# binli123/dsmil-wsi

Hardware: AMD Instinct MI355X
Metric: bags/sec aggregated (10kx512) (higher is better)
Workload: dtype f32; 1 GPU; DSMIL aggregator forward (FCLayer+BClassifier), c16 weights C=1, 64 bags x 10000 x 512 fp32 per GPU per pass, HBM-resident; bags_per_pass_per_gpu=64, rows=10000, feats=512, classes=1, tile_rows=128, parallelism=bag-sharded x1, streams=3, distinct_batches=3, logits_form=1, device_cus=256, persistent_grid=256

## Files before the change

### dsmil-wsi_amd/_native.py

```python
import ctypes
import os

PKG_DIR = os.path.dirname(os.path.abspath(__file__))
LIB_PATH = os.path.join(PKG_DIR, os.path.basename(os.environ.get("DSMIL_NATIVE_LIB", "libdsmil_hip.so")))

c_f32p = ctypes.c_void_p
c_i64p = ctypes.c_void_p


class NativeLibraryError(RuntimeError):
    pass


class AggParams(ctypes.Structure):
    _fields_ = [("fc_w", ctypes.c_void_p), ("fc_b", ctypes.c_void_p),
                ("q0_w", ctypes.c_void_p), ("q0_b", ctypes.c_void_p),
                ("q2_w", ctypes.c_void_p), ("q2_b", ctypes.c_void_p),
                ("fcc_w", ctypes.c_void_p), ("fcc_b", ctypes.c_void_p),
                ("K", ctypes.c_int32), ("Kv", ctypes.c_int32),
                ("C", ctypes.c_int32), ("nonlinear", ctypes.c_int32)]


class AggOpts(ctypes.Structure):
    _fields_ = [("packed_split", ctypes.c_void_p), ("row_map", ctypes.c_void_p), ("packed_f2", ctypes.c_void_p)]


class AggCall(ctypes.Structure):
    _fields_ = [("total_rows", ctypes.c_int64), ("max_rows", ctypes.c_int64)] + [(n, ctypes.c_int32) for n in (
        "n_bags", "K", "Kv", "C", "nonlinear", "bf16", "aligned", "classes_given", "vals_separate", "row_map", "packed_split",
        "packed_f2", "phase", "skip_pred", "prologue_job", "several_streams", "cus")]


class AggRoute(ctypes.Structure):
    _fields_ = [(n, ctypes.c_int32) for n in (
        "nw", "r0", "logits", "logits_vec", "logits_cp", "prologue", "rowmax", "qmax", "qmax_vec", "qmax_threads", "ragged",
        "ragged_attend", "tile_attend", "tile_logits", "image", "attend", "attend_nw", "attend_vec", "attend_np", "attend_xe",
        "attend_tu", "finish", "finish_rows", "pred")]


LOGITS = ("none", "given", "stream", "pipe", "argmax")
QMAX = ("launch", "inline", "shard1", "shard2")
IMAGE = ("none", "f2_caller", "f2_cut", "split_caller", "split_cut", "bf16")
ATTEND = ("none", "f3", "f2", "bf16_res", "bf16_dma", "bf16_ring", "split", "hs", "f32")
FINISH = ("none", "lean", "vec4", "scalar")


def forward_route(**call):
    c = AggCall(**dict({"aligned": 7}, **call))
    r = AggRoute()
    check(lib().dsmil_agg_forward_route(ctypes.byref(c), ctypes.byref(r)), "dsmil_agg_forward_route")
    return r


class AggGrads(ctypes.Structure):
    _fields_ = [(n, ctypes.c_void_p) for n in
                ("fc_w", "fc_b", "q0_w", "q0_b", "q2_w", "q2_b", "fcc_w", "fcc_b")]


class BceWeights(ctypes.Structure):
    _fields_ = [("pos_weight", ctypes.c_void_p), ("weight", ctypes.c_void_p)]


class AdamState(ctypes.Structure):
    _fields_ = [("exp_avg", ctypes.POINTER(ctypes.c_void_p)), ("exp_avg_sq", ctypes.POINTER(ctypes.c_void_p)),
                ("step", ctypes.c_int64), ("lr", ctypes.c_double), ("beta1", ctypes.c_double), ("beta2", ctypes.c_double),
                ("eps", ctypes.c_double), ("weight_decay", ctypes.c_double)]


SIGNATURES = {
    "dsmil_abi_version": (ctypes.c_int, []),
    "dsmil_strerror": (ctypes.c_char_p, [ctypes.c_int]),
    "dsmil_agg_mlp_form": (ctypes.c_int, []),
    "dsmil_agg_inline_query": (ctypes.c_int, [ctypes.c_int]),
    "dsmil_agg_batch_form": (ctypes.c_int, [ctypes.c_int]),
    "dsmil_agg_persistent_grid": (ctypes.c_int, [ctypes.c_int]),
    "dsmil_agg_logits_form": (ctypes.c_int, [ctypes.c_int]),
    "dsmil_device_cus": (ctypes.c_int, []),
    "dsmil_agg_packed_f2_bytes": (ctypes.c_size_t, [ctypes.c_int32]),
    "dsmil_agg_pack_f2": (ctypes.c_int, [c_f32p, c_f32p, ctypes.c_int32, ctypes.c_void_p, ctypes.c_void_p]),
    "dsmil_agg_packed_split_bytes": (ctypes.c_size_t, [ctypes.c_int32, ctypes.c_int32]),
    "dsmil_agg_pack_split": (ctypes.c_int, [c_f32p, c_f32p, ctypes.c_int32, ctypes.c_void_p, ctypes.c_void_p]),
    "dsmil_agg_forward_ex": (ctypes.c_int, [c_f32p, c_f32p, c_i64p, ctypes.c_int32, ctypes.c_int64,
                                            ctypes.c_int64, ctypes.POINTER(AggParams), ctypes.POINTER(AggOpts), c_f32p,
                                            c_f32p, c_f32p, c_f32p, c_f32p, c_i64p, ctypes.c_void_p,
                                            ctypes.c_size_t, ctypes.c_void_p]),
    "dsmil_agg_loss_head": (ctypes.c_int, [c_f32p, c_f32p, c_i64p, c_f32p, ctypes.c_int32, c_f32p, c_f32p, c_f32p,
                                           c_f32p, ctypes.c_void_p]),
    "dsmil_agg_loss_head_w": (ctypes.c_int, [c_f32p, c_f32p, c_i64p, c_f32p, ctypes.c_int32, c_f32p, c_f32p, c_f32p,
                                             c_f32p, ctypes.POINTER(BceWeights), ctypes.c_void_p]),
    "dsmil_agg_backward_ex": (ctypes.c_int, [c_f32p, c_f32p, ctypes.c_int64, ctypes.POINTER(AggParams), c_f32p,
                                             c_f32p, c_i64p, c_f32p, c_f32p, c_f32p, c_f32p, c_f32p,
                                             ctypes.POINTER(AggGrads), c_f32p, c_i64p, ctypes.c_void_p, ctypes.c_size_t,
                                             ctypes.c_void_p]),
    "dsmil_agg_shard_argmax": (ctypes.c_int, [c_f32p, ctypes.c_int64, ctypes.POINTER(AggParams), c_f32p, c_f32p,
                                              c_i64p, ctypes.c_void_p, ctypes.c_size_t, ctypes.c_void_p]),
    "dsmil_agg_shard_attend": (ctypes.c_int, [c_f32p, c_f32p, ctypes.c_int64, ctypes.POINTER(AggParams), c_f32p,
                                              c_f32p, c_f32p, c_f32p, ctypes.c_void_p, ctypes.c_size_t,
                                              ctypes.c_void_p]),
    "dsmil_agg_tile_rows": (ctypes.c_int, [ctypes.c_int32, ctypes.c_int64]),
    "dsmil_agg_forward_route": (ctypes.c_int, [ctypes.POINTER(AggCall), ctypes.POINTER(AggRoute)]),
    "dsmil_agg_workspace_bytes": (ctypes.c_size_t, [ctypes.c_int32, ctypes.c_int64, ctypes.c_int32,
                                                    ctypes.c_int32, ctypes.c_int32]),
    "dsmil_agg_packed_bf16_bytes": (ctypes.c_size_t, [ctypes.c_int32]),
    "dsmil_agg_pack_bf16": (ctypes.c_int, [c_f32p, c_f32p, ctypes.c_int32, ctypes.c_void_p, ctypes.c_void_p]),
    "dsmil_agg_forward_bf16": (ctypes.c_int, [ctypes.c_void_p, ctypes.c_void_p, c_i64p, ctypes.c_int32,
                                              ctypes.c_int64, ctypes.c_int64, ctypes.POINTER(AggParams),
                                              ctypes.c_void_p, c_f32p, c_f32p, c_f32p, c_f32p, c_f32p, c_i64p,
                                              ctypes.c_void_p, ctypes.c_size_t, ctypes.c_void_p]),
    "dsmil_profile_enable": (ctypes.c_int, [ctypes.c_int]),
    "dsmil_profile_collect": (ctypes.c_int, [ctypes.c_int, ctypes.POINTER(ctypes.c_double), ctypes.POINTER(ctypes.c_int64)]),
    "dsmil_resnet18_packed_bytes": (ctypes.c_size_t, []),
    "dsmil_resnet18_pack": (ctypes.c_int, [ctypes.POINTER(ctypes.c_void_p), c_f32p, ctypes.c_void_p]),
    "dsmil_resnet18_workspace_bytes": (ctypes.c_size_t, [ctypes.c_int32, ctypes.c_int32, ctypes.c_int32]),
    "dsmil_resnet18in_forward": (ctypes.c_int, [c_f32p, ctypes.c_int32, ctypes.c_int32, ctypes.c_int32,
                                                c_f32p, c_f32p, c_f32p, c_f32p, ctypes.c_int32, c_f32p,
                                                c_f32p, ctypes.c_void_p, ctypes.c_size_t, ctypes.c_void_p]),
    "dsmil_resnet18in_forward_u8": (ctypes.c_int, [ctypes.c_void_p, ctypes.c_int32, ctypes.c_int32, ctypes.c_int32,
                                                   c_f32p, c_f32p, c_f32p, c_f32p, ctypes.c_int32, c_f32p,
                                                   c_f32p, ctypes.c_void_p, ctypes.c_size_t, ctypes.c_void_p]),
    "dsmil_resnet18_norm_channels": (ctypes.c_int32, []),
    "dsmil_resnet18bn_forward": (ctypes.c_int, [ctypes.c_void_p, ctypes.c_int32, ctypes.c_int32, ctypes.c_int32,
                                                ctypes.c_int32, c_f32p, c_f32p, c_f32p, c_f32p, c_f32p, c_f32p,
                                                ctypes.c_int32, c_f32p, c_f32p, ctypes.c_void_p, ctypes.c_size_t,
                                                ctypes.c_void_p]),
    "dsmil_resnet_num_convs": (ctypes.c_int32, [ctypes.c_int32]),
    "dsmil_resnet_workspace_bytes": (ctypes.c_size_t, [ctypes.c_int32, ctypes.c_int32, ctypes.c_int32, ctypes.c_int32]),
    "dsmil_resnet_feature_dim": (ctypes.c_int32, [ctypes.c_int32]),
    "dsmil_resnet_mfma_forms": (ctypes.c_int, [ctypes.POINTER(ctypes.c_int32), ctypes.POINTER(ctypes.c_int32)]),
    "dsmil_resnet_norm_channels": (ctypes.c_int32, [ctypes.c_int32]),
    "dsmil_resnet_packed_bytes": (ctypes.c_size_t, [ctypes.c_int32]),
    "dsmil_resnet_packed_bytes_ex": (ctypes.c_size_t, [ctypes.c_int32, ctypes.c_int32]),
    "dsmil_resnet_pack": (ctypes.c_int, [ctypes.c_int32, ctypes.POINTER(ctypes.c_void_p), c_f32p, ctypes.c_void_p]),
    "dsmil_resnet_forward": (ctypes.c_int, [ctypes.c_int32, ctypes.c_void_p, ctypes.c_int32, ctypes.c_int32,
                                            ctypes.c_int32, ctypes.c_int32, c_f32p, c_f32p, c_f32p, c_f32p, c_f32p,
                                            c_f32p, ctypes.c_int32, c_f32p, c_f32p, ctypes.c_void_p,
                                            ctypes.c_size_t, ctypes.c_void_p]),
    "dsmil_resnet_pack_ex": (ctypes.c_int, [ctypes.c_int32, ctypes.POINTER(ctypes.c_void_p), c_f32p, ctypes.c_int32, ctypes.c_void_p]),
    "dsmil_resnet_forward_ex": (ctypes.c_int, [ctypes.c_int32, ctypes.c_void_p, ctypes.c_int32, ctypes.c_int32,
                                               ctypes.c_int32, ctypes.c_int32, c_f32p, c_f32p, c_f32p, c_f32p, c_f32p,
                                               c_f32p, ctypes.c_int32, c_f32p, c_f32p, ctypes.c_void_p,
                                               ctypes.c_size_t, ctypes.c_int32, ctypes.c_void_p]),
    "dsmil_trunk16_positions": (ctypes.c_size_t, [ctypes.c_int32, ctypes.c_int32, ctypes.c_int32]),
    "dsmil_trunk16_layout": (ctypes.c_int, [c_f32p, ctypes.c_void_p] + [ctypes.c_int32] * 6 + [ctypes.c_void_p]),
    "dsmil_trunk16_conv_workspace_bytes": (ctypes.c_size_t, [ctypes.c_int32, ctypes.c_int32, ctypes.c_int32]),
    "dsmil_trunk16_conv": (ctypes.c_int, [ctypes.c_void_p, c_f32p, ctypes.c_void_p] + [ctypes.c_int32] * 9 +
                           [ctypes.c_void_p, ctypes.c_size_t, ctypes.c_void_p]),
    "dsmil_trunk16_norm_workspace_bytes": (ctypes.c_size_t, [ctypes.c_int32, ctypes.c_int32]),
    "dsmil_trunk16_norm": (ctypes.c_int, [ctypes.c_void_p, ctypes.c_void_p, ctypes.c_void_p] + [ctypes.c_int32] * 6 +
                           [ctypes.c_void_p, ctypes.c_size_t, ctypes.c_void_p]),
    "dsmil_trunk16_pool": (ctypes.c_int, [ctypes.c_void_p, ctypes.c_void_p, c_f32p] + [ctypes.c_int32] * 5 +
                           [ctypes.c_void_p, ctypes.c_size_t, ctypes.c_void_p]),
    "dsmil_trunk16_workspace_bytes": (ctypes.c_size_t, [ctypes.c_int32] * 4),
    "dsmil_trunk16_forward": (ctypes.c_int, [ctypes.c_int32, c_f32p, ctypes.c_int32, ctypes.c_int32, ctypes.c_int32,
                                             ctypes.POINTER(ctypes.c_void_p), c_f32p, ctypes.c_int32, ctypes.c_void_p,
                                             ctypes.c_size_t, ctypes.c_void_p]),
    "dsmil_trunk32_conv_plan": (ctypes.c_int, [ctypes.c_int32] * 10 + [ctypes.POINTER(ctypes.c_int32)]),
    "dsmil_trunk32_conv_workspace_bytes": (ctypes.c_size_t, [ctypes.c_int32] * 9),
    "dsmil_trunk32_conv": (ctypes.c_int, [c_f32p] * 9 + [ctypes.c_int32] * 9 + [ctypes.c_void_p, ctypes.c_size_t, ctypes.c_void_p]),
    "dsmil_trunk32_stem_workspace_bytes": (ctypes.c_size_t, [ctypes.c_int32] * 3),
    "dsmil_trunk32_stem": (ctypes.c_int, [ctypes.c_void_p, ctypes.c_int32] + [c_f32p] * 6 + [ctypes.c_int32] * 4 +
                           [ctypes.c_void_p, ctypes.c_size_t, ctypes.c_void_p]),
    "dsmil_trunk32_tail": (ctypes.c_int, [ctypes.c_int32] + [c_f32p] * 7 + [ctypes.c_int32] * 4 + [ctypes.c_void_p]),
    "dsmil_tile_stats": (ctypes.c_int, [ctypes.c_void_p, ctypes.c_int32, ctypes.c_int32, ctypes.c_int32, ctypes.c_void_p,
                                        ctypes.c_void_p]),
    "dsmil_jpeg_plan_bytes": (ctypes.c_size_t, [ctypes.c_int32]),
    "dsmil_jpeg_workspace_bytes": (ctypes.c_size_t, [ctypes.c_int32, ctypes.c_int32, ctypes.c_int32, ctypes.c_int64]),
    "dsmil_jpeg_parse": (ctypes.c_int, [ctypes.c_void_p, ctypes.c_void_p, ctypes.c_int32, ctypes.c_void_p]),
    "dsmil_read_files": (ctypes.c_int64, [ctypes.c_void_p, ctypes.c_void_p, ctypes.c_int32, ctypes.c_void_p, ctypes.c_int64, ctypes.c_void_p]),
    "dsmil_csv_parse_f32": (ctypes.c_int64, [ctypes.c_void_p, ctypes.c_int64, ctypes.c_int64, ctypes.c_void_p, ctypes.c_int64]),
    "dsmil_csv_format_f32": (ctypes.c_int64, [ctypes.c_void_p, ctypes.c_int64, ctypes.c_int64, ctypes.c_int64, ctypes.c_int32,
                                              ctypes.c_void_p, ctypes.c_int64]),
    "dsmil_jpeg_decode": (ctypes.c_int, [ctypes.c_void_p, ctypes.c_int64, ctypes.c_void_p, ctypes.c_int32, ctypes.c_int32, ctypes.c_int32,
                                         ctypes.c_void_p, ctypes.c_void_p, ctypes.c_void_p, ctypes.c_size_t, ctypes.c_void_p]),
    "dsmil_fc_forward": (ctypes.c_int, [c_f32p, ctypes.c_int64, ctypes.c_int32, ctypes.c_int32,
                                        c_f32p, c_f32p, c_f32p, ctypes.c_void_p]),
    "dsmil_agg_backward_workspace_bytes": (ctypes.c_size_t, [ctypes.c_int64, ctypes.c_int32, ctypes.c_int32,
                                                             ctypes.c_int32]),
    "dsmil_agg_backward": (ctypes.c_int, [c_f32p, c_f32p, ctypes.c_int64, ctypes.POINTER(AggParams), c_f32p,
                                          c_f32p, c_i64p, c_f32p, c_f32p, c_f32p, c_f32p,
                                          ctypes.POINTER(AggGrads), c_f32p, ctypes.c_void_p, ctypes.c_size_t,
                                          ctypes.c_void_p]),
    "dsmil_agg_backward_rows_workspace_bytes": (ctypes.c_size_t, [ctypes.c_int64, ctypes.c_int32, ctypes.c_int32,
                                                                  ctypes.c_int32]),
    "dsmil_agg_backward_rows": (ctypes.c_int, [c_f32p, c_f32p, ctypes.c_int64, ctypes.POINTER(AggParams), c_f32p,
                                               c_f32p, c_i64p, c_f32p, c_f32p, c_f32p, c_f32p, c_f32p,
                                               ctypes.POINTER(AggGrads), c_f32p, c_i64p, ctypes.c_void_p, ctypes.c_size_t,
                                               ctypes.c_void_p, c_f32p]),
    "dsmil_agg_backward_bags_workspace_bytes": (ctypes.c_size_t, [ctypes.c_int32, ctypes.c_int64, ctypes.c_int32,
                                                                  ctypes.c_int32, ctypes.c_int32]),
    "dsmil_agg_backward_bags": (ctypes.c_int, [c_f32p, c_f32p, c_i64p, ctypes.c_int32, ctypes.c_int64, ctypes.c_int64,
                                               ctypes.POINTER(AggParams), c_f32p, c_f32p, c_i64p, c_f32p, c_f32p, c_f32p,
                                               c_f32p, c_f32p, ctypes.POINTER(AggGrads), c_f32p, c_i64p, ctypes.c_void_p,
                                               ctypes.c_size_t, ctypes.c_void_p, c_f32p]),
    "dsmil_agg_backward_bags_bf16_workspace_bytes": (ctypes.c_size_t, [ctypes.c_int32, ctypes.c_int64, ctypes.c_int32,
                                                                       ctypes.c_int32, ctypes.c_int32]),
    "dsmil_agg_backward_bags_bf16": (ctypes.c_int, [ctypes.c_void_p, ctypes.c_void_p, c_i64p, ctypes.c_int32, ctypes.c_int64,
                                                    ctypes.c_int64, ctypes.POINTER(AggParams), c_f32p, c_f32p, c_i64p, c_f32p,
                                                    c_f32p, c_f32p, c_f32p, c_f32p, ctypes.POINTER(AggGrads), c_f32p,
                                                    ctypes.c_void_p, ctypes.c_size_t, ctypes.c_void_p]),
    "dsmil_agg_loss_head_bags": (ctypes.c_int, [c_f32p, c_i64p, c_f32p, c_i64p, c_f32p, ctypes.c_int32, ctypes.c_int32,
                                                c_f32p, c_f32p, c_f32p, c_f32p, ctypes.c_void_p]),
    "dsmil_agg_loss_head_bags_w": (ctypes.c_int, [c_f32p, c_i64p, c_f32p, c_i64p, c_f32p, ctypes.c_int32, ctypes.c_int32,
                                                  c_f32p, c_f32p, c_f32p, c_f32p, ctypes.POINTER(BceWeights), ctypes.c_void_p]),
    "dsmil_value_backward_rows": (ctypes.c_int, [c_f32p, c_f32p, c_f32p, ctypes.c_int64, ctypes.c_int32, ctypes.c_int32,
                                                 c_f32p, ctypes.c_void_p, ctypes.c_int32, c_f32p, ctypes.c_void_p,
                                                 ctypes.c_size_t, ctypes.c_void_p]),
    "dsmil_value_packed_bytes": (ctypes.c_size_t, [ctypes.c_int32, ctypes.c_int32]),
    "dsmil_value_pack": (ctypes.c_int, [c_f32p, ctypes.c_int32, ctypes.c_int32, ctypes.c_void_p, ctypes.c_void_p]),
    "dsmil_value_workspace_bytes": (ctypes.c_size_t, [ctypes.c_int64, ctypes.c_int32, ctypes.c_int32]),
    "dsmil_value_forward": (ctypes.c_int, [c_f32p, ctypes.c_int64, ctypes.c_int32, ctypes.c_int32, c_f32p, c_f32p,
                                           ctypes.c_void_p, c_i64p, c_f32p, ctypes.c_void_p, ctypes.c_size_t, ctypes.c_void_p]),
    "dsmil_value_backward": (ctypes.c_int, [c_f32p, c_f32p, c_f32p, ctypes.c_int64, ctypes.c_int32, ctypes.c_int32, c_i64p,
                                            c_f32p, c_f32p, ctypes.c_void_p, ctypes.c_size_t, ctypes.c_void_p]),
    "dsmil_value_packed_bf16_bytes": (ctypes.c_size_t, [ctypes.c_int32, ctypes.c_int32]),
    "dsmil_value_pack_bf16": (ctypes.c_int, [c_f32p, ctypes.c_int32, ctypes.c_int32, ctypes.c_void_p, ctypes.c_void_p]),
    "dsmil_value_workspace_bf16_bytes": (ctypes.c_size_t, [ctypes.c_int64, ctypes.c_int32, ctypes.c_int32]),
    "dsmil_value_forward_bf16": (ctypes.c_int, [ctypes.c_void_p, ctypes.c_int64, ctypes.c_int32, ctypes.c_int32, c_f32p, c_f32p,
                                                ctypes.c_void_p, ctypes.c_void_p, ctypes.c_void_p, ctypes.c_size_t,
                                                ctypes.c_void_p]),
    "dsmil_value_backward_bf16_workspace_bytes": (ctypes.c_size_t, [ctypes.c_int64, ctypes.c_int32, ctypes.c_int32]),
    "dsmil_value_backward_bf16": (ctypes.c_int, [ctypes.c_void_p, ctypes.c_void_p, c_f32p, ctypes.c_int64, ctypes.c_int32,
                                                 ctypes.c_int32, c_f32p, c_f32p, ctypes.c_void_p, ctypes.c_size_t,
                                                 ctypes.c_void_p]),
    "dsmil_agg_train_step_workspace_bytes": (ctypes.c_size_t, [ctypes.c_int64, ctypes.c_int32, ctypes.c_int32, ctypes.c_int32]),
    "dsmil_agg_train_step": (ctypes.c_int, [c_f32p, ctypes.c_int64, c_i64p, c_f32p, ctypes.POINTER(AggParams),
                                            ctypes.POINTER(AdamState), c_f32p, ctypes.c_void_p, ctypes.c_size_t,
                                            ctypes.c_void_p]),
    "dsmil_agg_train_step_bags_workspace_bytes": (ctypes.c_size_t, [ctypes.c_int32, ctypes.c_int64, ctypes.c_int32,
                                                                    ctypes.c_int32, ctypes.c_int32]),
# ... 73 lines not shown
```

### dsmil-wsi_amd/csrc/agg_f3.h

```cpp
#pragma once
#include "agg_f2.h"

namespace {

constexpr int F3_BM = 32;
constexpr int F3_THREADS = 256;
constexpr int F3_MAX_WG = 1024;
constexpr int F3_HROW = 528;
constexpr int F3_SCR = 1856;
__host__ __device__ constexpr int f3_row_bytes(int K) { return 4 * K + 16; }
__host__ __device__ constexpr int f3_lds_bytes(int K) { return 2 * F3_BM * f3_row_bytes(K) + F3_BM * F3_HROW + F3_SCR * 4; }

__device__ __forceinline__ void f3_mfma_a(f32x4& acc, const f32x4& a_agpr, const f32x4& b) {
    asm volatile("v_mfma_f32_16x16x32_f16 %0, %1, %2, %0" : "+v"(acc) : "a"(a_agpr), "v"(b));
}
__device__ __forceinline__ void f3_mfma_a0(f32x4& acc, const f32x4& a_agpr, const f32x4& b) {
    asm volatile("v_mfma_f32_16x16x32_f16 %0, %1, %2, 0" : "=&v"(acc) : "a"(a_agpr), "v"(b));
}
__device__ __forceinline__ void f3_mfma_v(f32x4& acc, const f32x4& a, const f32x4& b) {
    asm volatile("v_mfma_f32_16x16x32_f16 %0, %1, %2, %0" : "+v"(acc) : "v"(a), "v"(b));
}
__device__ __forceinline__ void f3_mfma_v0(f32x4& acc, const f32x4& a, const f32x4& b) {
    asm volatile("v_mfma_f32_16x16x32_f16 %0, %1, %2, 0" : "=&v"(acc) : "v"(a), "v"(b));
}
#define F3_NOP() asm volatile("s_nop 15" ::: "memory")

template <int B, int E, class F>
__device__ __forceinline__ void f3_static_for(F&& f) {
    if constexpr (B < E) {
        f(std::integral_constant<int, B>{});
        f3_static_for<B + 1, E>(f);
    }
}

struct F3Work {
    int bag;
    long long off0, Nb, row0;
};

struct F3Cur {
    int item, b, tile;
};
__device__ __forceinline__ F3Cur f3_next(F3Cur c, int tiles_per_bag) {
    ++c.item;
    if (++c.tile == tiles_per_bag) { c.tile = 0; ++c.b; }
    return c;
}

__device__ __forceinline__ bool f3_fetch(const AttendArgs& a, int tiles_per_bag, int end, F3Cur& c, F3Work& w, const F3Work* hint = nullptr) {
    const __attribute__((address_space(4))) long long* offs = (const __attribute__((address_space(4))) long long*)(uintptr_t)a.offsets;
    while (c.item < end) {
        const int bag = a.bag0 + c.b;
        long long off0, Nb;
        if (hint && hint->bag == bag) { off0 = hint->off0; Nb = hint->Nb; }
        else { off0 = offs[bag]; Nb = offs[bag + 1] - off0; }
        const long long row0 = (long long)c.tile * F3_BM;
        if (row0 < Nb) {
            w.bag = bag; w.off0 = off0; w.Nb = Nb; w.row0 = row0;
            return true;
        }
        if (tiles_per_bag) c.item += tiles_per_bag - c.tile;
        c.tile = 0;
        ++c.b;
    }
    return false;
}

template <int NK1, bool TWO, int DBG = 0>
__global__ __launch_bounds__(F3_THREADS, 1) void k_attend_f3(AttendArgs a, const float* __restrict__ rowmax, int tiles_per_bag,
                                                             int n_items, int per_wg) {
    static_assert(NK1 % 4 == 0 && NK1 >= 4 && NK1 <= 16, "K a multiple of 128 up to 512");
    constexpr int K = 32 * NK1, NKS = 2 * NK1, NG = NK1 / 2;
    constexpr int RB = f3_row_bytes(K), BUF = F3_BM * RB;
    constexpr int NC = TWO ? 2 : 1;
    constexpr bool W2_STREAM = NK1 > 8;
    constexpr int NMOVE = 2;
    extern __shared__ __attribute__((aligned(16))) float smem[];
    char* sX = reinterpret_cast<char*>(smem);
    char* sH = sX + 2 * BUF;
    float* scr = reinterpret_cast<float*>(sH + F3_BM * F3_HROW);
    float* sS = scr;
    float* sBias = scr + 1024;
    float* sPall = scr + 1280;
    float* sInvAll = scr + 1536;
    float* sQ = scr + 1600;
    const int tid = threadIdx.x, lane = tid & 63;
    const int wave = __builtin_amdgcn_readfirstlane(tid >> 6);
    const int l31 = lane & 31, hi = lane >> 5;
    const int l15 = lane & 15, g = lane >> 4;
    const int ubase = 32 * wave + 16 * (g >> 1) + 4 * (g & 1);
    const f32x4* wimg = reinterpret_cast<const f32x4*>(a.wpk);
    const float* trailer = reinterpret_cast<const float*>(wimg + (long long)(NKS + 8) * F2_CHUNK_F4);
    const float* feats = reinterpret_cast<const float*>(a.feats);
    const float scale = 0.08838834764831845f;

    F3Cur pos;
    pos.item = (int)blockIdx.x * per_wg;
    if (a.tile_pre) {
        const int real = ((const __attribute__((address_space(4))) int*)(uintptr_t)a.tile_pre)[a.n_bags];
        n_items = n_items < real ? n_items : real;
        if (pos.item >= n_items) return;
        pos.b = tile_owner(a.tile_pre, a.n_bags, pos.item);
        pos.tile = pos.item - a.tile_pre[pos.b];
    } else {
        pos.b = pos.item / tiles_per_bag;
        pos.tile = pos.item - pos.b * tiles_per_bag;
    }
    const int item_end = pos.item + per_wg < n_items ? pos.item + per_wg : n_items;
    F3Work cur, nxt, nn;
    if (!f3_fetch(a, tiles_per_bag, item_end, pos, cur)) return;

    F2Frag w1[NK1][2][2], w2[4][2][2];
#pragma unroll
    for (int s = 0; s < NK1; ++s)
#pragma unroll
        for (int uh = 0; uh < 2; ++uh)
#pragma unroll
            for (int p = 0; p < 2; ++p) w1[s][uh][p].f = wimg[f3_frag_slot(s, 2 * wave + uh, p, lane)];
    const f32x4* w2p1 = wimg + f3_frag_slot(NK1, 2 * wave, 1, lane);
#pragma unroll
    for (int st = 0; st < 4; ++st)
#pragma unroll
        for (int uh = 0; uh < 2; ++uh) {
            w2[st][uh][0].f = wimg[f3_frag_slot(NK1 + st, 2 * wave + uh, 0, lane)];
            if constexpr (!W2_STREAM) w2[st][uh][1].f = w2p1[(long long)2 * st * F2_CHUNK_F4 + 8 * uh];
        }
    const float ia1 = trailer[0], ia2 = trailer[1];
    const float hb_n1 = trailer[2] * 16384.f;
    const float hb_b = wave_max(fmaxf(fabsf(a.q0_b[lane]), fabsf(a.q0_b[lane + 64])));
    sBias[tid] = tid < QD ? a.q0_b[tid] : a.q2_b[tid - QD];
#pragma unroll
    for (int s = 0; s < NK1; ++s)
#pragma unroll
        for (int uh = 0; uh < 2; ++uh)
#pragma unroll
            for (int p = 0; p < 2; ++p) asm volatile("" : "+a"(w1[s][uh][p].f));

    const int rr = lane & 7, o = lane >> 3;
    const int myrow = 8 * wave + rr;
    f32x4 ring[NG][2];
    auto row_raw = [&](const F3Work& w, float& rm, long long& phys, long long& logical) {
        long long gr = w.row0 + myrow;
        if (gr >= w.Nb) gr = w.Nb - 1;
        rm = rowmax[w.off0 + gr];
        const long long* mp = a.rowmap ? reinterpret_cast<const long long*>(a.rowmap) + (w.off0 + gr) : reinterpret_cast<const long long*>(a.offsets);
        phys = *mp;
        logical = w.off0 + gr;
    };
    auto row_done = [&](float rm, long long phys, long long logical, float& sc, float& sinv) -> const float* {
        sc = f2_scale(rm, sinv);
        return feats + (a.rowmap ? phys : logical) * (long long)K + 8 * o;
    };
    auto row_src = [&](const F3Work& w, float& sc, float& sinv) -> const float* {
        float rm;
        long long phys, logical;
        row_raw(w, rm, phys, logical);
        asm volatile("" : "+v"(phys));
        return row_done(rm, phys, logical, sc, sinv);
    };
    auto fill = [&](const float* src, int c) {
        ring[c][0] = *(const DSMIL_GLOBAL f32x4*)(src + 64 * c);
        ring[c][1] = *(const DSMIL_GLOBAL f32x4*)(src + 64 * c + 4);
    };
    char* const cut_dst = sX + myrow * RB + 16 * o;
    auto cut_write = [&](int pb, int c, float sc) {
        F2Frag f[2];
        split2h_scaled(ring[c][0], ring[c][1], sc, f);
        char* d = cut_dst + pb * BUF + 128 * c;
        *reinterpret_cast<f32x4*>(d) = f[0].f;
        *reinterpret_cast<f32x4*>(d + 2 * K) = f[1].f;
    };

    F2Frag cutf[2];
    auto cut_piece = [&](int pb, auto s_c, auto j_c, float sc, const float* refill_src) {
        constexpr int s_ = decltype(s_c)::value, j = decltype(j_c)::value;
        constexpr int c = s_ / 2, ph = (s_ % 2) * 8 + j;
        if constexpr (c < NG) {
            char* d = cut_dst + pb * BUF + 128 * c;
            if constexpr (ph < 8) {
                constexpr int i = ph / 2;
                const float va = i < 2 ? ring[c][0][(2 * i) & 3] : ring[c][1][(2 * i) & 3];
                const float vb = i < 2 ? ring[c][0][(2 * i + 1) & 3] : ring[c][1][(2 * i + 1) & 3];
                if constexpr (ph % 2 == 0) {
                    unsigned h;
                    asm("v_fma_mixlo_f16 %0, %1, %3, 0\n\tv_fma_mixhi_f16 %0, %2, %3, 0" : "=&v"(h) : "v"(va), "v"(vb), "v"(sc));
                    cutf[0].u[i] = h;
                } else {
                    unsigned l;
                    const unsigned h = cutf[0].u[i];
                    asm("v_fma_mixlo_f16 %0, %1, %3, -%4 op_sel_hi:[0,0,1]\n\tv_fma_mixhi_f16 %0, %2, %3, -%4 op_sel:[0,0,1] op_sel_hi:[0,0,1]"
                        : "=&v"(l) : "v"(va), "v"(vb), "v"(sc), "v"(h));
                    cutf[1].u[i] = l;
                }
            } else if constexpr (ph == 8) {
                *reinterpret_cast<f32x4*>(d) = cutf[0].f;
            } else if constexpr (ph == 9) {
                *reinterpret_cast<f32x4*>(d + 2 * K) = cutf[1].f;
            } else if constexpr (ph == 10) {
                if constexpr (DBG != 4 && c < NG - NMOVE) fill(refill_src, c);
            }
        }
    };

    float sc_c = 1.f, sinv_c = 1.f, sc_n = 1.f, sinv_n = 1.f, sc_nn = 1.f, sinv_nn = 1.f;
    const float* src_c = row_src(cur, sc_c, sinv_c);
#pragma unroll
    for (int c = 0; c < NG; ++c) fill(src_c, c);
    F3Cur pos_n = f3_next(pos, tiles_per_bag);
    bool has_next = f3_fetch(a, tiles_per_bag, item_end, pos_n, nxt);
    const float* src_n = has_next ? row_src(nxt, sc_n, sinv_n) : src_c;
    if (!has_next) { nxt = cur; sc_n = sc_c; sinv_n = sinv_c; }
#pragma unroll
    for (int c = 0; c < NG; ++c) {
        cut_write(0, c, sc_c);
        fill(src_n, c);
    }
    if (o == 0) sInvAll[myrow] = sinv_c;
    F3Cur pos_nn = f3_next(pos_n, tiles_per_bag);
    bool has_nn = has_next && f3_fetch(a, tiles_per_bag, item_end, pos_nn, nn);
    const float* src_nn = has_nn ? row_src(nn, sc_nn, sinv_nn) : src_n;
    if (!has_nn) { nn = nxt; sc_nn = sc_n; sinv_nn = sinv_n; }

    float bacc[NC][8];
    float l_run[NC];
    float m_bag[NC];
    auto reset_acc = [&]() {
#pragma unroll
        for (int c = 0; c < NC; ++c) {
            l_run[c] = 0.f;
#pragma unroll
            for (int e = 0; e < 8; ++e) bacc[c][e] = 0.f;
        }
    };
    reset_acc();
#pragma unroll
    for (int c = 0; c < NC; ++c) m_bag[c] = 0.f;
    int qbag = -1;
    float* sPw = sPall + wave * 64;

    unsigned long long stamps[16];
#pragma unroll
    for (int i = 0; i < 16; ++i) stamps[i] = 0;
    auto STAMP = [&](int i) {
        if constexpr (DBG >= 1) {
            __builtin_amdgcn_sched_barrier(0);
            asm volatile("s_waitcnt vmcnt(63) lgkmcnt(0)" ::: "memory");
            stamps[i] = __builtin_readcyclecounter();
            __builtin_amdgcn_sched_barrier(0);
        }
    };
    for (int t = 0;; ++t) {
        const int buf = t & 1;
        STAMP(0);
        if (cur.bag != qbag) {
            __syncthreads();
            if (tid < NC * QD) sQ[tid] = a.qmax[(long long)cur.bag * a.C * QD + tid];
            qbag = cur.bag;
            __syncthreads();
#pragma unroll
            for (int c = 0; c < NC; ++c) m_bag[c] = wave_sum(fabsf(sQ[c * QD + lane]) + fabsf(sQ[c * QD + 64 + lane])) * scale;
        }
        F3Cur pos_n3 = f3_next(pos_nn, tiles_per_bag);
        F3Work n3 = nn;
        float rm_n3;
        long long phys_n3, log_n3;
        const bool has_n3 = has_nn && f3_fetch(a, tiles_per_bag, item_end, pos_n3, n3, &nn);
        if (!has_n3) n3 = nn;
        row_raw(n3, rm_n3, phys_n3, log_n3);
        __syncthreads();
        STAMP(1);
        const char* xb_ = sX + buf * BUF + (2 * l15) * RB + 16 * g;
        const float* sInv = sInvAll + buf * F3_BM;
        f32x4 Hacc[2][2];
        {
            F2Frag xs[2][2][2];
            auto rd = [&](int s_, int rh, int p, F2Frag& d) {
                d.f = *reinterpret_cast<const f32x4*>(xb_ + rh * RB + p * (2 * K) + 64 * s_);
            };
#pragma unroll
            for (int q = 0; q < 4; ++q) rd(0, q >> 1, q & 1, xs[0][q >> 1][q & 1]);
            f3_static_for<0, NK1>([&](auto s_c) {
                constexpr int s = decltype(s_c)::value;
                f3_static_for<0, 12>([&](auto j_c) {
                    constexpr int j = decltype(j_c)::value;
                    constexpr int pr = j / 4, uh = (j >> 1) & 1, rh = j & 1;
                    constexpr int pa = pr == 0 ? 1 : 0, pb = pr == 1 ? 1 : 0;
                    __builtin_amdgcn_sched_barrier(0);
                    if constexpr (s == 0 && pr == 0) f3_mfma_a0(Hacc[uh][rh], w1[s][uh][pa].f, xs[s % 2][rh][pb].f);
                    else f3_mfma_a(Hacc[uh][rh], w1[s][uh][pa].f, xs[s % 2][rh][pb].f);
                    if constexpr (j < 4) {
                        if constexpr (DBG != 3 && DBG != 5 && s + 1 < NK1) rd(s + 1, j >> 1, j & 1, xs[(s + 1) % 2][j >> 1][j & 1]);
                    } else if constexpr (DBG != 2 && DBG != 5) {
                        cut_piece(buf ^ 1, s_c, std::integral_constant<int, j - 4>{}, sc_n, src_nn);
                    }
                });
                __builtin_amdgcn_sched_barrier(0);
                if constexpr (s == 3) STAMP(10);
                if constexpr (s == 7) STAMP(11);
                if constexpr (s == 11) STAMP(12);
            });
            F3_NOP();
        }
        if (o == 0) sInvAll[(buf ^ 1) * F3_BM + myrow] = sinv_n;
        if constexpr (W2_STREAM) {
#pragma unroll
            for (int st = 0; st < 4; ++st)
#pragma unroll
                for (int uh = 0; uh < 2; ++uh) w2[st][uh][1].f = *(const DSMIL_GLOBAL f32x4*)(w2p1 + (long long)2 * st * F2_CHUNK_F4 + 8 * uh);
        }
        STAMP(2);
        const float rinv1[2] = {sInv[2 * l15], sInv[2 * l15 + 1]};
#pragma unroll
        for (int uh = 0; uh < 2; ++uh) {
            const f32x4 bq = *reinterpret_cast<const f32x4*>(sBias + ubase + 8 * uh);
#pragma unroll
            for (int rh = 0; rh < 2; ++rh) {
                const float iv1 = ia1 * rinv1[rh];
#pragma unroll
                for (int e = 0; e < 4; ++e) Hacc[uh][rh][e] = fmaxf(fmaf(Hacc[uh][rh][e], iv1, bq[e]), 0.f);
            }
        }
        STAMP(3);
        float hinv[2];
#pragma unroll
        for (int rh = 0; rh < 2; ++rh) {
            const float hsc = f2_scale(fmaf(hb_n1, rinv1[rh], hb_b), hinv[rh]);
            F2Frag f[2];
            split2h_scaled(Hacc[0][rh], Hacc[1][rh], hsc, f);
            char* d = sH + (2 * l15 + rh) * F3_HROW + 64 * wave + 16 * g;
            *reinterpret_cast<f32x4*>(d) = f[0].f;
            *reinterpret_cast<f32x4*>(d + 256) = f[1].f;
        }
        __syncthreads();
        STAMP(4);
        f32x4 Qacc[2][2];
        {
            const char* hb_ = sH + (2 * l15) * F3_HROW + 16 * g;
            F2Frag hs[2][2][2];
            auto rdh = [&](int st_, F2Frag (&d)[2][2]) {
#pragma unroll
                for (int rh = 0; rh < 2; ++rh)
#pragma unroll
                    for (int p = 0; p < 2; ++p) d[rh][p].f = *reinterpret_cast<const f32x4*>(hb_ + rh * F3_HROW + 256 * p + 64 * st_);
            };
            rdh(0, hs[0]);
            f3_static_for<0, 4>([&](auto st_c) {
                constexpr int st = decltype(st_c)::value;
                if constexpr (st + 1 < 4) rdh(st + 1, hs[(st + 1) % 2]);
                f3_static_for<0, 12>([&](auto j_c) {
                    constexpr int j = decltype(j_c)::value;
                    constexpr int pr = j / 4, uh = (j >> 1) & 1, rh = j & 1;
                    constexpr int pa = pr == 0 ? 1 : 0, pb = pr == 1 ? 1 : 0;
                    __builtin_amdgcn_sched_barrier(0);
                    if constexpr (st == 0 && pr == 0) f3_mfma_v0(Qacc[uh][rh], w2[st][uh][pa].f, hs[st % 2][rh][pb].f);
                    else f3_mfma_v(Qacc[uh][rh], w2[st][uh][pa].f, hs[st % 2][rh][pb].f);
                    if constexpr (DBG != 4 && st == 0 && j % 6 == 5 && j / 6 < NMOVE) fill(src_nn, NG - NMOVE + j / 6);
                });
                __builtin_amdgcn_sched_barrier(0);
            });
            F3_NOP();
        }
        STAMP(5);
        {
            float s0[2] = {0.f, 0.f}, s1[2] = {0.f, 0.f};
#pragma unroll
            for (int uh = 0; uh < 2; ++uh) {
                const f32x4 bq = *reinterpret_cast<const f32x4*>(sBias + QD + ubase + 8 * uh);
                const f32x4 u0 = *reinterpret_cast<const f32x4*>(sQ + ubase + 8 * uh);
                f32x4 u1 = u0;
                if constexpr (TWO) u1 = *reinterpret_cast<const f32x4*>(sQ + QD + ubase + 8 * uh);
#pragma unroll
                for (int rh = 0; rh < 2; ++rh) {
                    const float iv2 = ia2 * hinv[rh];
#pragma unroll
                    for (int e = 0; e < 4; ++e) {
                        const float qv = fast_tanh(fmaf(Qacc[uh][rh][e], iv2, bq[e]));
                        s0[rh] = fmaf(qv, u0[e], s0[rh]);
                        if constexpr (TWO) s1[rh] = fmaf(qv, u1[e], s1[rh]);
                    }
                }
            }
#pragma unroll
            for (int rh = 0; rh < 2; ++rh) {
                sS[((wave * 4 + g) * 2 + 0) * F3_BM + 2 * l15 + rh] = s0[rh];
                if constexpr (TWO) sS[((wave * 4 + g) * 2 + 1) * F3_BM + 2 * l15 + rh] = s1[rh];
            }
        }
        STAMP(6);
        __syncthreads();
        STAMP(7);
        {
            const long long grow = cur.row0 + l31;
            const bool valid = grow < cur.Nb;
            const float rinv = sInv[l31];
#pragma unroll
            for (int c = 0; c < NC; ++c) {
                auto part = [&](int i) { return sS[(i * 2 + c) * F3_BM + l31]; };
                auto quad = [&](int i) { return (part(i) + part(i + 1)) + (part(i + 2) + part(i + 3)); };
                const float s = ((quad(0) + quad(4)) + (quad(8) + quad(12))) * scale;
                const float p = valid ? expf(s - m_bag[c]) : 0.f;
                if (hi == 0) l_run[c] += p;
                if (DBG == 0 && wave == 0 && hi == 0 && valid) a.scores[(cur.off0 + grow) * (long long)a.C + c] = s;
                if (hi == 0) sPw[c * F3_BM + l31] = p * rinv;
            }
        }
        STAMP(8);
        if (lane < K / 8) {
            const char* xv = sX + buf * BUF + (8 * wave) * RB + 16 * lane;
#pragma unroll
            for (int j = 0; j < 8; ++j) {
                F2Frag f0, f1;
                f0.f = *reinterpret_cast<const f32x4*>(xv + j * RB);
                f1.f = *reinterpret_cast<const f32x4*>(xv + j * RB + 2 * K);
#pragma unroll
                for (int c = 0; c < NC; ++c) {
                    const float w = sPw[c * F3_BM + 8 * wave + j];
#pragma unroll
                    for (int e = 0; e < 8; ++e) {
                        bacc[c][e] = fmaf((float)f0.v[e], w, bacc[c][e]);
                        bacc[c][e] = fmaf((float)f1.v[e], w, bacc[c][e]);
                    }
                }
            }
        }
        STAMP(9);
        if constexpr (DBG >= 1) {
            if (tid == 0 && !TWO && cur.row0 + F3_BM <= cur.Nb) {
                unsigned long long* so = reinterpret_cast<unsigned long long*>(a.scores + (cur.off0 + cur.row0));
#pragma unroll
                for (int i = 0; i < 16; ++i) so[i] = stamps[i];
            }
        }
        if (!has_next || nxt.bag != cur.bag) {
            const long long slot = (long long)blockIdx.x + cur.bag;
            float* red = reinterpret_cast<float*>(sH);
            __syncthreads();
            if (lane < K / 8) {
#pragma unroll
                for (int c = 0; c < NC; ++c) {
                    float* d = red + (wave * NC + c) * K + 8 * lane;
                    *reinterpret_cast<f32x4*>(d) = f32x4{bacc[c][0], bacc[c][1], bacc[c][2], bacc[c][3]};
                    *reinterpret_cast<f32x4*>(d + 4) = f32x4{bacc[c][4], bacc[c][5], bacc[c][6], bacc[c][7]};
                }
            }
            __syncthreads();
            for (int i = tid; i < NC * K; i += F3_THREADS) {
                const int c = i / K, k = i - c * K;
                const float v = (red[(0 * NC + c) * K + k] + red[(1 * NC + c) * K + k]) + (red[(2 * NC + c) * K + k] + red[(3 * NC + c) * K + k]);
                a.part_B[(slot * a.C + c) * (long long)a.Kv + k] = v;
            }
            if (wave == 0) {
#pragma unroll
                for (int c = 0; c < NC; ++c) {
                    const float lsum = wave_sum(hi == 0 ? l_run[c] : 0.f);
                    if (lane == 0) {
                        float* ml = a.part_ml + (slot * a.C + c) * 2;
                        ml[0] = m_bag[c];
                        ml[1] = lsum;
                    }
                }
            }
            reset_acc();
        }
        STAMP(13);
        if constexpr (DBG >= 1) {
            if (tid == 0 && !TWO && cur.row0 + F3_BM <= cur.Nb)
                reinterpret_cast<unsigned long long*>(a.scores + (cur.off0 + cur.row0))[13] = stamps[13];
        }
        if (!has_next) break;
        cur = nxt; nxt = nn; nn = n3;
        has_next = has_nn; has_nn = has_n3;
        pos_nn = pos_n3;
        sc_c = sc_n; sinv_c = sinv_n;
        sc_n = sc_nn; sinv_n = sinv_nn; src_n = src_nn;
        asm volatile("" : "+v"(rm_n3), "+v"(phys_n3));
        src_nn = row_done(rm_n3, phys_n3, log_n3, sc_nn, sinv_nn);
    }
}

}
```

### dsmil-wsi_amd/csrc/agg_fwd.hip

```cpp

#include <hip/hip_runtime.h>
#include <stdint.h>
#include <math.h>
#include <stdio.h>
#include <stdlib.h>
#include <string.h>
#include <atomic>
#include "dsmil_hip.h"
#include "prof.h"

#include "agg_common.h"
#include "agg_split.h"
#include "agg_hs.h"
#include "agg_f2.h"
#include "agg_f3.h"
#include "agg_res.h"
#define DSMIL_VALUE_FWD
#include "agg_value.h"
#include "lds_attr.h"

namespace {

template <int VEC, bool GIVEN, typename T = float>
__device__ __forceinline__ void logits_tile(
    const T* __restrict__ feats, const int64_t* __restrict__ offsets,
    const float* __restrict__ fc_w, const float* __restrict__ fc_b,
    const float* __restrict__ classes_in, float* __restrict__ classes_out,
    float* __restrict__ part_val, long long* __restrict__ part_idx, int K, int C,
    int bag, int tile, float* s_v, long long* s_i, const int64_t* __restrict__ rowmap) {
    const long long off0 = offsets[bag];
    const long long Nb = offsets[bag + 1] - off0;
    const long long row0 = (long long)tile * R0;
    if (row0 >= Nb) return;
    const int lane = threadIdx.x & 63, wave = threadIdx.x >> 6;
    const long long slot = off0 / R0 + bag + tile;

    for (int c0 = 0; c0 < C; c0 += 2) {
        const int c1 = (c0 + 1 < C) ? c0 + 1 : c0;
        float bv0 = -INFINITY, bv1 = -INFINITY;
        long long bi0 = 0x7fffffffffffffffLL, bi1 = 0x7fffffffffffffffLL;
        for (int rg = 0; rg < 8; ++rg) {
            const long long rbase = row0 + wave * 32 + rg * 4;
            if (rbase >= Nb) break;
            float va0, va1, vb0, vb1, vc0, vc1, vd0, vd1;
            const long long ra = rbase, rb = (rbase + 1 < Nb) ? rbase + 1 : Nb - 1,
                            rc = (rbase + 2 < Nb) ? rbase + 2 : Nb - 1, rd = (rbase + 3 < Nb) ? rbase + 3 : Nb - 1;
            if constexpr (!GIVEN) {
                const T* xa = feats + phys_row(rowmap, off0 + ra) * (long long)K;
                const T* xb = feats + phys_row(rowmap, off0 + rb) * (long long)K;
                const T* xc = feats + phys_row(rowmap, off0 + rc) * (long long)K;
                const T* xd = feats + phys_row(rowmap, off0 + rd) * (long long)K;
                const float* w0p = fc_w + (long long)c0 * K;
                const float* w1p = fc_w + (long long)c1 * K;
                va0 = va1 = vb0 = vb1 = vc0 = vc1 = vd0 = vd1 = 0.f;
                for (int k0 = 0; k0 < K; k0 += 256) {
                    const int k = k0 + lane * 4;
                    const f32x4 w0 = load4<VEC>(w0p, k, K);
                    const f32x4 w1 = load4<VEC>(w1p, k, K);
                    const f32x4 a = load4<VEC, T>(xa, k, K);
                    const f32x4 b = load4<VEC, T>(xb, k, K);
                    const f32x4 c = load4<VEC, T>(xc, k, K);
                    const f32x4 d = load4<VEC, T>(xd, k, K);
#pragma unroll
                    for (int e = 0; e < 4; ++e) {
                        va0 = fmaf(a[e], w0[e], va0); va1 = fmaf(a[e], w1[e], va1);
                        vb0 = fmaf(b[e], w0[e], vb0); vb1 = fmaf(b[e], w1[e], vb1);
                        vc0 = fmaf(c[e], w0[e], vc0); vc1 = fmaf(c[e], w1[e], vc1);
                        vd0 = fmaf(d[e], w0[e], vd0); vd1 = fmaf(d[e], w1[e], vd1);
                    }
                }
                const float b0 = fc_b[c0], b1 = fc_b[c1];
                va0 = wave_sum(va0) + b0; va1 = wave_sum(va1) + b1;
                vb0 = wave_sum(vb0) + b0; vb1 = wave_sum(vb1) + b1;
                vc0 = wave_sum(vc0) + b0; vc1 = wave_sum(vc1) + b1;
                vd0 = wave_sum(vd0) + b0; vd1 = wave_sum(vd1) + b1;
                if (lane < 4 && rbase + lane < Nb) {
                    const float o0 = lane == 0 ? va0 : lane == 1 ? vb0 : lane == 2 ? vc0 : vd0;
                    const float o1 = lane == 0 ? va1 : lane == 1 ? vb1 : lane == 2 ? vc1 : vd1;
                    float* o = classes_out + (off0 + rbase + lane) * (long long)C;
                    o[c0] = o0;
                    if (c1 != c0) o[c1] = o1;
                }
            } else {
                const float* ci = classes_in + off0 * (long long)C;
                va0 = ci[ra * C + c0]; va1 = ci[ra * C + c1];
                vb0 = ci[rb * C + c0]; vb1 = ci[rb * C + c1];
                vc0 = ci[rc * C + c0]; vc1 = ci[rc * C + c1];
                vd0 = ci[rd * C + c0]; vd1 = ci[rd * C + c1];
            }
            if (better(va0, ra, bv0, bi0)) { bv0 = va0; bi0 = ra; }
            if (better(vb0, rb, bv0, bi0)) { bv0 = vb0; bi0 = rb; }
            if (better(vc0, rc, bv0, bi0)) { bv0 = vc0; bi0 = rc; }
            if (better(vd0, rd, bv0, bi0)) { bv0 = vd0; bi0 = rd; }
            if (better(va1, ra, bv1, bi1)) { bv1 = va1; bi1 = ra; }
            if (better(vb1, rb, bv1, bi1)) { bv1 = vb1; bi1 = rb; }
            if (better(vc1, rc, bv1, bi1)) { bv1 = vc1; bi1 = rc; }
            if (better(vd1, rd, bv1, bi1)) { bv1 = vd1; bi1 = rd; }
        }
        __syncthreads();
        if (lane == 0) { s_v[wave] = bv0; s_i[wave] = bi0; s_v[4 + wave] = bv1; s_i[4 + wave] = bi1; }
        __syncthreads();
        if (threadIdx.x < 2 && (threadIdx.x == 0 || c1 != c0)) {
            const int h = threadIdx.x * 4;
            float bv = s_v[h];
            long long bi = s_i[h];
            for (int w = 1; w < 4; ++w)
                if (better(s_v[h + w], s_i[h + w], bv, bi)) { bv = s_v[h + w]; bi = s_i[h + w]; }
            const int c = threadIdx.x ? c1 : c0;
            part_val[slot * C + c] = bv;
            part_idx[slot * C + c] = bi;
        }
    }
}

template <int VEC, bool GIVEN, typename T = float>
__global__ __launch_bounds__(256) void k_logits_argmax(
    const T* __restrict__ feats, const int64_t* __restrict__ offsets,
    const float* __restrict__ fc_w, const float* __restrict__ fc_b,
    const float* __restrict__ classes_in, float* __restrict__ classes_out,
    float* __restrict__ part_val, long long* __restrict__ part_idx, int K, int C, int bag0,
    const int64_t* __restrict__ rowmap) {
    __shared__ float s_v[8];
    __shared__ long long s_i[8];
    logits_tile<VEC, GIVEN, T>(feats, offsets, fc_w, fc_b, classes_in, classes_out, part_val, part_idx, K, C,
                               bag0 + (int)blockIdx.y, (int)blockIdx.x, s_v, s_i, rowmap);
}

template <typename T>
struct StreamVec;
template <>
struct StreamVec<float> {
    static constexpr int EPL = 4;
    f32x4 v;
    __device__ __forceinline__ void load(const float* p) { v = __builtin_nontemporal_load((const DSMIL_GLOBAL f32x4*)p); }
    __device__ __forceinline__ float at(int e) const { return v[e]; }
};
template <>
struct StreamVec<bf16_t> {
    static constexpr int EPL = 8;
    typedef unsigned u32x4_t __attribute__((ext_vector_type(4)));
    u32x4_t v;
    __device__ __forceinline__ void load(const bf16_t* p) { v = __builtin_nontemporal_load((const DSMIL_GLOBAL u32x4_t*)p); }
    __device__ __forceinline__ float at(int e) const {
        const unsigned w = v[e >> 1];
        return __uint_as_float((e & 1) ? (w & 0xffff0000u) : (w << 16));
    }
};

template <int CP, typename T>
__global__ __launch_bounds__(256, (CP == 1 ? 6 : 3)) void k_logits_stream(
    const T* __restrict__ feats, const int64_t* __restrict__ offsets,
    const float* __restrict__ fc_w, const float* __restrict__ fc_b, float* __restrict__ classes_out,
    float* __restrict__ part_val, long long* __restrict__ part_idx, int K, int C, int bag0,
    const int64_t* __restrict__ rowmap, int r0 = R0, int* __restrict__ qm_flag = nullptr,
    TrainPrologueJob job = TrainPrologueJob{}, float* __restrict__ rowmax = nullptr,
    const int* __restrict__ tile_pre = nullptr, int n_bags = 0) {
    if (qm_flag && blockIdx.x == 0 && (int)threadIdx.x < C) qm_flag[(long long)(bag0 + (int)blockIdx.y) * C + threadIdx.x] = 0;
    if (job.blocks) {
        const int first = (int)gridDim.x - job.blocks;
        if ((int)blockIdx.x >= first) {
// ... 113 lines not shown
        __syncthreads();
        if (tid < 2 && (tid == 0 || c1 != c0)) {
            const int h = tid * 4;
            float bv = s_v[h];
            long long bi = s_i[h];
            for (int w = 1; w < 4; ++w)
                if (better(s_v[h + w], s_i[h + w], bv, bi)) { bv = s_v[h + w]; bi = s_i[h + w]; }
            const int c = tid ? c1 : c0;
            part_val[slot * C + c] = bv;
            part_idx[slot * C + c] = bi;
        }
    }
}

template <int CP>
__global__ __launch_bounds__(256, 6) void k_logits_pipe(
    const bf16_t* __restrict__ feats, const int64_t* __restrict__ offsets,
    const float* __restrict__ fc_w, const float* __restrict__ fc_b, float* __restrict__ classes_out,
    float* __restrict__ part_val, long long* __restrict__ part_idx, int bag0,
    int r0, const int* __restrict__ tile_pre, int n_bags) {
    constexpr int K = 512, SEG = 64;
    __shared__ __attribute__((aligned(16))) float s_w[CP * K];
    __shared__ float s_v[8];
    __shared__ int s_i[8];
    int bag = bag0 + (int)blockIdx.y, tile = (int)blockIdx.x;
    if (tile_pre) {
        if ((int)blockIdx.x >= tile_pre[n_bags]) return;
        const int b = tile_owner(tile_pre, n_bags, (int)blockIdx.x);
        bag = bag0 + b;
        tile = (int)blockIdx.x - tile_pre[b];
    }
    const long long off0 = offsets[bag];
    const long long Nbl = offsets[bag + 1] - off0;
    const long long row0l = (long long)tile * r0;
    if (row0l >= Nbl) return;
    const int Nb = (int)Nbl, row0 = (int)row0l;
    const int tid = threadIdx.x, lane = tid & 63, wave = tid >> 6;
    const int j = lane & 7, rr = lane >> 3;
    const int ngrp = r0 >> 5, rpw = r0 >> 2;
    const int wbase = row0 + wave * rpw;
    int ng = 0;
    if (wbase < Nb) { const int left = (Nb - wbase + 7) >> 3; ng = left < ngrp ? left : ngrp; }
    for (int i = tid; i < CP * K; i += 256) s_w[i] = fc_w[i];
    __syncthreads();
    const float b0 = fc_b[0], b1 = fc_b[CP - 1];
    float bv0 = -INFINITY, bv1 = -INFINITY;
    int bi0 = 0x7fffffff, bi1 = 0x7fffffff;
    if (ng > 0) {
        typedef StreamVec<bf16_t> SV;
        const bf16_t* fbase = feats + j * 8;
        auto row_of = [&](int g) { const int r = wbase + g * 8 + rr; return r < Nb ? r : Nb - 1; };
        auto ptr_of = [&](int r) { return fbase + (off0 + r) * (long long)K; };
        SV va[4], vb[4];
        float a0 = 0.f, a1 = 0.f;
        const unsigned wad = (unsigned)(size_t)(__attribute__((address_space(3))) float*)s_w + j * 32;
        auto piece = [&](const SV& v, auto off_tag) {
            constexpr int OFF = decltype(off_tag)::value;
            f32x4 wa, wb, wc, wd;
            if constexpr (CP == 2) {
                asm volatile("ds_read_b128 %0, %6 offset:%7\n\tds_read_b128 %1, %6 offset:%8\n\t"
                             "ds_read_b128 %2, %6 offset:%9\n\tds_read_b128 %3, %6 offset:%10\n\ts_waitcnt lgkmcnt(0)"
                             : "=&v"(wa), "=&v"(wb), "=&v"(wc), "=&v"(wd), "+v"(a0), "+v"(a1)
                             : "v"(wad), "n"(OFF), "n"(OFF + 16), "n"(OFF + K * 4), "n"(OFF + K * 4 + 16) : "memory");
            } else {
                asm volatile("ds_read_b128 %0, %3 offset:%4\n\tds_read_b128 %1, %3 offset:%5\n\ts_waitcnt lgkmcnt(0)"
                             : "=&v"(wa), "=&v"(wb), "+v"(a0) : "v"(wad), "n"(OFF), "n"(OFF + 16) : "memory");
            }
#pragma unroll
            for (int e = 0; e < 4; ++e) a0 = fmaf(v.at(e), wa[e], a0);
#pragma unroll
            for (int e = 0; e < 4; ++e) a0 = fmaf(v.at(4 + e), wb[e], a0);
            if constexpr (CP == 2) {
#pragma unroll
                for (int e = 0; e < 4; ++e) a1 = fmaf(v.at(e), wc[e], a1);
#pragma unroll
                for (int e = 0; e < 4; ++e) a1 = fmaf(v.at(4 + e), wd[e], a1);
            }
        };
        auto consume_lo = [&](const SV (&v)[4]) {
            piece(v[0], std::integral_constant<int, 0 * 256>{}); piece(v[1], std::integral_constant<int, 1 * 256>{});
            piece(v[2], std::integral_constant<int, 2 * 256>{}); piece(v[3], std::integral_constant<int, 3 * 256>{});
        };
        auto consume_hi = [&](const SV (&v)[4]) {
            piece(v[0], std::integral_constant<int, 4 * 256>{}); piece(v[1], std::integral_constant<int, 5 * 256>{});
            piece(v[2], std::integral_constant<int, 6 * 256>{}); piece(v[3], std::integral_constant<int, 7 * 256>{});
        };
        auto finish_rows = [&](int g, int r) {
#pragma unroll
            for (int m = 1; m < 8; m <<= 1) {
                a0 += __shfl_xor(a0, m, 64);
                if constexpr (CP == 2) a1 += __shfl_xor(a1, m, 64);
            }
            a0 += b0;
            a1 += b1;
            if (j == 0 && wbase + g * 8 + rr < Nb) {
                float* o = classes_out + (off0 + r) * (long long)CP;
                o[0] = a0;
                if constexpr (CP == 2) o[1] = a1;
            }
            if (a0 > bv0 || (a0 == bv0 && r < bi0)) { bv0 = a0; bi0 = r; }
            if (CP == 2 && (a1 > bv1 || (a1 == bv1 && r < bi1))) { bv1 = a1; bi1 = r; }
            a0 = 0.f;
            a1 = 0.f;
        };
        int r = row_of(0);
        const bf16_t* x = ptr_of(r);
#pragma unroll
        for (int u = 0; u < 4; ++u) va[u].load(x + u * SEG);
#pragma unroll 1
        for (int g = 0; g + 1 < ng; ++g) {
            const int rn = row_of(g + 1);
            const bf16_t* xn = ptr_of(rn);
#pragma unroll
            for (int u = 0; u < 4; ++u) vb[u].load(x + (4 + u) * SEG);
            consume_lo(va);
#pragma unroll
            for (int u = 0; u < 4; ++u) va[u].load(xn + u * SEG);
            consume_hi(vb);
            finish_rows(g, r);
            r = rn;
            x = xn;
        }
#pragma unroll
        for (int u = 0; u < 4; ++u) vb[u].load(x + (4 + u) * SEG);
        consume_lo(va);
        consume_hi(vb);
        finish_rows(ng - 1, r);
    }
#pragma unroll
    for (int m = 8; m < 64; m <<= 1) {
        const float ov0 = __shfl_xor(bv0, m, 64);
        const int oi0 = __shfl_xor(bi0, m, 64);
        if (ov0 > bv0 || (ov0 == bv0 && oi0 < bi0)) { bv0 = ov0; bi0 = oi0; }
        if constexpr (CP == 2) {
            const float ov1 = __shfl_xor(bv1, m, 64);
            const int oi1 = __shfl_xor(bi1, m, 64);
            if (ov1 > bv1 || (ov1 == bv1 && oi1 < bi1)) { bv1 = ov1; bi1 = oi1; }
        }
    }
    if (lane == 0) { s_v[wave] = bv0; s_i[wave] = bi0; s_v[4 + wave] = bv1; s_i[4 + wave] = bi1; }
    __syncthreads();
    if (tid < CP) {
        const int h = tid * 4;
        float bv = s_v[h];
        int bi = s_i[h];
        for (int w = 1; w < 4; ++w)
            if (s_v[h + w] > bv || (s_v[h + w] == bv && s_i[h + w] < bi)) { bv = s_v[h + w]; bi = s_i[h + w]; }
        const long long slot = off0 / r0 + bag + tile;
        part_val[slot * CP + tid] = bv;
        part_idx[slot * CP + tid] = bi == 0x7fffffff ? 0x7fffffffffffffffLL : (long long)bi;
    }
}

template <int VEC, typename T = float, bool PRE = false>
__device__ __forceinline__ void qmax_block(
    const T* __restrict__ feats, const int64_t* __restrict__ offsets,
    const float* __restrict__ part_val, const long long* __restrict__ part_idx,
    const float* __restrict__ q0_w, const float* __restrict__ q0_b,
    const float* __restrict__ q2_w, const float* __restrict__ q2_b,
    float* __restrict__ qmax, int64_t* __restrict__ idx_out, int K, int C, int nonlinear,
    int bag, int c, float* s_v, long long* s_i, float* s_h, int mode = 0, float* __restrict__ best_val_out = nullptr,
    const int64_t* __restrict__ rowmap = nullptr, int r0 = R0) {
    const long long off0 = mode == 2 ? 0 : offsets[bag];
    const long long Nb = mode == 2 ? C : offsets[bag + 1] - off0;
    const int lane = threadIdx.x & 63, wave = threadIdx.x >> 6;
    const int nwv = (int)blockDim.x >> 6;
    const int upw = QD / nwv;
    const long long slot0 = off0 / r0 + bag;
    const long long ntile = mode == 2 ? 0 : (Nb + r0 - 1) / r0;
    f32x4 w1r[PRE ? 32 : 1];
    float w2r[PRE ? 32 : 1];
    bool pre = false;
    float bv = -INFINITY;
    long long bi = 0x7fffffffffffffffLL;
    long long t_next = threadIdx.x;
    if constexpr (PRE) {
        pre = K == 512 && nwv == 8 && nonlinear && VEC == 4;
        if (pre) {
            if (t_next < ntile) {
                bv = part_val[(slot0 + t_next) * C + c];
                bi = part_idx[(slot0 + t_next) * C + c];
                t_next += blockDim.x;
            }
            __builtin_amdgcn_sched_barrier(0);
#pragma unroll
            for (int jb = 0; jb < 2; ++jb)
#pragma unroll
                for (int kk = 0; kk < 2; ++kk)
#pragma unroll
                    for (int u = 0; u < 8; ++u)
                        w1r[(jb * 2 + kk) * 8 + u] = *reinterpret_cast<const f32x4*>(q0_w + (long long)(wave * 16 + jb * 8 + u) * 512 + kk * 256 + lane * 4);
#pragma unroll
            for (int jb = 0; jb < 2; ++jb)
#pragma unroll
                for (int u = 0; u < 8; ++u) {
                    const float* wr = q2_w + (long long)(wave * 16 + jb * 8 + u) * QD;
                    w2r[(jb * 8 + u) * 2] = wr[lane];
                    w2r[(jb * 8 + u) * 2 + 1] = wr[lane + 64];
                }
            __builtin_amdgcn_sched_barrier(0);
        }
    }
    for (long long t = t_next; t < ntile; t += blockDim.x) {
        const float v = part_val[(slot0 + t) * C + c];
        const long long i = part_idx[(slot0 + t) * C + c];
        if (better(v, i, bv, bi)) { bv = v; bi = i; }
    }
#pragma unroll
    for (int o = 32; o >= 1; o >>= 1) {
        const float ov = __shfl_xor(bv, o, 64);
        const long long oi = __shfl_xor(bi, o, 64);
        if (better(ov, oi, bv, bi)) { bv = ov; bi = oi; }
    }
    if (lane == 0) { s_v[wave] = bv; s_i[wave] = bi; }
    __syncthreads();
    bv = s_v[0]; bi = s_i[0];
    for (int w = 1; w < nwv; ++w)
        if (better(s_v[w], s_i[w], bv, bi)) { bv = s_v[w]; bi = s_i[w]; }
    long long best = mode == 2 ? c : bi;
    if (best < 0 || best >= Nb) best = 0;
    if (threadIdx.x == 0 && mode != 2) {
        idx_out[(long long)bag * C + c] = best;
        if (best_val_out) best_val_out[(long long)bag * C + c] = bv;
    }
    if (mode == 1) return;
    const T* x = feats + (mode == 2 ? best : phys_row(rowmap, off0 + best)) * (long long)K;
    if (PRE && pre) {
        const f32x4 xv0 = load4<VEC, T>(x, lane * 4, K), xv1 = load4<VEC, T>(x, 256 + lane * 4, K);
#pragma unroll
        for (int jb = 0; jb < 2; ++jb) {
            float acc[8] = {0.f, 0.f, 0.f, 0.f, 0.f, 0.f, 0.f, 0.f};
#pragma unroll
            for (int kk = 0; kk < 2; ++kk) {
                const f32x4 xv = kk ? xv1 : xv0;
#pragma unroll
                for (int u = 0; u < 8; ++u) {
                    const f32x4 wv = w1r[(jb * 2 + kk) * 8 + u];
#pragma unroll
                    for (int e = 0; e < 4; ++e) acc[u] = fmaf(xv[e], wv[e], acc[u]);
                }
            }
#pragma unroll
            for (int u = 0; u < 8; ++u) {
                const float a = fmaxf(wave_sum(acc[u]) + q0_b[wave * 16 + jb * 8 + u], 0.f);
                if (lane == 0) s_h[wave * 16 + jb * 8 + u] = a;
            }
        }
        __syncthreads();
        float* out = qmax + ((long long)bag * C + c) * QD;
        const float h0 = s_h[lane], h1 = s_h[lane + 64];
#pragma unroll
        for (int jb = 0; jb < 2; ++jb) {
            float acc[8];
#pragma unroll
            for (int u = 0; u < 8; ++u) acc[u] = fmaf(h0, w2r[(jb * 8 + u) * 2], h1 * w2r[(jb * 8 + u) * 2 + 1]);
#pragma unroll
            for (int u = 0; u < 8; ++u) {
                const float a = wave_sum(acc[u]) + q2_b[wave * 16 + jb * 8 + u];
                if (lane == 0) out[wave * 16 + jb * 8 + u] = tanhf(a);
            }
        }
        return;
    }
    for (int jb = 0; jb < upw; jb += 8) {
        float acc[8] = {0.f, 0.f, 0.f, 0.f, 0.f, 0.f, 0.f, 0.f};
        const float* wr = q0_w + (long long)(wave * upw + jb) * K;
        for (int k0 = 0; k0 < K; k0 += 256) {
            const int k = k0 + lane * 4;
            const f32x4 xv = load4<VEC, T>(x, k, K);
#pragma unroll
            for (int u = 0; u < 8; ++u) {
                const f32x4 wv = load4<VEC>(wr + (long long)u * K, k, K);
#pragma unroll
                for (int e = 0; e < 4; ++e) acc[u] = fmaf(xv[e], wv[e], acc[u]);
            }
        }
#pragma unroll
        for (int u = 0; u < 8; ++u) {
            float a = wave_sum(acc[u]) + q0_b[wave * upw + jb + u];
            if (nonlinear) a = fmaxf(a, 0.f);
            if (lane == 0) s_h[wave * upw + jb + u] = a;
        }
    }
    __syncthreads();
    float* out = qmax + ((long long)bag * C + c) * QD;
    if (!nonlinear) {
        if (threadIdx.x < QD) out[threadIdx.x] = s_h[threadIdx.x];
        return;
    }
    const float h0 = s_h[lane], h1 = s_h[lane + 64];
    for (int jb = 0; jb < upw; jb += 8) {
        float acc[8];
#pragma unroll
        for (int u = 0; u < 8; ++u) {
            const float* wr = q2_w + (long long)(wave * upw + jb + u) * QD;
            acc[u] = fmaf(h0, wr[lane], h1 * wr[lane + 64]);
        }
#pragma unroll
        for (int u = 0; u < 8; ++u) {
            const float a = wave_sum(acc[u]) + q2_b[wave * upw + jb + u];
            if (lane == 0) out[wave * upw + jb + u] = tanhf(a);
        }
    }
}

constexpr int QMAX_T = 1024;
// ... 322 lines not shown
                for (int sidx = 0; sidx < 2; ++sidx) {
                    union { unsigned u[4]; bf16x8 v; } hb;
#pragma unroll
                    for (int e = 0; e < 4; ++e)
                        hb.u[e] = pack_bf16x2(H[t][8 * sidx + 2 * e], H[t][8 * sidx + 2 * e + 1]);
#pragma unroll
                    for (int t2 = 0; t2 < 4; ++t2) {
                        union { f32x4 f; bf16x8 v; } wa;
                        wa.f = w[((tt * 2 + sidx) * 4 + t2) * 64];
                        Q[t2] = __builtin_amdgcn_mfma_f32_32x32x16_bf16(wa.v, hb.v, Q[t2], 0, 0, 0);
                    }
                }
            }
            S3_WAIT_VM(0);
            __builtin_amdgcn_s_barrier();
        }
#pragma unroll
        for (int t = 0; t < 4; ++t)
#pragma unroll
            for (int g = 0; g < 4; ++g) {
                const f32x4 b = *reinterpret_cast<const f32x4*>(a.q2_b + 32 * t + 8 * g + 4 * hi);
#pragma unroll
                for (int e = 0; e < 4; ++e) Q[t][4 * g + e] = fast_tanh(Q[t][4 * g + e] + b[e]);
            }
    } else {
#pragma unroll
        for (int t = 0; t < 4; ++t) Q[t] = H[t];
    }
    attend_tail<NW, 4, bf16_t>(a, Q, smem, bag, off0, Nb, row0, slot);
}

__global__ void k_pack_agg_bf16(const float* __restrict__ q0_w, const float* __restrict__ q2_w,
                                bf16_t* __restrict__ out, int K, int K64) {
    const int n1 = QD * K64;
    const int nrow = n1 + QD * QD;
    const int nfrag = (K64 / 64 + 2) * BD_WCHUNK_F4 * 8;
    for (int i = blockIdx.x * blockDim.x + threadIdx.x; i < nrow + nfrag; i += gridDim.x * blockDim.x) {
        if (i < n1) {
            const int j = i / K64, k = i - j * K64;
            out[i] = k < K ? f2bf(q0_w[(long long)j * K + k]) : (bf16_t)0;
        } else if (i < nrow) {
            const int q = i - n1, j = q / QD, kk = q - j * QD;
            const int base = kk & ~15, r = kk & 15, hi = r >> 3, e = r & 7;
            out[i] = q2_w ? f2bf(q2_w[j * QD + base + (e & 3) + 8 * (e >> 2) + 4 * hi]) : (bf16_t)0;
        } else {
            int r = i - nrow;
            const int e = r & 7; r >>= 3;
            const int lane = r & 63; r >>= 6;
            const int t = r & 3; r >>= 2;
            const int ks = r & 3; r >>= 2;
            const int s = r, l31 = lane & 31, hi = lane >> 5;
            float v = 0.f;
            if (s < K64 / 64) {
                const int k = 64 * s + 16 * ks + 8 * hi + e;
                if (k < K) v = q0_w[(long long)(32 * t + l31) * K + k];
            } else if (q2_w) {
                const int c2 = s - K64 / 64, tt = ks >> 1, sidx = ks & 1;
                v = q2_w[(32 * t + l31) * QD + 32 * (2 * c2 + tt) + 16 * sidx + (e & 3) + 8 * (e >> 2) + 4 * hi];
            }
            out[i] = f2bf(v);
        }
    }
}

__device__ __forceinline__ void publish_flag(int* flag) {
    __builtin_amdgcn_fence(__ATOMIC_RELEASE, "agent");
    asm volatile("s_waitcnt vmcnt(0)" ::: "memory");
    __hip_atomic_store(flag, 1, __ATOMIC_RELAXED, __HIP_MEMORY_SCOPE_AGENT);
}

template <int NP>
__global__ __launch_bounds__(HS_THREADS, 2) void k_attend_hs(AttendArgs a) {
    extern __shared__ __attribute__((aligned(16))) float smem[];
    const int bag = a.bag0 + (int)blockIdx.y;
    int tile = (int)blockIdx.x;
    if (a.qm_flag) {
        if (tile < a.C) {
            if (a.offsets[bag + 1] <= a.offsets[bag]) {
                if (threadIdx.x == 0) {
                    a.qm_idx[(long long)bag * a.C + tile] = 0;
                    publish_flag(a.qm_flag + (long long)bag * a.C + tile);
                }
                return;
            }
            long long* s_i = reinterpret_cast<long long*>(smem);
            float* s_v = smem + 2 * (HS_THREADS / 64), *s_h = s_v + HS_THREADS / 64;
            qmax_block<4, float, true>(reinterpret_cast<const float*>(a.feats), a.offsets, a.qm_part_val, a.qm_part_idx, a.q0_w, a.q0_b,
                                 a.q2_w, a.q2_b, const_cast<float*>(a.qmax), a.qm_idx, a.K, a.C, a.nonlinear, bag, tile, s_v, s_i,
                                 s_h, 0, nullptr, a.rowmap, a.qm_r0);
            __syncthreads();
            if (threadIdx.x == 0) publish_flag(a.qm_flag + (long long)bag * a.C + tile);
            return;
        }
        tile -= a.C;
    }
    f32x16 Hw[HS_RG], Qw[HS_RG];
    if (!mlp_tile_hs<NP>(a, bag, tile, smem, Hw, Qw)) return;
    const long long off0 = a.offsets[bag];
    const long long Nb = a.offsets[bag + 1] - off0;
    attend_tail_hs<float>(a, Qw, smem + HS_STAGE + HS_PLANES, smem, bag, off0, Nb, (long long)tile * HS_BM, off0 / HS_BM + bag + tile);
#ifdef DSMIL_TRACE
    if (DSMIL_EXPT_ON(a, 64) && threadIdx.x == 0 && a.C == 1)
        reinterpret_cast<unsigned long long*>(a.scores + (off0 + (long long)tile * HS_BM) * (long long)a.C)[4] = __builtin_readcyclecounter();
#endif
}

__global__ __launch_bounds__(1024) void k_tile_prefix(const int64_t* __restrict__ offsets, int n_bags, int BMa, int BMb,
                                                      int* __restrict__ pre_a, int* __restrict__ pre_b) {
    __shared__ int s_w[2][16];
    __shared__ int s_base[2];
    const int tid = threadIdx.x, lane = tid & 63, wave = tid >> 6;
    if (tid < 2) s_base[tid] = 0;
    __syncthreads();
    for (int b0 = 0; b0 < n_bags; b0 += 1024) {
        const int b = b0 + tid;
        int v[2] = {0, 0}, x[2];
        if (b < n_bags) {
            const long long n = offsets[b + 1] - offsets[b];
            v[0] = (int)((n + BMa - 1) / BMa);
            v[1] = (int)((n + BMb - 1) / BMb);
        }
#pragma unroll
        for (int q = 0; q < 2; ++q) {
            x[q] = v[q];
#pragma unroll
            for (int d = 1; d < 64; d <<= 1) {
                const int y = __shfl_up(x[q], d);
                if (lane >= d) x[q] += y;
            }
            if (lane == 63) s_w[q][wave] = x[q];
        }
        __syncthreads();
        int before[2] = {s_base[0], s_base[1]};
        for (int w = 0; w < wave; ++w) { before[0] += s_w[0][w]; before[1] += s_w[1][w]; }
        if (b < n_bags) { pre_a[b] = before[0] + x[0] - v[0]; pre_b[b] = before[1] + x[1] - v[1]; }
        __syncthreads();
        if (tid == 1023) { s_base[0] = before[0] + x[0]; s_base[1] = before[1] + x[1]; }
        __syncthreads();
    }
    if (tid == 0) { pre_a[n_bags] = s_base[0]; pre_b[n_bags] = s_base[1]; }
}

constexpr int FR = 2048;
inline long long finish_blocks(long long max_rows, int Kv) {
    const long long a = (max_rows + FR - 1) / FR, b = (Kv + 63) / 64;
    return a > b ? (a > 1 ? a : 1) : b;
}

template <int VEC, int UB = 8>
__global__ __launch_bounds__(256, (UB == 8 ? 1 : 6)) void k_finish(
    const int64_t* __restrict__ offsets, const float* __restrict__ part_ml,
    const float* __restrict__ part_B, const float* __restrict__ fcc_w,
    float* __restrict__ A, float* __restrict__ B, float* __restrict__ pred_part, int Kv, int C, int BM,
    float* __restrict__ ml_out = nullptr, int seg_per = 0, int seg_T = 0, const int* __restrict__ tile_pre = nullptr) {
    const int bag = blockIdx.y, nblk = gridDim.x;
    const long long off0 = offsets[bag];
    const long long Nb = offsets[bag + 1] - off0;
    long long slot0 = off0 / BM + bag;
    long long ntile = (Nb + BM - 1) / BM;
    if (seg_per > 0 && ntile > 0) {
        const long long it0 = tile_pre ? (long long)tile_pre[bag] : (long long)bag * seg_T, g_lo = it0 / seg_per, g_hi = (it0 + ntile - 1) / seg_per;
        slot0 = g_lo + bag;
        ntile = g_hi - g_lo + 1;
    }
    const int tid = threadIdx.x, lane = tid & 63, wave = tid >> 6;
    __shared__ float s_red[8];
    __shared__ __attribute__((aligned(16))) float s_acc[16][64];
    const int kb = (int)blockIdx.x * 64;
    const bool has_k = kb < Kv;
    long long rpb = (Nb + nblk - 1) / nblk;
    rpb = rpb < 256 ? 256 : rpb;
    const long long rbeg = (long long)blockIdx.x * rpb;
    const long long rend = (rbeg + rpb < Nb) ? rbeg + rpb : Nb;
    const int kq = tid & 15, tg = tid >> 4;
    constexpr int UA = UB == 8 ? 8 : 4;
    if (!has_k && rbeg >= rend && !ml_out) {
        for (int i = tid; i < C * C; i += 256) pred_part[(((long long)bag * nblk + blockIdx.x) * C) * C + i] = 0.f;
        return;
    }
    for (int c = 0; c < C; ++c) {
        float m = -INFINITY;
        for (long long t = tid; t < ntile; t += 256) m = fmaxf(m, part_ml[((slot0 + t) * C + c) * 2]);
        m = wave_max(m);
        __syncthreads();
        if (lane == 0) s_red[wave] = m;
        __syncthreads();
        m = fmaxf(fmaxf(s_red[0], s_red[1]), fmaxf(s_red[2], s_red[3]));
        float l = 0.f;
        for (long long t = tid; t < ntile; t += 256) {
            const float* ml = part_ml + ((slot0 + t) * C + c) * 2;
            l += ml[1] * expf(ml[0] - m);
        }
        l = wave_sum(l);
        if (lane == 0) s_red[4 + wave] = l;
        __syncthreads();
        l = (s_red[4] + s_red[5]) + (s_red[6] + s_red[7]);
        const float il = ml_out ? 1.f : 1.f / l;
        if (ml_out && blockIdx.x == 0 && tid == 0) { ml_out[((long long)bag * C + c) * 2] = m; ml_out[((long long)bag * C + c) * 2 + 1] = l; }
        for (long long r0 = rbeg + tid; r0 < rend; r0 += 256 * UA) {
            float sv[UA];
#pragma unroll
            for (int u = 0; u < UA; ++u) {
                const long long r = r0 + 256 * u;
                sv[u] = A[(off0 + (r < rend ? r : rend - 1)) * (long long)C + c];
            }
#pragma unroll
            for (int u = 0; u < UA; ++u) {
                const long long r = r0 + 256 * u;
                if (r < rend) A[(off0 + r) * (long long)C + c] = expf(sv[u] - m) * il;
            }
        }
        float* pp = pred_part + (((long long)bag * nblk + blockIdx.x) * C) * C + c;
        if (!has_k) {
            for (int o = tid; o < C; o += 256) pp[(long long)o * C] = 0.f;
            continue;
        }
        f32x4 acc = {0.f, 0.f, 0.f, 0.f};
        const float* pb = part_B + (slot0 * C + c) * (long long)Kv;
        const float* pm = part_ml + (slot0 * C + c) * 2;
        for (long long t0 = tg; t0 < ntile; t0 += 16 * UB) {
            float wv[UB];
            f32x4 bv[UB];
#pragma unroll
            for (int u = 0; u < UB; ++u) {
                long long t = t0 + 16 * u;
                t = t < ntile ? t : ntile - 1;
                wv[u] = pm[t * C * 2];
                bv[u] = load4<VEC>(pb + t * C * (long long)Kv, kb + kq * 4, Kv);
            }
#pragma unroll
            for (int u = 0; u < UB; ++u) {
                if (t0 + 16 * u < ntile) {
                    const float w = expf(wv[u] - m);
#pragma unroll
                    for (int e = 0; e < 4; ++e) acc[e] = fmaf(w, bv[u][e], acc[e]);
                }
            }
        }
        *reinterpret_cast<f32x4*>(&s_acc[tg][kq * 4]) = acc;
        __syncthreads();
        if (wave == 0) {
            float b = 0.f;
#pragma unroll
            for (int g = 0; g < 16; ++g) b += s_acc[g][lane];
            b *= il;
            const int k = kb + lane;
            if (k < Kv) B[((long long)bag * C + c) * Kv + k] = b;
            for (int o = 0; o < C; ++o) {
                const float d = wave_sum(k < Kv ? fcc_w[((long long)o * C + c) * Kv + k] * b : 0.f);
                if (lane == 0) pp[o * C] = d;
            }
        }
        __syncthreads();
    }
}

__global__ void k_pred(const float* __restrict__ pred_part, const float* __restrict__ fcc_b,
                       float* __restrict__ pred, int C, int nblk, int n_bags) {
    const int i = blockIdx.x * blockDim.x + threadIdx.x;
    if (i >= n_bags * C) return;
    const int bag = i / C, o = i % C;
    float s = fcc_b[o];
    for (int j = 0; j < nblk; ++j)
        for (int c = 0; c < C; ++c) s += pred_part[(((long long)bag * nblk + j) * C + o) * C + c];
    pred[i] = s;
}

template <int VEC>
__global__ __launch_bounds__(256) void k_fc(const float* __restrict__ feats,
                                            const float* __restrict__ fc_w,
                                            const float* __restrict__ fc_b,
                                            float* __restrict__ classes, long long N, int K, int C,
                                            const int64_t* __restrict__ rowmap) {
    const int lane = threadIdx.x & 63;
    const long long wid = (long long)blockIdx.x * 4 + (threadIdx.x >> 6);
    const long long nw = (long long)gridDim.x * 4;
    for (long long r = wid; r < N; r += nw) {
        const float* x = feats + phys_row(rowmap, r) * K;
        for (int c = 0; c < C; ++c) {
            float acc = 0.f;
            for (int k0 = 0; k0 < K; k0 += 256) {
                const int k = k0 + lane * 4;
                const f32x4 xv = load4<VEC>(x, k, K);
                const f32x4 wv = load4<VEC>(fc_w + (long long)c * K, k, K);
#pragma unroll
                for (int e = 0; e < 4; ++e) acc = fmaf(xv[e], wv[e], acc);
            }
            acc = wave_sum(acc) + fc_b[c];
            if (lane == 0) classes[r * C + c] = acc;
        }
    }
}

struct WsLayout {
    size_t part_val, part_idx, qmax, qflag, part_ml, part_B, pred_part, wsplit, wf2, rowmax, off2, tile_pre, total;
    long long slots0, slots, nchunk_max;
};

struct Expt {
    int bits;
    int nw;
    int lds_pad;
    int logits_old;
    int no_hs, no_qmi, no_f2;
    int f2_abl, f2_grid, f3_dbg;
    int no_prologue_role;
    int mlp;
};
#ifdef DSMIL_EXPERIMENTS
const Expt& expt() {
    static const Expt e = [] {
        auto env = [](const char* name) { const char* v = getenv(name); return v ? atoi(v) : 0; };
        const char* m = getenv("DSMIL_MLP");
        return Expt{env("DSMIL_EXPT"), env("DSMIL_NW"), env("DSMIL_LDS_PAD"), env("DSMIL_LOGITS_OLD"), env("DSMIL_NO_HS"),
                    env("DSMIL_NO_QMI"), env("DSMIL_NO_F2"), env("DSMIL_F2_ABL"), env("DSMIL_F2_GRID"), env("DSMIL_F3_DBG"),
                    env("DSMIL_NO_PROLOGUE_ROLE"), !m ? 0 : !strcmp(m, "f32") ? 1 : !strcmp(m, "s9") ? 9 : 0};
    }();
    return e;
}
#else
constexpr Expt kNoExpt{};
constexpr const Expt& expt() { return kNoExpt; }
#endif

int mlp_mode() { return expt().mlp == 1 ? 0 : expt().mlp == 9 ? 9 : 6; }

int pick_nw(int n_bags, long long total_rows) {
    const int force = expt().nw;
    if (force == 8 || force == 4 || force == 1) return force;
    const long long tiles128 = total_rows / 128 + n_bags;
    return tiles128 >= 512 ? 4 : 1;
}

inline size_t f2_image_bytes(int K) { return (size_t)(2 * ((K + 31) / 32) + 8) * F2_CHUNK_F4 * 16 + F2_TRAILER_BYTES; }

WsLayout ws_layout(int n_bags, long long total_rows, long long max_rows, int K, int Kv, int C) {
    WsLayout w;
    const int BM = pick_nw(n_bags, total_rows) * 32;
    w.slots0 = total_rows / 32 + n_bags + 1;
    const int bms = BM > F2_BM ? F2_BM : BM;
    w.slots = total_rows / bms + n_bags + 1;
    if (w.slots < RS_MAX_WG + n_bags) w.slots = RS_MAX_WG + n_bags;
    w.nchunk_max = finish_blocks(max_rows, Kv);
    size_t o = 0;
    auto take = [&](size_t bytes) { size_t p = o; o = al(o + bytes); return p; };
    w.part_val = take((size_t)w.slots0 * C * sizeof(float));
    w.part_idx = take((size_t)w.slots0 * C * sizeof(long long));
    w.qmax = take((size_t)n_bags * C * QD * sizeof(float));
    w.qflag = take((size_t)n_bags * C * sizeof(int));
    w.part_ml = take((size_t)w.slots * C * 2 * sizeof(float));
    w.part_B = take((size_t)w.slots * C * Kv * sizeof(float));
    w.pred_part = take((size_t)n_bags * w.nchunk_max * C * C * sizeof(float));
    w.wsplit = take((size_t)(2 * ((K + 31) / 32) + 8) * S3_CHUNK_F4 * 16);
    w.wf2 = take(f2_image_bytes(K));
    w.rowmax = take((size_t)total_rows * sizeof(float));
    w.off2 = take(2 * sizeof(int64_t));
    w.tile_pre = take((size_t)2 * (n_bags + 1) * sizeof(int));
    w.total = o;
    return w;
}

int device_cus() {
    static std::atomic<int> cus[64];
    int dev = 0;
    if (hipGetDevice(&dev) != hipSuccess || dev < 0 || dev >= 64) return 0;
    int v = cus[dev].load(std::memory_order_relaxed);
    if (v <= 0) {
        if (hipDeviceGetAttribute(&v, hipDeviceAttributeMultiprocessorCount, dev) != hipSuccess) return 0;
        cus[dev].store(v, std::memory_order_relaxed);
    }
    return v;
}

std::atomic<int> g_inline_query{1};
std::atomic<int> g_use_f2{2};
std::atomic<int> g_persistent_grid{256};
std::atomic<int> g_logits_form{1};
bool several_streams_recently(hipStream_t st) {
    static std::atomic<uintptr_t> ring[4];
    static std::atomic<unsigned> pos{0};
    const uintptr_t me = (uintptr_t)st + 1;
    bool several = false;
    for (auto& r : ring) {
        const uintptr_t v = r.load(std::memory_order_relaxed);
        several |= (v != 0 && v != me);
    }
    ring[pos.fetch_add(1, std::memory_order_relaxed) & 3].store(me, std::memory_order_relaxed);
    return several;
}
constexpr int PIPE_R0 = 512;
constexpr int PIPE_QT = 256;
int persistent_grid(int cap) {
    int g = g_persistent_grid.load(std::memory_order_relaxed);
    if (g <= 0) g = 256;
    return g < cap ? g : cap;
}

typedef dsmil_agg_call Call;
typedef dsmil_agg_route Route;

int aligned_bits(const void* feats, const void* vals, const dsmil_agg_params* p, const void* crit_rows) {
    const uintptr_t all = (uintptr_t)feats | (uintptr_t)vals | (uintptr_t)p->q0_w | (uintptr_t)p->fc_w |
                          (uintptr_t)(p->nonlinear ? p->q2_w : p->q0_w);
    const uintptr_t w = (uintptr_t)p->q0_w | (uintptr_t)p->fc_w, r = (uintptr_t)crit_rows | (uintptr_t)p->q0_w;
    return (all % 16 == 0 ? 1 : 0) | (w % 16 == 0 ? 2 : 0) | (r % 16 == 0 ? 4 : 0);
}
bool call_v4(const Call& c) { return c.bf16 || ((c.K % 4 == 0) && (c.Kv % 4 == 0) && (c.aligned & 1)); }
bool call_w4(const Call& c) { return (c.K % 4 == 0) && (c.aligned & 2); }
bool stream_ok(const Call& c) { return !c.classes_given && !expt().logits_old && (c.bf16 ? (c.K % 8 == 0) : call_v4(c)); }
bool pipe_shape(const Call& c) {
    return c.bf16 && stream_ok(c) && c.K == 512 && c.C <= 2 && pick_nw(c.n_bags, c.total_rows) == 4 && c.phase == 0 &&
           !c.row_map && c.max_rows < 0x7fffffffLL;
}

Route pick_route(const Call& c) {
    const Expt& ex = expt();
    const int K = c.K, C = c.C, NW = pick_nw(c.n_bags, c.total_rows), BM = NW * 32;
    const bool bf16 = c.bf16, v4 = call_v4(c), w4 = call_w4(c), sok = stream_ok(c), same_vals = !c.vals_separate;
    const int batch_form = g_use_f2.load(std::memory_order_relaxed), logits_form = g_logits_form.load(std::memory_order_relaxed);
    Route r{};
    r.nw = NW;
    const bool lpipe = pipe_shape(c) && (logits_form == 2 || (logits_form == 1 && c.several_streams));
    r.r0 = lpipe ? PIPE_R0 : (NW == 1 && sok && c.phase != 2) ? 32 : R0;
    if (c.phase == 2) r.logits = DSMIL_LOGITS_NONE;
    else if (c.classes_given) { r.logits = DSMIL_LOGITS_GIVEN; r.logits_vec = 1; }
    else if (sok) { r.logits = lpipe ? DSMIL_LOGITS_PIPE : DSMIL_LOGITS_STREAM; r.logits_cp = C >= 2 ? 2 : 1; }
    else { r.logits = DSMIL_LOGITS_ARGMAX; r.logits_vec = (bf16 ? w4 : v4) ? 4 : 1; }
    r.prologue = c.prologue_job && r.logits == DSMIL_LOGITS_STREAM && !bf16;
    const bool use_hs = !bf16 && NW == 1 && v4 && !ex.no_hs && mlp_mode() == 6 && !(ex.bits & 8);
    const bool use_f2 = !bf16 && NW == 4 && v4 && !ex.no_f2 && mlp_mode() == 6 && sok && c.phase == 0 && same_vals &&
                        (K % 128 == 0) && K <= 16 * F2_MAXSTEPS && batch_form;
    r.rowmax = use_f2;
    r.ragged = NW == 4 && sok && c.phase == 0 && (long long)c.max_rows * c.n_bags != (long long)c.total_rows &&
               c.total_rows / 32 + c.n_bags < 0x7fffffffLL;
    r.tile_attend = bf16 ? RS_BM : F3_BM;
    r.tile_logits = r.r0;
    const long long hs_wgs = ((c.max_rows + HS_BM - 1) / HS_BM + C) * (long long)c.n_bags;
    auto hs_inline_fits = [&] { return hs_wgs <= 2LL * (c.cus > 0 ? c.cus : device_cus()); };
    r.qmax_threads = QMAX_T;
    if (c.phase == 1) { r.qmax = DSMIL_QMAX_SHARD1; r.qmax_vec = v4 ? 4 : 1; return r; }
    if (use_hs && sok && c.phase == 0 && !ex.no_qmi && g_inline_query.load(std::memory_order_relaxed) && hs_inline_fits())
        r.qmax = DSMIL_QMAX_INLINE, r.qmax_threads = 0;
    else if (c.phase == 2) { r.qmax = DSMIL_QMAX_SHARD2; r.qmax_vec = (K % 4 == 0) && (c.aligned & 4) ? 4 : 1; }
    else if (bf16) { r.qmax = DSMIL_QMAX_LAUNCH; r.qmax_vec = w4 ? 4 : 1; r.qmax_threads = lpipe ? PIPE_QT : QMAX_T; }
    else { r.qmax = DSMIL_QMAX_LAUNCH; r.qmax_vec = v4 ? 4 : 1; }
    const int mode = (NW == 8) ? 0 : mlp_mode();
    if (use_f2) r.image = c.packed_f2 ? DSMIL_IMAGE_F2_CALLER : DSMIL_IMAGE_F2_CUT;
    else if (!bf16 && mode) r.image = c.packed_split ? DSMIL_IMAGE_SPLIT_CALLER : DSMIL_IMAGE_SPLIT_CUT;
    else r.image = bf16 ? DSMIL_IMAGE_BF16 : DSMIL_IMAGE_NONE;
    const bool bf16_dma = bf16 && NW == 4 && !(ex.bits & 256);
    const bool bf16_res = bf16_dma && (K == 512 || K == 256) && c.Kv == K && same_vals && C <= 2 && !(ex.bits & 512);
    const bool use_f3 = use_f2 && c.nonlinear && C <= 2 && batch_form == 2;
    auto tiled = [&](int kind, int nw, int vec, int np, int xe = 0, int tu = 8) {
        r.attend = kind; r.attend_nw = nw; r.attend_vec = vec; r.attend_np = np; r.attend_xe = xe; r.attend_tu = tu;
    };
    const int vec = v4 ? 4 : 1;
    if (use_f3) r.attend = DSMIL_ATTEND_F3;
    else if (use_f2) r.attend = DSMIL_ATTEND_F2;
    else if (bf16_res) r.attend = DSMIL_ATTEND_BF16_RES;
    else if (bf16_dma) r.attend = DSMIL_ATTEND_BF16_DMA;
    else if (bf16) tiled(DSMIL_ATTEND_BF16_RING, NW == 4 ? 4 : 1, 0, 0);
    else if (mode == 9) tiled(DSMIL_ATTEND_SPLIT, NW == 4 ? 4 : 1, vec, 9);
    else if (mode == 6 && NW == 4 && v4 && (ex.bits & 16)) tiled(DSMIL_ATTEND_SPLIT, 4, 4, 6, 0, 16);
    else if (mode == 6 && NW == 4 && v4 && (ex.bits & 32)) tiled(DSMIL_ATTEND_SPLIT, 4, 4, 6, 0, 32);
    else if (mode == 6 && (NW == 4 || NW == 1) && v4 && (ex.bits & 8)) tiled(DSMIL_ATTEND_SPLIT, NW, 4, 6, 1);
    else if (mode == 6 && NW == 4) tiled(DSMIL_ATTEND_SPLIT, 4, vec, 6);
    else if (use_hs) r.attend = DSMIL_ATTEND_HS;
    else if (mode == 6) tiled(DSMIL_ATTEND_SPLIT, 1, vec, 6);
    else if (NW == 8) tiled(DSMIL_ATTEND_F32, 8, 4, 0);
    else tiled(DSMIL_ATTEND_F32, NW == 4 ? 4 : 1, vec, 0);
    r.ragged_attend = r.ragged && (use_f3 || bf16_res);
    if (ex.bits & 64) return r;
    const int a_bm = r.attend == DSMIL_ATTEND_F3 ? F3_BM : r.attend == DSMIL_ATTEND_F2 ? F2_BM : r.attend == DSMIL_ATTEND_HS ? HS_BM :
                     r.attend == DSMIL_ATTEND_BF16_RES ? RS_BM : BM;
    if (c.Kv % 4 == 0 && lpipe && r.attend == DSMIL_ATTEND_BF16_RES) { r.finish = DSMIL_FINISH_LEAN; r.finish_rows = RS_BM; }
    else if (c.Kv % 4 == 0) { r.finish = DSMIL_FINISH_VEC4; r.finish_rows = a_bm; }
    else { r.finish = DSMIL_FINISH_SCALAR; r.finish_rows = BM; }
    r.pred = c.phase == 0 && !c.skip_pred;
    return r;
}

template <typename Kern, typename... Args>
int launch_attend_kernel(Kern kern, dim3 grid, int threads, size_t lds, hipStream_t st, const Args&... args) {
    if (!dsmil_lds::allow((const void*)kern, (int)lds)) return DSMIL_E_LAUNCH;
    const int slot = dsmil_prof::begin(dsmil_prof::CH_ATTEND, st);
    hipLaunchKernelGGL(kern, grid, dim3(threads), lds, st, args...);
    dsmil_prof::end(dsmil_prof::CH_ATTEND, slot, st);
    return hipGetLastError() == hipSuccess ? DSMIL_OK : DSMIL_E_LAUNCH;
}

struct Attended { int rc, per, T; };

template <typename Kern, typename... Lead>
Attended launch_runs(Kern kern, int threads, int lds, int bm, int cap, int ragged_T, const AttendArgs& a, long long max_rows,
                     long long total_rows, int n_bags, hipStream_t st, const Lead&... lead) {
    const int cus = persistent_grid(cap);
    const long long T = a.tile_pre ? ragged_T : (max_rows + bm - 1) / bm;
    const long long n_items = a.tile_pre ? total_rows / bm + n_bags : T * n_bags;
    if (n_items > 0x7fffffffLL) return {DSMIL_E_UNSUPPORTED, 0, 0};
    const long long per = (n_items + cus - 1) / cus;
    const unsigned grid = (unsigned)((n_items + per - 1) / per);
    return {launch_attend_kernel(kern, dim3(grid), threads, (size_t)lds, st, a, lead..., (int)T, (int)n_items, (int)per), (int)per, (int)T};
}

Attended launch_f3(const AttendArgs& a, const float* rowmax, long long max_rows, long long total_rows, int n_bags, hipStream_t st) {
    void (*fn)(AttendArgs, const float*, int, int, int) = nullptr;
    const bool two = a.C == 2;
    switch (a.K / 32) {
        case 4: fn = two ? k_attend_f3<4, true> : k_attend_f3<4, false>; break;
        case 8: fn = two ? k_attend_f3<8, true> : k_attend_f3<8, false>; break;
        case 12: fn = two ? k_attend_f3<12, true> : k_attend_f3<12, false>; break;
        case 16: fn = two ? k_attend_f3<16, true> : k_attend_f3<16, false>; break;
        default: return {DSMIL_E_UNSUPPORTED, 0, 0};
    }
#ifdef DSMIL_EXPERIMENTS
#define F3_DBG(n) case n: fn = k_attend_f3<16, false, n>; break;
    if (a.K == 512 && a.C == 1) switch (expt().f3_dbg) { F3_DBG(1) F3_DBG(2) F3_DBG(3) F3_DBG(4) F3_DBG(5) default: break; }
#undef F3_DBG
#endif
    return launch_runs(fn, F3_THREADS, f3_lds_bytes(a.K), F3_BM, F3_MAX_WG, 0, a, max_rows, total_rows, n_bags, st, rowmax);
}

int launch_f2(const AttendArgs& a, const float* rowmax, long long max_rows, int n_bags, hipStream_t st) {
    void (*fn)(AttendArgs, const float*, int, int) = nullptr;
    switch (a.K / 32) {
        case 4: fn = k_attend_f2<4>; break;
        case 8: fn = k_attend_f2<8>; break;
        case 12: fn = k_attend_f2<12>; break;
        case 16: fn = k_attend_f2<16>; break;
        default: return DSMIL_E_UNSUPPORTED;
    }
#ifdef DSMIL_EXPERIMENTS
#define F2_ABL(n) case n: fn = k_attend_f2<16, n>; break;
    switch (a.K == 512 ? expt().f2_abl : 0) {
        F2_ABL(1) F2_ABL(2) F2_ABL(3) F2_ABL(4) F2_ABL(7) F2_ABL(8) F2_ABL(16) F2_ABL(31) F2_ABL(32) F2_ABL(64) F2_ABL(128) F2_ABL(192) F2_ABL(256)
        default: break;
    }
#undef F2_ABL
#endif
    const int tiles_per_bag = (int)((max_rows + F2_BM - 1) / F2_BM);
    const long long n_items = (long long)tiles_per_bag * n_bags;
    if (n_items > 0x7fffffffLL) return DSMIL_E_UNSUPPORTED;
    const int cus = expt().f2_grid > 0 ? expt().f2_grid : persistent_grid(1 << 20);
    const long long grid = n_items < cus ? n_items : cus;
    return launch_attend_kernel(fn, dim3((unsigned)grid), F2_THREADS, F2_LDS_BYTES, st, a, rowmax, tiles_per_bag, (int)n_items);
}

Attended launch_bf16_res(const AttendArgs& a, long long max_rows, long long total_rows, int n_bags, hipStream_t st) {
    void (*fn)(AttendArgs, int, int, int);
#define RES_FN(nch) (a.C == 2 ? (a.nonlinear ? k_attend_bf16_res<nch, true, true> : k_attend_bf16_res<nch, true, false>) \
                              : (a.nonlinear ? k_attend_bf16_res<nch, false, true> : k_attend_bf16_res<nch, false, false>))
    fn = a.K == 512 ? RES_FN(8) : RES_FN(4);
#undef RES_FN
#ifdef DSMIL_EXPERIMENTS
    if (a.K == 512 && a.C == 2 && a.nonlinear && (a.expt & 1024)) fn = k_attend_bf16_res<8, true, true, 1>;
    if (a.K == 512 && a.C == 2 && a.nonlinear && (a.expt & 2048)) fn = k_attend_bf16_res<8, true, true, 2>;
#endif
    return launch_runs(fn, RS_THREADS, RS_LDS_BYTES, RS_BM, RS_MAX_WG, 1, a, max_rows, total_rows, n_bags, st);
}

template <int NW, int VEC, int NP, bool XE = false, int TU = 8>
int launch_split(const AttendArgs& a, dim3 grid, hipStream_t st) {
    constexpr int BM = NW * 32;
    const size_t lds = (VEC == 4 ? (size_t)(3 * S3_CHUNK_F4 * 4 + 2 * BM * 32) * sizeof(float)
                                 : (size_t)(2 * S3_CHUNK_F4 * 4 + 2 * BM * LDK) * sizeof(float)) + (size_t)expt().lds_pad;
    return launch_attend_kernel(k_query_attend_split<NW, VEC, NP, XE, TU>, grid, NW * 64, lds, st, a);
}

Attended launch_attend(const Route& r, AttendArgs a, const float* rowmax, long long max_rows, long long total_rows, int n_bags,
                       hipStream_t st) {
    const int BM = r.attend_nw * 32, threads = r.attend_nw * 64;
    const dim3 grid((unsigned)((max_rows + BM - 1) / (BM ? BM : 1)), (unsigned)n_bags);
    const size_t lds_ring = (size_t)(2 * W_TILE + 2 * BM * LDK) * sizeof(float);
    const bool n4 = r.attend_nw == 4, vec4 = r.attend_vec == 4;
    auto plain = [](int rc) { return Attended{rc, 0, 0}; };
    switch (r.attend) {
        case DSMIL_ATTEND_F3: return launch_f3(a, rowmax, max_rows, total_rows, n_bags, st);
        case DSMIL_ATTEND_F2: return plain(launch_f2(a, rowmax, max_rows, n_bags, st));
        case DSMIL_ATTEND_BF16_RES:
        case DSMIL_ATTEND_BF16_DMA:
            a.wpk = a.wpk + (size_t)QD * ((a.K + 63) / 64 * 64) + QD * QD;
            if (r.attend == DSMIL_ATTEND_BF16_RES) return launch_bf16_res(a, max_rows, total_rows, n_bags, st);
            return plain(launch_attend_kernel(k_query_attend_bf16_dma<4>, dim3((unsigned)((max_rows + 127) / 128), (unsigned)n_bags), 256,
                                              (size_t)(2 * BD_WCHUNK_F4 + 3 * 128 * 8) * 16, st, a));
        case DSMIL_ATTEND_BF16_RING:
            return plain(n4 ? launch_attend_kernel(k_query_attend_bf16<4>, grid, threads, lds_ring, st, a)
                            : launch_attend_kernel(k_query_attend_bf16<1>, grid, threads, lds_ring, st, a));
        case DSMIL_ATTEND_SPLIT:
#ifdef DSMIL_EXPERIMENTS
            if (r.attend_np == 9) return plain(n4 ? (vec4 ? launch_split<4, 4, 9>(a, grid, st) : launch_split<4, 1, 9>(a, grid, st))
                                                  : (vec4 ? launch_split<1, 4, 9>(a, grid, st) : launch_split<1, 1, 9>(a, grid, st)));
            if (r.attend_tu == 16) return plain(launch_split<4, 4, 6, false, 16>(a, grid, st));
            if (r.attend_tu == 32) return plain(launch_split<4, 4, 6, false, 32>(a, grid, st));
            if (r.attend_xe) return plain(n4 ? launch_split<4, 4, 6, true>(a, grid, st) : launch_split<1, 4, 6, true>(a, grid, st));
#endif
            return plain(n4 ? (vec4 ? launch_split<4, 4, 6>(a, grid, st) : launch_split<4, 1, 6>(a, grid, st))
                            : (vec4 ? launch_split<1, 4, 6>(a, grid, st) : launch_split<1, 1, 6>(a, grid, st)));
        case DSMIL_ATTEND_HS:
            return plain(launch_attend_kernel(k_attend_hs<6>, dim3((unsigned)((max_rows + HS_BM - 1) / HS_BM + (a.qm_flag ? a.C : 0)), (unsigned)n_bags),
                                              HS_THREADS, (size_t)HS_LDS_BYTES + (size_t)expt().lds_pad, st, a));
        case DSMIL_ATTEND_F32:
#ifdef DSMIL_EXPERIMENTS
            if (r.attend_nw == 8) return plain(launch_attend_kernel(k_query_attend<8, 4>, grid, threads, lds_ring, st, a));
#endif
            return plain(n4 ? (vec4 ? launch_attend_kernel(k_query_attend<4, 4>, grid, threads, lds_ring, st, a)
                                    : launch_attend_kernel(k_query_attend<4, 1>, grid, threads, lds_ring, st, a))
                            : (vec4 ? launch_attend_kernel(k_query_attend<1, 4>, grid, threads, lds_ring, st, a)
                                    : launch_attend_kernel(k_query_attend<1, 1>, grid, threads, lds_ring, st, a)));
        default: return plain(DSMIL_E_INVALID);
    }
}

}

int dsmil_fc_forward_rows(const float* feats, int64_t total_rows, int32_t K, int32_t C, const float* fc_w,
                          const float* fc_b, float* classes, const int64_t* rowmap, void* stream) {
    if (!feats || !fc_w || !fc_b || !classes || total_rows <= 0 || K <= 0 || C <= 0) return DSMIL_E_INVALID;
    hipStream_t st = (hipStream_t)stream;
    long long blocks = (total_rows + 3) / 4;
    if (blocks > 4096) blocks = 4096;
    const bool v4 = (K % 4 == 0) && (((uintptr_t)feats | (uintptr_t)fc_w) % 16 == 0);
    auto go = [&](auto kern) { hipLaunchKernelGGL(kern, dim3((unsigned)blocks), dim3(256), 0, st, feats, fc_w, fc_b, classes, (long long)total_rows, K, C, rowmap); };
    if (v4) go(k_fc<4>); else go(k_fc<1>);
    return hipGetLastError() == hipSuccess ? DSMIL_OK : DSMIL_E_LAUNCH;
}

void dsmil_agg_forward_leftovers(void* ws, int32_t n_bags, int64_t total_rows, int32_t K, int32_t Kv, int32_t C,
                                 const float** qmax, const float** pred_part, int* pred_blocks) {
    const WsLayout L = ws_layout(n_bags, total_rows, total_rows, K, Kv, C);
    if (pred_part) *pred_part = (const float*)((char*)ws + L.pred_part);
    if (pred_blocks) *pred_blocks = (int)L.nchunk_max;
    if (qmax) *qmax = (const float*)((char*)ws + L.qmax);
}

extern "C" {

int dsmil_abi_version(void) { return DSMIL_ABI_VERSION; }

int dsmil_agg_mlp_form(void) { return mlp_mode(); }
int dsmil_agg_batch_form(int mode) {
    if (mode >= 0 && mode <= 2) return g_use_f2.exchange(mode);
    return g_use_f2.load();
}
int dsmil_agg_logits_form(int mode) {
    if (mode >= 0 && mode <= 2) return g_logits_form.exchange(mode);
    return g_logits_form.load();
}
int dsmil_agg_persistent_grid(int n) {
    if (n >= 1 && n <= 1024) return g_persistent_grid.exchange(n);
    return g_persistent_grid.load();
}
int dsmil_device_cus(void) { return device_cus(); }
int dsmil_agg_inline_query(int mode) {
    if (mode == 0 || mode == 1) return g_inline_query.exchange(mode);
    return g_inline_query.load();
}

const char* dsmil_strerror(int code) {
    switch (code) {
        case DSMIL_OK: return "ok";
        case DSMIL_E_INVALID: return "invalid argument";
        case DSMIL_E_UNSUPPORTED: return "unsupported shape or dtype";
        case DSMIL_E_WORKSPACE: return "workspace too small";
        case DSMIL_E_LAUNCH: return "kernel launch failed";
        case DSMIL_E_ALIGN: return "pointer not aligned";
        default: return "unknown error";
    }
}

int dsmil_agg_tile_rows(int32_t n_bags, int64_t total_rows) { return pick_nw(n_bags, total_rows) * 32; }

int dsmil_agg_forward_route(const dsmil_agg_call* call, dsmil_agg_route* route) {
    if (!call || !route) return DSMIL_E_INVALID;
    if (call->n_bags <= 0 || call->total_rows <= 0 || call->max_rows <= 0 || call->max_rows > call->total_rows) return DSMIL_E_INVALID;
    if (call->K <= 0 || call->Kv <= 0 || call->C <= 0) return DSMIL_E_INVALID;
    *route = pick_route(*call);
    return DSMIL_OK;
}

size_t dsmil_agg_workspace_bytes(int32_t n_bags, int64_t total_rows, int32_t K, int32_t Kv,
                                 int32_t C) {
    if (n_bags <= 0 || total_rows <= 0 || Kv <= 0 || C <= 0) return 0;
    return ws_layout(n_bags, total_rows, total_rows, K, Kv, C).total;
}

int dsmil_fc_forward(const float* feats, int64_t total_rows, int32_t K, int32_t C,
                     const float* fc_w, const float* fc_b, float* classes, void* stream) {
    return dsmil_fc_forward_rows(feats, total_rows, K, C, fc_w, fc_b, classes, nullptr, stream);
}

struct ShardCtl {
    int phase = 0;
    const float* crit_rows = nullptr;
    float* best_val = nullptr;
    float* ml_out = nullptr;
    bool skip_pred = false;
    const TrainPrologueJob* job = nullptr;
    const void* packed_f2 = nullptr;
};

static Call describe_call(const void* feats, const void* vals, int32_t n_bags, int64_t total_rows, int64_t max_rows,
                          const dsmil_agg_params* p, bool bf16, bool classes_given, const ShardCtl& sh, const void* packed_split,
                          const int64_t* rowmap) {
    Call c{};
    c.total_rows = total_rows; c.max_rows = max_rows; c.n_bags = n_bags;
    c.K = p->K; c.Kv = p->Kv; c.C = p->C; c.nonlinear = p->nonlinear;
    c.bf16 = bf16;
    c.aligned = aligned_bits(feats, vals, p, sh.crit_rows);
    c.classes_given = classes_given; c.vals_separate = vals != feats; c.row_map = rowmap != nullptr;
    c.packed_split = packed_split != nullptr; c.packed_f2 = sh.packed_f2 != nullptr;
    c.phase = sh.phase; c.skip_pred = sh.skip_pred; c.prologue_job = sh.job != nullptr;
    return c;
}

static int agg_forward_impl(const void* feats, const void* vals, const int64_t* offsets,
                            int32_t n_bags, int64_t total_rows, int64_t max_rows, const dsmil_agg_params* p,
                            const void* packed_bf16, bool bf16, const float* classes_in, float* classes_out,
                            float* A, float* B, float* pred, int64_t* idx, void* ws, size_t ws_bytes,
                            void* stream, const ShardCtl& sh = ShardCtl(), const void* packed_split = nullptr,
                            const int64_t* rowmap = nullptr) {
    if (!feats || !p || !ws) return DSMIL_E_INVALID;
    if (sh.phase == 0 && (!offsets || !A || !B || (!pred && !sh.skip_pred) || !idx)) return DSMIL_E_INVALID;
    if (sh.phase == 1 && (!classes_out || !idx || !sh.best_val)) return DSMIL_E_INVALID;
    if (sh.phase == 2 && (!A || !B || !sh.crit_rows || !sh.ml_out)) return DSMIL_E_INVALID;
    if (n_bags <= 0 || total_rows <= 0 || max_rows <= 0 || max_rows > total_rows) return DSMIL_E_INVALID;
    if (p->K <= 0 || p->Kv <= 0 || p->C <= 0) return DSMIL_E_INVALID;
    if (!p->q0_w || !p->q0_b || !p->fcc_w || !p->fcc_b) return DSMIL_E_INVALID;
    if (p->nonlinear && (!p->q2_w || !p->q2_b)) return DSMIL_E_INVALID;
    if (sh.phase != 2 && !classes_in && (!p->fc_w || !p->fc_b || !classes_out)) return DSMIL_E_INVALID;
    if (bf16 && !packed_bf16) return DSMIL_E_INVALID;
    if (n_bags > 65535) return DSMIL_E_UNSUPPORTED;
    if (!vals) vals = feats;
    if (vals == feats && p->Kv != p->K) return DSMIL_E_INVALID;
    if (((uintptr_t)ws % 256) || ((uintptr_t)p->q0_b % 16) || (p->nonlinear && ((uintptr_t)p->q2_b % 16)))
        return DSMIL_E_ALIGN;
    const int K = p->K, Kv = p->Kv, C = p->C;
    if (bf16 && ((K % 8) || (Kv % 4) || ((uintptr_t)feats % 16) || ((uintptr_t)vals % 8) ||
                 ((uintptr_t)packed_bf16 % 16)))
        return DSMIL_E_UNSUPPORTED;
    const WsLayout L = ws_layout(n_bags, total_rows, max_rows, K, Kv, C);
    if (ws_bytes < L.total) return DSMIL_E_WORKSPACE;
    hipStream_t st = (hipStream_t)stream;
    char* w8 = (char*)ws;
    if (sh.phase) {
        int64_t* off2 = (int64_t*)(w8 + L.off2);
        hipLaunchKernelGGL(k_set_offsets, dim3(1), dim3(1), 0, st, off2, (long long)total_rows);
        if (hipGetLastError() != hipSuccess) return DSMIL_E_LAUNCH;
        offsets = off2;
    }
    float* part_val = (float*)(w8 + L.part_val);
    long long* part_idx = (long long*)(w8 + L.part_idx);
    float* qmax = (float*)(w8 + L.qmax);
    float* part_ml = (float*)(w8 + L.part_ml);
    float* part_B = (float*)(w8 + L.part_B);
    float* pred_part = (float*)(w8 + L.pred_part);
    const float* f32 = (const float*)feats;
    const bf16_t* b16 = (const bf16_t*)feats;

    Call call = describe_call(feats, vals, n_bags, total_rows, max_rows, p, bf16, classes_in != nullptr, sh, packed_split, rowmap);
    if (pipe_shape(call)) call.several_streams = several_streams_recently(st);
    const Route r = pick_route(call);
    AttendArgs a{feats, vals, (const bf16_t*)packed_bf16, offsets, p->q0_w, p->q0_b, p->q2_w, p->q2_b, qmax, A,
                 part_ml, part_B, K, Kv, C, p->nonlinear, expt().bits, 0, rowmap};
    float* rowmax = r.rowmax ? (float*)(w8 + L.rowmax) : nullptr;
    int* qflag = r.qmax == DSMIL_QMAX_INLINE ? (int*)(w8 + L.qflag) : nullptr;
    int *tile_pre_a = nullptr, *tile_pre_l = nullptr;
    if (r.ragged) {
        tile_pre_a = (int*)(w8 + L.tile_pre);
        tile_pre_l = tile_pre_a + (n_bags + 1);
        hipLaunchKernelGGL(k_tile_prefix, dim3(1), dim3(1024), 0, st, offsets, n_bags, r.tile_attend, r.tile_logits, tile_pre_a, tile_pre_l);
        if (hipGetLastError() != hipSuccess) return DSMIL_E_LAUNCH;
    }
    {
        const dim3 grid = r.ragged ? dim3((unsigned)(total_rows / r.r0 + n_bags), 1u)
                                   : dim3((unsigned)((max_rows + r.r0 - 1) / r.r0), (unsigned)n_bags);
        auto argmax = [&](auto kern, auto* x) {
            hipLaunchKernelGGL(kern, grid, dim3(256), 0, st, x, offsets, p->fc_w, p->fc_b, classes_in, classes_out, part_val, part_idx, K, C, 0, rowmap);
        };
        auto pipe = [&](auto kern) {
            hipLaunchKernelGGL(kern, grid, dim3(256), 0, st, b16, offsets, p->fc_w, p->fc_b, classes_out, part_val, part_idx, 0, r.r0, tile_pre_l, n_bags);
        };
        auto strm = [&](auto kern, auto* x, int kstep) {
            const size_t ldsw = (size_t)r.logits_cp * (((K + kstep - 1) / kstep + 1) * kstep) * sizeof(float);
            const TrainPrologueJob job = r.prologue ? *sh.job : TrainPrologueJob{};
            const dim3 gridj(grid.x + (unsigned)job.blocks, grid.y);
            hipLaunchKernelGGL(kern, gridj, dim3(256), ldsw, st, x, offsets, p->fc_w, p->fc_b, classes_out, part_val, part_idx, K, C, 0, rowmap, r.r0, qflag, job, rowmax, tile_pre_l, n_bags);
        };
        const bool two = r.logits_cp == 2, vec4 = r.logits_vec == 4;
        switch (r.logits) {
            case DSMIL_LOGITS_GIVEN: argmax(k_logits_argmax<1, true, float>, f32); break;
            case DSMIL_LOGITS_PIPE: if (two) pipe(k_logits_pipe<2>); else pipe(k_logits_pipe<1>); break;
            case DSMIL_LOGITS_STREAM:
                if (bf16) { if (two) strm(k_logits_stream<2, bf16_t>, b16, 64); else strm(k_logits_stream<1, bf16_t>, b16, 64); }
                else { if (two) strm(k_logits_stream<2, float>, f32, 32); else strm(k_logits_stream<1, float>, f32, 32); }
                break;
            case DSMIL_LOGITS_ARGMAX:
                if (bf16) { if (vec4) argmax(k_logits_argmax<4, false, bf16_t>, b16); else argmax(k_logits_argmax<1, false, bf16_t>, b16); }
                else { if (vec4) argmax(k_logits_argmax<4, false, float>, f32); else argmax(k_logits_argmax<1, false, float>, f32); }
                break;
            default: break;
        }
        if (hipGetLastError() != hipSuccess) return DSMIL_E_LAUNCH;
    }
    if (r.qmax == DSMIL_QMAX_INLINE) {
        a.qm_flag = qflag; a.qm_part_val = part_val; a.qm_part_idx = part_idx; a.qm_idx = idx; a.qm_r0 = r.r0;
    } else {
        auto go = [&](auto kern, auto* x) {
            hipLaunchKernelGGL(kern, dim3((unsigned)n_bags, (unsigned)C), dim3(r.qmax_threads), 0, st, x, offsets, part_val, part_idx, p->q0_w, p->q0_b, p->q2_w, p->q2_b,
                               qmax, idx, K, C, p->nonlinear, 0, sh.phase, sh.best_val, sh.phase == 2 ? nullptr : rowmap, r.r0);
        };
        const float* x = sh.phase == 2 ? sh.crit_rows : f32;
        if (bf16 && !sh.phase) { if (r.qmax_vec == 4) go(k_qmax<4, bf16_t>, b16); else go(k_qmax<1, bf16_t>, b16); }
        else { if (r.qmax_vec == 4) go(k_qmax<4, float>, x); else go(k_qmax<1, float>, x); }
        if (hipGetLastError() != hipSuccess) return DSMIL_E_LAUNCH;
        if (sh.phase == 1) return DSMIL_OK;
    }
    switch (r.image) {
        case DSMIL_IMAGE_F2_CALLER: a.wpk = (const bf16_t*)sh.packed_f2; break;
        case DSMIL_IMAGE_SPLIT_CALLER: a.wpk = (const bf16_t*)packed_split; break;
        case DSMIL_IMAGE_F2_CUT:
        case DSMIL_IMAGE_SPLIT_CUT: {
            const float* w2 = p->nonlinear ? p->q2_w : nullptr;
            const int nks = 2 * ((K + 31) / 32);
            a.wpk = (const bf16_t*)(w8 + (r.image == DSMIL_IMAGE_F2_CUT ? L.wf2 : L.wsplit));
            if (r.image == DSMIL_IMAGE_F2_CUT) hipLaunchKernelGGL(k_pack_agg_f2, dim3(64), dim3(256), 0, st, p->q0_w, w2, (_Float16*)a.wpk, K, nks);
            else hipLaunchKernelGGL(k_pack_agg_split, dim3(64), dim3(256), 0, st, p->q0_w, w2, (bf16_t*)a.wpk, K, nks);
            if (hipGetLastError() != hipSuccess) return DSMIL_E_LAUNCH;
            break;
        }
        default: break;
    }
    if (r.ragged_attend) { a.tile_pre = tile_pre_a; a.n_bags = n_bags; }
    const Attended att = launch_attend(r, a, rowmax, max_rows, total_rows, n_bags, st);
    if (att.rc != DSMIL_OK) return att.rc;
    if (r.finish == DSMIL_FINISH_NONE) return DSMIL_OK;
    auto finish = [&](auto kern, int per, int T, const int* tile_pre) {
        hipLaunchKernelGGL(kern, dim3((unsigned)L.nchunk_max, (unsigned)n_bags), dim3(256), 0, st, offsets, part_ml, part_B, p->fcc_w, A, B, pred_part, Kv, C,
                           r.finish_rows, sh.ml_out, per, T, tile_pre);
    };
    if (r.finish == DSMIL_FINISH_LEAN) finish(k_finish<4, 2>, att.per, att.T, a.tile_pre);
    else if (r.finish == DSMIL_FINISH_VEC4) finish(k_finish<4>, att.per, att.T, a.tile_pre);
    else finish(k_finish<1>, 0, 0, nullptr);
    if (hipGetLastError() != hipSuccess) return DSMIL_E_LAUNCH;
    if (!r.pred) return DSMIL_OK;
    const int n = n_bags * C;
    hipLaunchKernelGGL(k_pred, dim3((unsigned)((n + 255) / 256)), dim3(256), 0, st, pred_part,
                       p->fcc_b, pred, C, (int)L.nchunk_max, n_bags);
    return hipGetLastError() == hipSuccess ? DSMIL_OK : DSMIL_E_LAUNCH;
}

int dsmil_agg_forward(const float* feats, const float* vals, const int64_t* offsets,
                      int32_t n_bags, int64_t total_rows, int64_t max_rows,
                      const dsmil_agg_params* p, const float* classes_in, float* classes_out,
                      float* A, float* B, float* pred, int64_t* idx, void* ws, size_t ws_bytes,
                      void* stream) {
    return agg_forward_impl(feats, vals, offsets, n_bags, total_rows, max_rows, p, nullptr, false, classes_in,
                            classes_out, A, B, pred, idx, ws, ws_bytes, stream);
}

size_t dsmil_agg_packed_split_bytes(int32_t K, int32_t nonlinear) {
    if (K <= 0) return 0;
    return (size_t)(2 * ((K + 31) / 32) + (nonlinear ? 8 : 0)) * S3_CHUNK_F4 * 16;
}

int dsmil_agg_pack_split(const float* q0_w, const float* q2_w, int32_t K, void* packed, void* stream) {
    if (!q0_w || !packed || K <= 0) return DSMIL_E_INVALID;
    if ((uintptr_t)packed % 16) return DSMIL_E_ALIGN;
    hipLaunchKernelGGL(k_pack_agg_split, dim3(64), dim3(256), 0, (hipStream_t)stream, q0_w, q2_w, (bf16_t*)packed, K,
                       2 * ((K + 31) / 32));
    return hipGetLastError() == hipSuccess ? DSMIL_OK : DSMIL_E_LAUNCH;
}

size_t dsmil_agg_packed_f2_bytes(int32_t K) { return K <= 0 ? 0 : f2_image_bytes(K); }

int dsmil_agg_pack_f2(const float* q0_w, const float* q2_w, int32_t K, void* packed, void* stream) {
    if (!q0_w || !packed || K <= 0) return DSMIL_E_INVALID;
    if ((uintptr_t)packed % 16) return DSMIL_E_ALIGN;
    hipLaunchKernelGGL(k_pack_agg_f2, dim3(64), dim3(256), 0, (hipStream_t)stream, q0_w, q2_w, (_Float16*)packed, K,
                       2 * ((K + 31) / 32));
    return hipGetLastError() == hipSuccess ? DSMIL_OK : DSMIL_E_LAUNCH;
}

size_t dsmil_value_packed_bytes(int32_t K, int32_t Kv) { return (K <= 0 || Kv <= 0) ? 0 : vp_image_bytes(K, Kv); }

int dsmil_value_pack(const float* v_w, int32_t K, int32_t Kv, void* packed, void* stream) {
    if (!v_w || !packed || K <= 0 || Kv <= 0) return DSMIL_E_INVALID;
    if ((uintptr_t)packed % 16) return DSMIL_E_ALIGN;
    hipLaunchKernelGGL(k_pack_value, dim3(256), dim3(256), 0, (hipStream_t)stream, v_w, (_Float16*)packed, K, Kv, vp_nks(K),
                       vp_ntp(Kv));
    return hipGetLastError() == hipSuccess ? DSMIL_OK : DSMIL_E_LAUNCH;
}

int dsmil_value_forward(const float* feats, int64_t rows, int32_t K, int32_t Kv, const float* v_w, const float* v_b,
                        const void* packed, const int64_t* row_map, float* V_out, void* ws, size_t ws_bytes, void* stream) {
    if (!feats || !v_w || !v_b || !V_out || rows <= 0 || K <= 0 || Kv <= 0) return DSMIL_E_INVALID;
    if (rows * (int64_t)Kv / 256 + 1 > 0x7fffffffLL) return DSMIL_E_UNSUPPORTED;
    hipStream_t st = (hipStream_t)stream;
    if (K > VP_MAX_K) {
        hipLaunchKernelGGL(k_value_proj_valu, dim3((unsigned)((rows * Kv + 255) / 256)), dim3(256), 0, st, feats, row_map, v_w,
                           v_b, V_out, (long long)rows, K, Kv);
        return hipGetLastError() == hipSuccess ? DSMIL_OK : DSMIL_E_LAUNCH;
    }
    if (!packed) {
        if (!ws) return DSMIL_E_INVALID;
        if ((uintptr_t)ws % 256) return DSMIL_E_ALIGN;
        if (ws_bytes < vp_image_bytes(K, Kv)) return DSMIL_E_WORKSPACE;
        const int rc = dsmil_value_pack(v_w, K, Kv, ws, stream);
        if (rc) return rc;
        packed = ws;
    }
    if ((uintptr_t)packed % 16) return DSMIL_E_ALIGN;
    const int nks = vp_nks(K);
    const int RG = K <= 512 ? 2 : 1;
    const int lds = nks * 4 * (32 * RG) * 16 + 32 * RG * 4;
    const int vec = (K % 4 == 0) && ((uintptr_t)feats % 16 == 0);
    const bool full = vec && K % 32 == 0;
    void (*fn)(const float*, const int64_t*, const f32x4*, const float*, float*, long long, int, int, int) =
        RG == 2 ? (full ? (nks == 32 ? k_value_proj<2, 32, true> : k_value_proj<2, 0, true>) : k_value_proj<2, 0, false>)
                : (full ? k_value_proj<1, 0, true> : k_value_proj<1, 0, false>);
    if (!dsmil_lds::allow((const void*)fn, lds)) return DSMIL_E_LAUNCH;
    const long long tiles = (rows + 32 * RG - 1) / (32 * RG);
    hipLaunchKernelGGL(fn, dim3((unsigned)tiles), dim3(VP_THREADS), lds, st, feats, row_map, (const f32x4*)packed, v_b, V_out,
                       (long long)rows, K, Kv, vec);
    return hipGetLastError() == hipSuccess ? DSMIL_OK : DSMIL_E_LAUNCH;
}

size_t dsmil_value_packed_bf16_bytes(int32_t K, int32_t Kv) { return (K <= 0 || Kv <= 0) ? 0 : vb_image_bytes(K, Kv); }

int dsmil_value_pack_bf16(const float* v_w, int32_t K, int32_t Kv, void* packed, void* stream) {
    if (!v_w || !packed || K <= 0 || Kv <= 0) return DSMIL_E_INVALID;
    if ((uintptr_t)packed % 16) return DSMIL_E_ALIGN;
    hipLaunchKernelGGL(k_pack_value_b16, dim3(256), dim3(256), 0, (hipStream_t)stream, v_w, (bf16_t*)packed, K, Kv, vp_nks(K),
                       vp_ntp(Kv));
    return hipGetLastError() == hipSuccess ? DSMIL_OK : DSMIL_E_LAUNCH;
}

size_t dsmil_value_workspace_bf16_bytes(int64_t rows, int32_t K, int32_t Kv) {
    if (rows <= 0 || K <= 0 || Kv <= 0 || K > VB_MAX_K) return 0;
    return vp_al(vb_image_bytes(K, Kv));
}

int dsmil_value_forward_bf16(const void* feats_bf16, int64_t rows, int32_t K, int32_t Kv, const float* v_w, const float* v_b,
                             const void* packed, void* V_out_bf16, void* ws, size_t ws_bytes, void* stream) {
    if (!feats_bf16 || !v_w || !v_b || !V_out_bf16 || rows <= 0 || K <= 0 || Kv <= 0) return DSMIL_E_INVALID;
    if ((K % 8) || (Kv % 4)) return DSMIL_E_UNSUPPORTED;
    if (((uintptr_t)feats_bf16 % 16) || ((uintptr_t)V_out_bf16 % 4)) return DSMIL_E_ALIGN;
    if (rows * (int64_t)Kv / 256 + 1 > 0x7fffffffLL) return DSMIL_E_UNSUPPORTED;
    hipStream_t st = (hipStream_t)stream;
    const bf16_t* x = (const bf16_t*)feats_bf16;
    bf16_t* V = (bf16_t*)V_out_bf16;
    if (K > VB_MAX_K) {
        hipLaunchKernelGGL(k_value_proj_b16_valu, dim3((unsigned)((rows * Kv + 255) / 256)), dim3(256), 0, st, x, v_w, v_b, V,
                           (long long)rows, K, Kv);
        return hipGetLastError() == hipSuccess ? DSMIL_OK : DSMIL_E_LAUNCH;
    }
    const bool cut = !packed;
    if (cut) {
        if (!ws) return DSMIL_E_INVALID;
        if ((uintptr_t)ws % 256) return DSMIL_E_ALIGN;
        if (ws_bytes < vb_image_bytes(K, Kv)) return DSMIL_E_WORKSPACE;
        packed = ws;
    }
    if ((uintptr_t)packed % 16) return DSMIL_E_ALIGN;
    if (cut) {
        const int rc = dsmil_value_pack_bf16(v_w, K, Kv, ws, stream);
        if (rc) return rc;
    }
    const int nks = vp_nks(K);
    const int lds = 2 * nks * VB_BM * 16;
    const bool full = K % 64 == 0;
    void (*fn)(const bf16_t*, const f32x4*, const float*, bf16_t*, long long, int, int) =
        full ? (nks == 32 ? k_value_proj_b16<32, true> : k_value_proj_b16<0, true>) : k_value_proj_b16<0, false>;
    if (!dsmil_lds::allow((const void*)fn, lds)) return DSMIL_E_LAUNCH;
    const long long tiles = (rows + VB_BM - 1) / VB_BM;
    hipLaunchKernelGGL(fn, dim3((unsigned)tiles), dim3(VP_THREADS), lds, st, x, (const f32x4*)packed, v_b, V, (long long)rows, K,
                       Kv);
    return hipGetLastError() == hipSuccess ? DSMIL_OK : DSMIL_E_LAUNCH;
}

int dsmil_agg_forward_ex(const float* feats, const float* vals, const int64_t* offsets,
                         int32_t n_bags, int64_t total_rows, int64_t max_rows,
                         const dsmil_agg_params* p, const dsmil_agg_opts* opts, const float* classes_in,
                         float* classes_out, float* A, float* B, float* pred, int64_t* idx, void* ws,
                         size_t ws_bytes, void* stream) {
    const void* packed_split = opts ? opts->packed_split : nullptr;
    const int64_t* row_map = opts ? opts->row_map : nullptr;
    if (packed_split && ((uintptr_t)packed_split % 16)) return DSMIL_E_ALIGN;
    ShardCtl sh;
    sh.packed_f2 = opts ? opts->packed_f2 : nullptr;
    if (sh.packed_f2 && ((uintptr_t)sh.packed_f2 % 16)) return DSMIL_E_ALIGN;
    return agg_forward_impl(feats, vals, offsets, n_bags, total_rows, max_rows, p, nullptr, false, classes_in,
// ... 112 lines not shown
```

### dsmil-wsi_amd/csrc/prof.h

```cpp
#pragma once
#include <hip/hip_runtime.h>

namespace dsmil_prof {
constexpr int CH_ATTEND = 0, CH_CONV = 1, NCH = 2;
int begin(int channel, hipStream_t st);
void end(int channel, int slot, hipStream_t st);
}
```

### include/dsmil_hip.h

```cpp
#ifndef DSMIL_HIP_H
#define DSMIL_HIP_H

#include <stddef.h>
#include <stdint.h>

#ifdef __cplusplus
extern "C" {
#endif

#define DSMIL_ABI_VERSION 6
#define DSMIL_Q_DIM 128

enum {
    DSMIL_OK = 0,
    DSMIL_E_INVALID = -1,
    DSMIL_E_UNSUPPORTED = -2,
    DSMIL_E_WORKSPACE = -3,
    DSMIL_E_LAUNCH = -4,
    DSMIL_E_ALIGN = -5
};

enum { DSMIL_F32 = 0, DSMIL_BF16 = 1 };

typedef struct dsmil_agg_params {
    const float* fc_w;
    const float* fc_b;
    const float* q0_w;
    const float* q0_b;
    const float* q2_w;
    const float* q2_b;
    const float* fcc_w;
    const float* fcc_b;
    int32_t K;
    int32_t Kv;
    int32_t C;
    int32_t nonlinear;
} dsmil_agg_params;


int dsmil_agg_forward(const float* feats, const float* vals, const int64_t* offsets,
                      int32_t n_bags, int64_t total_rows, int64_t max_rows,
                      const dsmil_agg_params* p, const float* classes_in, float* classes_out,
                      float* A, float* B, float* pred, int64_t* idx, void* ws, size_t ws_bytes,
                      void* stream);

size_t dsmil_agg_workspace_bytes(int32_t n_bags, int64_t total_rows, int32_t K, int32_t Kv,
                                 int32_t C);

size_t dsmil_agg_packed_bf16_bytes(int32_t K);
int dsmil_agg_pack_bf16(const float* q0_w, const float* q2_w, int32_t K, void* packed, void* stream);
int dsmil_agg_forward_bf16(const void* feats_bf16, const void* vals_bf16, const int64_t* offsets,
                           int32_t n_bags, int64_t total_rows, int64_t max_rows,
                           const dsmil_agg_params* p, const void* packed, const float* classes_in,
                           float* classes_out, float* A, float* B, float* pred, int64_t* idx, void* ws,
                           size_t ws_bytes, void* stream);

int dsmil_agg_shard_argmax(const float* feats, int64_t rows, const dsmil_agg_params* p,
                           float* classes_out, float* best_val, int64_t* best_idx, void* ws,
                           size_t ws_bytes, void* stream);
int dsmil_agg_shard_attend(const float* feats, const float* vals, int64_t rows,
                           const dsmil_agg_params* p, const float* crit_rows, float* A_unnorm,
                           float* ml, float* B_unnorm, void* ws, size_t ws_bytes, void* stream);

int dsmil_agg_mlp_form(void);

int dsmil_agg_inline_query(int mode);

int dsmil_agg_batch_form(int mode);

int dsmil_agg_persistent_grid(int n);

int dsmil_agg_logits_form(int mode);

int dsmil_device_cus(void);

typedef struct dsmil_agg_opts {
    const void* packed_split;
    const int64_t* row_map;
    const void* packed_f2;
} dsmil_agg_opts;
size_t dsmil_agg_packed_split_bytes(int32_t K, int32_t nonlinear);
int dsmil_agg_pack_split(const float* q0_w, const float* q2_w, int32_t K, void* packed, void* stream);
size_t dsmil_agg_packed_f2_bytes(int32_t K);
int dsmil_agg_pack_f2(const float* q0_w, const float* q2_w, int32_t K, void* packed, void* stream);
int dsmil_agg_forward_ex(const float* feats, const float* vals, const int64_t* offsets,
                         int32_t n_bags, int64_t total_rows, int64_t max_rows,
                         const dsmil_agg_params* p, const dsmil_agg_opts* opts, const float* classes_in,
                         float* classes_out, float* A, float* B, float* pred, int64_t* idx, void* ws,
                         size_t ws_bytes, void* stream);

int dsmil_agg_loss_head(const float* classes, const float* pred, const int64_t* idx, const float* label,
                        int32_t C, float* loss, float* max_pred, float* g_pred, float* g_max, void* stream);

typedef struct dsmil_bce_weights {
    const float* pos_weight;
    const float* weight;
} dsmil_bce_weights;
int dsmil_agg_loss_head_w(const float* classes, const float* pred, const int64_t* idx, const float* label, int32_t C,
                          float* loss, float* max_pred, float* g_pred, float* g_max, const dsmil_bce_weights* bw,
                          void* stream);

int dsmil_fc_forward(const float* feats, int64_t total_rows, int32_t K, int32_t C,
                     const float* fc_w, const float* fc_b, float* classes, void* stream);

typedef struct dsmil_agg_grads {
    float* fc_w;
    float* fc_b;
    float* q0_w;
    float* q0_b;
    float* q2_w;
    float* q2_b;
    float* fcc_w;
    float* fcc_b;
} dsmil_agg_grads;

size_t dsmil_agg_backward_workspace_bytes(int64_t N, int32_t K, int32_t Kv, int32_t C);
int dsmil_agg_backward_ex(const float* feats, const float* vals, int64_t N, const dsmil_agg_params* p,
                          const float* A, const float* B, const int64_t* idx, const float* g_classes,
                          const float* g_max, const float* g_pred, const float* g_A, const float* g_B,
                          const dsmil_agg_grads* g, float* g_vals, const int64_t* row_map, void* ws,
                          size_t ws_bytes, void* stream);
int dsmil_agg_backward(const float* feats, const float* vals, int64_t N, const dsmil_agg_params* p,
                       const float* A, const float* B, const int64_t* idx, const float* g_classes,
                       const float* g_pred, const float* g_A, const float* g_B,
                       const dsmil_agg_grads* g, float* g_vals, void* ws, size_t ws_bytes,
                       void* stream);
size_t dsmil_agg_backward_rows_workspace_bytes(int64_t N, int32_t K, int32_t Kv, int32_t C);
int dsmil_agg_backward_rows(const float* feats, const float* vals, int64_t N, const dsmil_agg_params* p,
                            const float* A, const float* B, const int64_t* idx, const float* g_classes,
                            const float* g_max, const float* g_pred, const float* g_A, const float* g_B,
                            const dsmil_agg_grads* g, float* g_vals, const int64_t* row_map, void* ws,
                            size_t ws_bytes, void* stream, float* g_feats);

size_t dsmil_agg_backward_bags_workspace_bytes(int32_t n_bags, int64_t total_rows, int32_t K, int32_t Kv, int32_t C);
int dsmil_agg_backward_bags(const float* feats, const float* vals, const int64_t* offsets, int32_t n_bags,
                            int64_t total_rows, int64_t max_rows, const dsmil_agg_params* p, const float* A,
                            const float* B, const int64_t* idx, const float* g_classes, const float* g_max,
                            const float* g_pred, const float* g_A, const float* g_B, const dsmil_agg_grads* g,
                            float* g_vals, const int64_t* row_map, void* ws, size_t ws_bytes, void* stream,
                            float* g_feats);
int dsmil_agg_loss_head_bags(const float* classes, const int64_t* offsets, const float* pred, const int64_t* idx,
                             const float* labels, int32_t n_bags, int32_t C, float* loss, float* max_pred,
                             float* g_pred, float* g_max, void* stream);
int dsmil_agg_loss_head_bags_w(const float* classes, const int64_t* offsets, const float* pred, const int64_t* idx,
                               const float* labels, int32_t n_bags, int32_t C, float* loss, float* max_pred,
                               float* g_pred, float* g_max, const dsmil_bce_weights* bw, void* stream);

size_t dsmil_agg_backward_bags_bf16_workspace_bytes(int32_t n_bags, int64_t total_rows, int32_t K, int32_t Kv, int32_t C);
int dsmil_agg_backward_bags_bf16(const void* feats_bf16, const void* vals_bf16, const int64_t* offsets, int32_t n_bags,
                                 int64_t total_rows, int64_t max_rows, const dsmil_agg_params* p, const float* A,
                                 const float* B, const int64_t* idx, const float* g_classes, const float* g_max,
                                 const float* g_pred, const float* g_A, const float* g_B, const dsmil_agg_grads* g,
                                 float* g_vals, void* ws, size_t ws_bytes, void* stream);

size_t dsmil_value_packed_bytes(int32_t K, int32_t Kv);
int dsmil_value_pack(const float* v_w, int32_t K, int32_t Kv, void* packed, void* stream);
size_t dsmil_value_workspace_bytes(int64_t rows, int32_t K, int32_t Kv);
int dsmil_value_forward(const float* feats, int64_t rows, int32_t K, int32_t Kv, const float* v_w, const float* v_b,
                        const void* packed, const int64_t* row_map, float* V_out, void* ws, size_t ws_bytes, void* stream);
int dsmil_value_backward(const float* feats, const float* V, const float* g_vals, int64_t rows, int32_t K, int32_t Kv,
                         const int64_t* row_map, float* g_v_w, float* g_v_b, void* ws, size_t ws_bytes, void* stream);
int dsmil_value_backward_rows(const float* feats, const float* V, const float* g_vals, int64_t rows, int32_t K, int32_t Kv,
                              const float* v_w, const void* packed, int32_t accumulate, float* g_feats, void* ws,
                              size_t ws_bytes, void* stream);

size_t dsmil_value_packed_bf16_bytes(int32_t K, int32_t Kv);
int dsmil_value_pack_bf16(const float* v_w, int32_t K, int32_t Kv, void* packed, void* stream);
size_t dsmil_value_workspace_bf16_bytes(int64_t rows, int32_t K, int32_t Kv);
int dsmil_value_forward_bf16(const void* feats_bf16, int64_t rows, int32_t K, int32_t Kv, const float* v_w, const float* v_b,
                             const void* packed, void* V_out_bf16, void* ws, size_t ws_bytes, void* stream);

size_t dsmil_value_backward_bf16_workspace_bytes(int64_t rows, int32_t K, int32_t Kv);
int dsmil_value_backward_bf16(const void* feats_bf16, const void* V_bf16, const float* g_vals, int64_t rows, int32_t K, int32_t Kv,
                              float* g_v_w, float* g_v_b, void* ws, size_t ws_bytes, void* stream);

#define DSMIL_ADAM_MAX_TENSORS 8
typedef struct dsmil_adam_state {
    float* const* exp_avg;
    float* const* exp_avg_sq;
    int64_t step;
    double lr, beta1, beta2, eps, weight_decay;
} dsmil_adam_state;
size_t dsmil_agg_train_step_workspace_bytes(int64_t N, int32_t K, int32_t C, int32_t nonlinear);
int dsmil_agg_train_step(const float* feats, int64_t N, const int64_t* row_map, const float* label,
                         const dsmil_agg_params* p, const dsmil_adam_state* opt, float* loss, void* ws,
                         size_t ws_bytes, void* stream);
int dsmil_adam_step(int32_t n_tensors, float* const* params, const float* const* grads, float* const* exp_avg,
                    float* const* exp_avg_sq, const int64_t* numel, int64_t step, double lr, double beta1,
                    double beta2, double eps, double weight_decay, void* stream);

size_t dsmil_agg_train_step_bags_workspace_bytes(int32_t n_bags, int64_t total_rows, int32_t K, int32_t C, int32_t nonlinear);
int dsmil_agg_train_step_bags(const float* feats, const int64_t* offsets, int32_t n_bags, int64_t total_rows, int64_t max_rows,
                              const int64_t* row_map, const float* labels, const dsmil_agg_params* p,
                              const dsmil_adam_state* opt, float* loss_each, float* loss, void* ws, size_t ws_bytes,
                              void* stream);
size_t dsmil_agg_train_step_bags_bf16_workspace_bytes(int32_t n_bags, int64_t total_rows, int32_t K, int32_t C,
                                                      int32_t nonlinear);
int dsmil_agg_train_step_bags_bf16(const void* feats_bf16, const int64_t* offsets, int32_t n_bags, int64_t total_rows,
                                   int64_t max_rows, const float* labels, const dsmil_agg_params* p,
                                   const dsmil_adam_state* opt, float* loss_each, float* loss, void* ws, size_t ws_bytes,
                                   void* stream);
int dsmil_agg_train_step_bags_w(const float* feats, const int64_t* offsets, int32_t n_bags, int64_t total_rows,
                                int64_t max_rows, const int64_t* row_map, const float* labels, const dsmil_agg_params* p,
                                const dsmil_adam_state* opt, float* loss_each, float* loss, void* ws, size_t ws_bytes,
                                const dsmil_bce_weights* bw, void* stream);
int dsmil_agg_train_step_bags_bf16_w(const void* feats_bf16, const int64_t* offsets, int32_t n_bags, int64_t total_rows,
                                     int64_t max_rows, const float* labels, const dsmil_agg_params* p,
                                     const dsmil_adam_state* opt, float* loss_each, float* loss, void* ws, size_t ws_bytes,
                                     const dsmil_bce_weights* bw, void* stream);

size_t dsmil_resnet18_packed_bytes(void);
int dsmil_resnet18_pack(const float* const* conv_w, float* packed, void* stream);
size_t dsmil_resnet18_workspace_bytes(int32_t B, int32_t H, int32_t W);
int dsmil_resnet18in_forward(const float* x_nchw, int32_t B, int32_t H, int32_t W,
                             const float* conv1_w, const float* packed, const float* fc_w,
                             const float* fc_b, int32_t C, float* feats, float* classes, void* ws,
                             size_t ws_bytes, void* stream);

int dsmil_resnet18in_forward_u8(const uint8_t* x_nhwc, int32_t B, int32_t H, int32_t W,
                                const float* conv1_w, const float* packed, const float* fc_w,
                                const float* fc_b, int32_t C, float* feats, float* classes, void* ws,
                                size_t ws_bytes, void* stream);

int32_t dsmil_resnet18_norm_channels(void);
int dsmil_resnet18bn_forward(const void* x, int32_t x_is_u8_nhwc, int32_t B, int32_t H, int32_t W,
                             const float* conv1_w, const float* packed, const float* bn_mean,
                             const float* bn_rstd, const float* fc_w, const float* fc_b, int32_t C,
                             float* feats, float* classes, void* ws, size_t ws_bytes, void* stream);

size_t dsmil_resnet_workspace_bytes(int32_t depth, int32_t B, int32_t H, int32_t W);
int32_t dsmil_resnet_feature_dim(int32_t depth);
int32_t dsmil_resnet_num_convs(int32_t depth);
int dsmil_resnet_mfma_forms(int32_t* wino_products, int32_t* direct_products);
int32_t dsmil_resnet_norm_channels(int32_t depth);
size_t dsmil_resnet_packed_bytes(int32_t depth);
int dsmil_resnet_pack(int32_t depth, const float* const* conv_w, float* packed, void* stream);
int dsmil_resnet_forward(int32_t depth, const void* x, int32_t x_is_u8_nhwc, int32_t B, int32_t H,
                         int32_t W, const float* conv1_w, const float* packed, const float* bn_mean,
                         const float* bn_rstd, const float* fc_w, const float* fc_b, int32_t C,
                         float* feats, float* classes, void* ws, size_t ws_bytes, void* stream);

int dsmil_resnet_pack_ex(int32_t depth, const float* const* conv_w, float* packed, int32_t precision, void* stream);
size_t dsmil_resnet_packed_bytes_ex(int32_t depth, int32_t precision);
int dsmil_resnet_forward_ex(int32_t depth, const void* x, int32_t x_is_u8_nhwc, int32_t B, int32_t H, int32_t W,
                            const float* conv1_w, const float* packed, const float* bn_mean, const float* bn_rstd,
                            const float* fc_w, const float* fc_b, int32_t C, float* feats, float* classes, void* ws,
                            size_t ws_bytes, int32_t precision, void* stream);

size_t dsmil_trunk16_positions(int32_t B, int32_t H, int32_t W);
int dsmil_trunk16_layout(const float* x_nhwc, void* out16, int32_t B, int32_t H, int32_t W, int32_t C, int32_t kind,
                         int32_t borders_only, void* stream);
size_t dsmil_trunk16_conv_workspace_bytes(int32_t Cin, int32_t Cout, int32_t ks);
int dsmil_trunk16_conv(const void* in16, const float* w_oihw, void* out16, int32_t B, int32_t Hi, int32_t Wi, int32_t Cin,
                       int32_t Cout, int32_t ks, int32_t stride, int32_t pad, int32_t kind, void* ws, size_t ws_bytes,
                       void* stream);
size_t dsmil_trunk16_norm_workspace_bytes(int32_t B, int32_t C);
int dsmil_trunk16_norm(const void* x16, const void* idn16, void* y16, int32_t B, int32_t H, int32_t W, int32_t C, int32_t relu,
                       int32_t kind, void* ws, size_t ws_bytes, void* stream);
int dsmil_trunk16_pool(const void* x16, const void* idn16, float* feats, int32_t B, int32_t H, int32_t W, int32_t C,
                       int32_t kind, void* ws, size_t ws_bytes, void* stream);
size_t dsmil_trunk16_workspace_bytes(int32_t depth, int32_t B, int32_t Hp, int32_t Wp);
int dsmil_trunk16_forward(int32_t depth, const float* x_nhwc, int32_t B, int32_t Hp, int32_t Wp, const float* const* conv_w,
                          float* feats, int32_t kind, void* ws, size_t ws_bytes, void* stream);

#define DSMIL_T32_W1 0
#define DSMIL_T32_UNIT 1
#define DSMIL_T32_S6 2
#define DSMIL_T32_OTHER 3
#define DSMIL_T32_PLAN_INTS 16
int dsmil_trunk32_conv_plan(int32_t Cin, int32_t Cout, int32_t ks, int32_t stride, int32_t pad, int32_t B, int32_t H, int32_t W,
                            int32_t norm, int32_t precision, int32_t* plan);
size_t dsmil_trunk32_conv_workspace_bytes(int32_t Cin, int32_t Cout, int32_t ks, int32_t stride, int32_t pad, int32_t B, int32_t H,
                                          int32_t W, int32_t precision);
int dsmil_trunk32_conv(const float* x, const float* w_oihw, const float* in_mean, const float* in_rstd, const float* bn_m,
                       const float* bn_r, float* y, float* mean, float* rstd, int32_t B, int32_t H, int32_t W, int32_t Cin,
                       int32_t Cout, int32_t ks, int32_t stride, int32_t pad, int32_t precision, void* ws, size_t ws_bytes,
                       void* stream);
size_t dsmil_trunk32_stem_workspace_bytes(int32_t B, int32_t H, int32_t W);
int dsmil_trunk32_stem(const void* x, int32_t x_is_u8_nhwc, const float* conv1_w, const float* bn_m, const float* bn_r,
                       float* pooled, float* mean, float* rstd, int32_t B, int32_t H, int32_t W, int32_t precision, void* ws,
                       size_t ws_bytes, void* stream);
int dsmil_trunk32_tail(int32_t kind, const float* y2, const float* m2, const float* r2, const float* idn, const float* md,
                       const float* rd, float* out, int32_t B, int32_t HW, int32_t C, int32_t precision, void* stream);

int dsmil_tile_stats(const uint8_t* tiles_nhwc, int32_t B, int32_t H, int32_t W, uint64_t* out, void* stream);

#define DSMIL_JPEG_MAX_QTABLES 256
#define DSMIL_JPEG_MAX_HTABLES 64
typedef struct dsmil_jpeg_image {
    int64_t ecs_begin, ecs_end;
    int32_t width, height;
    int32_t ncomp;
    int32_t hsamp, vsamp;
    int32_t restart_interval;
    int32_t qt[3];
    int32_t dc[3], ac[3];
    int32_t status;
} dsmil_jpeg_image;
size_t dsmil_jpeg_plan_bytes(int32_t n);
size_t dsmil_jpeg_workspace_bytes(int32_t n, int32_t height, int32_t width, int64_t data_bytes);
int dsmil_jpeg_parse(const uint8_t* data, const int64_t* offsets, int32_t n, void* plan);
int dsmil_jpeg_decode(const uint8_t* data, int64_t data_bytes, const void* plan, int32_t n, int32_t height, int32_t width,
                      uint8_t* out_nhwc, int32_t* status, void* ws, size_t ws_bytes, void* stream);

int64_t dsmil_csv_format_f32(const float* x, int64_t rows, int64_t cols, int64_t row_stride, int32_t decimals, char* out, int64_t cap);
int64_t dsmil_csv_parse_f32(const char* text, int64_t nbytes, int64_t cols, float* out, int64_t max_rows);
int64_t dsmil_read_files(const char* paths, const int64_t* path_off, int32_t n, uint8_t* out, int64_t cap, int64_t* sizes);

const char* dsmil_strerror(int code);
int dsmil_abi_version(void);
int dsmil_agg_tile_rows(int32_t n_bags, int64_t total_rows);

typedef struct dsmil_agg_call {
    int64_t total_rows, max_rows;
    int32_t n_bags, K, Kv, C, nonlinear;
    int32_t bf16;
    int32_t aligned;
    int32_t classes_given;
    int32_t vals_separate;
    int32_t row_map;
    int32_t packed_split;
    int32_t packed_f2;
    int32_t phase;
    int32_t skip_pred;
    int32_t prologue_job;
    int32_t several_streams;
    int32_t cus;
} dsmil_agg_call;

enum { DSMIL_LOGITS_NONE = 0, DSMIL_LOGITS_GIVEN, DSMIL_LOGITS_STREAM, DSMIL_LOGITS_PIPE, DSMIL_LOGITS_ARGMAX };
enum { DSMIL_QMAX_LAUNCH = 0, DSMIL_QMAX_INLINE, DSMIL_QMAX_SHARD1, DSMIL_QMAX_SHARD2 };
enum { DSMIL_IMAGE_NONE = 0, DSMIL_IMAGE_F2_CALLER, DSMIL_IMAGE_F2_CUT, DSMIL_IMAGE_SPLIT_CALLER, DSMIL_IMAGE_SPLIT_CUT,
       DSMIL_IMAGE_BF16 };
enum { DSMIL_ATTEND_NONE = 0, DSMIL_ATTEND_F3, DSMIL_ATTEND_F2, DSMIL_ATTEND_BF16_RES, DSMIL_ATTEND_BF16_DMA,
       DSMIL_ATTEND_BF16_RING, DSMIL_ATTEND_SPLIT, DSMIL_ATTEND_HS, DSMIL_ATTEND_F32 };
enum { DSMIL_FINISH_NONE = 0, DSMIL_FINISH_LEAN, DSMIL_FINISH_VEC4, DSMIL_FINISH_SCALAR };

typedef struct dsmil_agg_route {
    int32_t nw;
    int32_t r0;
    int32_t logits;
    int32_t logits_vec;
    int32_t logits_cp;
    int32_t prologue;
    int32_t rowmax;
    int32_t qmax;
    int32_t qmax_vec;
    int32_t qmax_threads;
    int32_t ragged;
    int32_t ragged_attend;
    int32_t tile_attend;
    int32_t tile_logits;
    int32_t image;
    int32_t attend;
    int32_t attend_nw;
    int32_t attend_vec;
    int32_t attend_np;
    int32_t attend_xe;
    int32_t attend_tu;
    int32_t finish;
    int32_t finish_rows;
    int32_t pred;
} dsmil_agg_route;

int dsmil_agg_forward_route(const dsmil_agg_call* call, dsmil_agg_route* route);

size_t dsmil_ntxent_workspace_bytes(int64_t n, int d);
int dsmil_ntxent_forward(const float* zis, const float* zjs, int64_t n, int d, float temperature, int cosine, float* loss,
                         float* lse, void* ws, size_t ws_bytes, void* stream);
int dsmil_ntxent_backward(const float* zis, const float* zjs, int64_t n, int d, float temperature, int cosine, const float* lse,
                          const float* g_loss, float* g_zis, float* g_zjs, void* ws, size_t ws_bytes, void* stream);

enum { DSMIL_SIMCLR_FLIP = 1, DSMIL_SIMCLR_JITTER = 2, DSMIL_SIMCLR_GREY = 4, DSMIL_SIMCLR_BLUR = 8 };
typedef struct dsmil_simclr_view {
    int32_t tile;
    int32_t i, j, h, w;
    int32_t flags;
    int32_t order;
    int32_t hue;
    float brightness, contrast, saturation;
    float sigma;
} dsmil_simclr_view;
size_t dsmil_simclr_views_workspace_bytes(int64_t n_views, int H, int W, int S);
int dsmil_simclr_views(const uint8_t* tiles_nhwc, int64_t n_tiles, int H, int W, const dsmil_simclr_view* views, int64_t n_views,
                       int S, float* out_nchw, uint8_t* out_nhwc, void* ws, size_t ws_bytes, void* stream);
int dsmil_simclr_views_host(const uint8_t* tiles_nhwc, int64_t n_tiles, int H, int W, const dsmil_simclr_view* views,
                            int64_t n_views, int S, float* out_nchw, uint8_t* out_nhwc, void* ws, size_t ws_bytes);

int dsmil_profile_enable(int on);
int dsmil_profile_collect(int channel, double* total_ms, int64_t* launches);

#ifdef __cplusplus
}
#endif
#endif
```

Baseline: 110,800 bags/s.

## Add paired-CU wide logits kernel and virtual-run partitioning for f3 attend

Adds a 'wide' logits kernel that runs on a small fixed set of large workgroups. With pair_cus mode enabled, logits and attend launches from different streams are chained through events so the two stages can share CUs across concurrent streams. The f3 attend kernel now splits work into a fixed number of virtual runs that are independent of grid size, and the finish kernel maps tiles back to run slots to match. The pairing path is off unless pair_cus is set (default 0), so by default the change mostly alters the f3 work partition and partial-slot layout. It adds complexity and a risk of host-side serialization through the mutex.

Result: slower. 108,900 bags/s (-1.7%).

```diff
diff --git a/dsmil-wsi_amd/_native.py b/dsmil-wsi_amd/_native.py
--- a/dsmil-wsi_amd/_native.py
+++ b/dsmil-wsi_amd/_native.py
@@ -28,17 +28,17 @@
 class AggCall(ctypes.Structure):
     _fields_ = [("total_rows", ctypes.c_int64), ("max_rows", ctypes.c_int64)] + [(n, ctypes.c_int32) for n in (
         "n_bags", "K", "Kv", "C", "nonlinear", "bf16", "aligned", "classes_given", "vals_separate", "row_map", "packed_split",
-        "packed_f2", "phase", "skip_pred", "prologue_job", "several_streams", "cus")]
+        "packed_f2", "phase", "skip_pred", "prologue_job", "several_streams", "cus", "no_pair")]
 
 
 class AggRoute(ctypes.Structure):
     _fields_ = [(n, ctypes.c_int32) for n in (
         "nw", "r0", "logits", "logits_vec", "logits_cp", "prologue", "rowmax", "qmax", "qmax_vec", "qmax_threads", "ragged",
         "ragged_attend", "tile_attend", "tile_logits", "image", "attend", "attend_nw", "attend_vec", "attend_np", "attend_xe",
-        "attend_tu", "finish", "finish_rows", "pred")]
-
-
-LOGITS = ("none", "given", "stream", "pipe", "argmax")
+        "attend_tu", "finish", "finish_rows", "pred", "pair", "attend_grid")]
+
+
+LOGITS = ("none", "given", "stream", "pipe", "argmax", "wide")
 QMAX = ("launch", "inline", "shard1", "shard2")
 IMAGE = ("none", "f2_caller", "f2_cut", "split_caller", "split_cut", "bf16")
 ATTEND = ("none", "f3", "f2", "bf16_res", "bf16_dma", "bf16_ring", "split", "hs", "f32")
@@ -75,6 +75,7 @@
     "dsmil_agg_batch_form": (ctypes.c_int, [ctypes.c_int]),
     "dsmil_agg_persistent_grid": (ctypes.c_int, [ctypes.c_int]),
     "dsmil_agg_logits_form": (ctypes.c_int, [ctypes.c_int]),
+    "dsmil_agg_pair_cus": (ctypes.c_int, [ctypes.c_int]),
     "dsmil_device_cus": (ctypes.c_int, []),
     "dsmil_agg_packed_f2_bytes": (ctypes.c_size_t, [ctypes.c_int32]),
     "dsmil_agg_pack_f2": (ctypes.c_int, [c_f32p, c_f32p, ctypes.c_int32, ctypes.c_void_p, ctypes.c_void_p]),
diff --git a/dsmil-wsi_amd/csrc/agg_f3.h b/dsmil-wsi_amd/csrc/agg_f3.h
--- a/dsmil-wsi_amd/csrc/agg_f3.h
+++ b/dsmil-wsi_amd/csrc/agg_f3.h
@@ -6,6 +6,7 @@
 constexpr int F3_BM = 32;
 constexpr int F3_THREADS = 256;
 constexpr int F3_MAX_WG = 1024;
+constexpr int F3_VRUNS = 768;
 constexpr int F3_HROW = 528;
 constexpr int F3_SCR = 1856;
 __host__ __device__ constexpr int f3_row_bytes(int K) { return 4 * K + 16; }
@@ -31,6 +32,15 @@
         f(std::integral_constant<int, B>{});
         f3_static_for<B + 1, E>(f);
     }
+}
+
+__device__ __forceinline__ unsigned f3_run_start(unsigned v, unsigned q, unsigned rem, unsigned runs) { return v * q + v * rem / runs; }
+__device__ __forceinline__ unsigned f3_run_of(unsigned i, unsigned n, unsigned q, unsigned rem, unsigned runs) {
+    unsigned v = (unsigned)((float)i * (float)runs / (float)n);
+    v = v < runs ? v : runs - 1;
+    while (f3_run_start(v, q, rem, runs) > i) --v;
+    while (v + 1 < runs && f3_run_start(v + 1, q, rem, runs) <= i) ++v;
+    return v;
 }
 
 struct F3Work {
@@ -68,7 +78,7 @@
 
 template <int NK1, bool TWO, int DBG = 0>
 __global__ __launch_bounds__(F3_THREADS, 1) void k_attend_f3(AttendArgs a, const float* __restrict__ rowmax, int tiles_per_bag,
-                                                             int n_items, int per_wg) {
+                                                             int n_items, int vruns) {
     static_assert(NK1 % 4 == 0 && NK1 >= 4 && NK1 <= 16, "K a multiple of 128 up to 512");
     constexpr int K = 32 * NK1, NKS = 2 * NK1, NG = NK1 / 2;
     constexpr int RB = f3_row_bytes(K), BUF = F3_BM * RB;
@@ -94,19 +104,30 @@
     const float* feats = reinterpret_cast<const float*>(a.feats);
     const float scale = 0.08838834764831845f;
 
-    F3Cur pos;
-    pos.item = (int)blockIdx.x * per_wg;
     if (a.tile_pre) {
         const int real = ((const __attribute__((address_space(4))) int*)(uintptr_t)a.tile_pre)[a.n_bags];
         n_items = n_items < real ? n_items : real;
-        if (pos.item >= n_items) return;
+    }
+    if (n_items <= 0) return;
+    const unsigned veff = (unsigned)(vruns < n_items ? vruns : n_items);
+    int vcur = (int)(blockIdx.x * veff / gridDim.x);
+    const unsigned v_last = (blockIdx.x + 1) * veff / gridDim.x;
+    if ((unsigned)vcur >= v_last) return;
+    const unsigned vq = (unsigned)n_items / veff, vrem = (unsigned)n_items % veff;
+    unsigned vacc = (unsigned)vcur * vrem % veff;
+    F3Cur pos;
+    pos.item = (int)f3_run_start((unsigned)vcur, vq, vrem, veff);
+    int vnext = pos.item;
+    auto run_step = [&]() { vacc += vrem; vnext += (int)vq + (vacc >= veff ? 1 : 0); vacc -= vacc >= veff ? veff : 0u; };
+    run_step();
+    if (a.tile_pre) {
         pos.b = tile_owner(a.tile_pre, a.n_bags, pos.item);
         pos.tile = pos.item - a.tile_pre[pos.b];
     } else {
         pos.b = pos.item / tiles_per_bag;
         pos.tile = pos.item - pos.b * tiles_per_bag;
     }
-    const int item_end = pos.item + per_wg < n_items ? pos.item + per_wg : n_items;
+    const int item_end = (int)f3_run_start(v_last, vq, vrem, veff);
     F3Work cur, nxt, nn;
     if (!f3_fetch(a, tiles_per_bag, item_end, pos, cur)) return;
 
@@ -208,6 +229,7 @@
     for (int c = 0; c < NG; ++c) fill(src_c, c);
     F3Cur pos_n = f3_next(pos, tiles_per_bag);
     bool has_next = f3_fetch(a, tiles_per_bag, item_end, pos_n, nxt);
+    int left = vnext - pos.item;
     const float* src_n = has_next ? row_src(nxt, sc_n, sinv_n) : src_c;
     if (!has_next) { nxt = cur; sc_n = sc_c; sinv_n = sinv_c; }
 #pragma unroll
@@ -416,10 +438,9 @@
                 for (int c = 0; c < NC; ++c) {
                     const float w = sPw[c * F3_BM + 8 * wave + j];
 #pragma unroll
-                    for (int e = 0; e < 8; ++e) {
-                        bacc[c][e] = fmaf((float)f0.v[e], w, bacc[c][e]);
-                        bacc[c][e] = fmaf((float)f1.v[e], w, bacc[c][e]);
-                    }
+                    for (int e = 0; e < 8; ++e) bacc[c][e] = fmaf((float)f0.v[e], w, bacc[c][e]);
+#pragma unroll
+                    for (int e = 0; e < 8; ++e) bacc[c][e] = fmaf((float)f1.v[e], w, bacc[c][e]);
                 }
             }
         }
@@ -431,8 +452,10 @@
                 for (int i = 0; i < 16; ++i) so[i] = stamps[i];
             }
         }
-        if (!has_next || nxt.bag != cur.bag) {
-            const long long slot = (long long)blockIdx.x + cur.bag;
+        --left;
+        const bool run_ends = has_next && left == 0;
+        if (!has_next || nxt.bag != cur.bag || run_ends) {
+            const long long slot = (long long)vcur + cur.bag;
             float* red = reinterpret_cast<float*>(sH);
             __syncthreads();
             if (lane < K / 8) {
@@ -461,6 +484,7 @@
                 }
             }
             reset_acc();
+            if (run_ends) { const int at = vnext; ++vcur; run_step(); left = vnext - at; }
         }
         STAMP(13);
         if constexpr (DBG >= 1) {
diff --git a/dsmil-wsi_amd/csrc/agg_fwd.hip b/dsmil-wsi_amd/csrc/agg_fwd.hip
--- a/dsmil-wsi_amd/csrc/agg_fwd.hip
+++ b/dsmil-wsi_amd/csrc/agg_fwd.hip
@@ -6,6 +6,7 @@
 #include <stdlib.h>
 #include <string.h>
 #include <atomic>
+#include <mutex>
 #include "dsmil_hip.h"
 #include "prof.h"
 
@@ -425,6 +426,147 @@
     }
 }
 
+constexpr int WIDE_CUS = 64;
+constexpr int WIDE_THREADS = 1024;
+constexpr int WIDE_LDS = 96 * 1024;
+template <int CP>
+__global__ __launch_bounds__(WIDE_THREADS) void k_logits_wide(
+    const float* __restrict__ feats, const int64_t* __restrict__ offsets, const float* __restrict__ fc_w,
+    const float* __restrict__ fc_b, float* __restrict__ classes_out, float* __restrict__ part_val,
+    long long* __restrict__ part_idx, int K, const int64_t* __restrict__ rowmap, float* __restrict__ rowmax,
+    int tiles_per_bag, int n_tiles, int per_wave) {
+    constexpr int SEG = 32, SETN = 4;
+    extern __shared__ __attribute__((aligned(16))) float s_w[];
+    const int tid = threadIdx.x, lane = tid & 63;
+    const int wave = __builtin_amdgcn_readfirstlane(tid >> 6);
+    const int j = lane & 7, rr = lane >> 3;
+    const int nseg = (K + SEG - 1) / SEG, Kpad = (nseg + 1) * SEG;
+    const int npair = (nseg + 2 * SETN - 1) / (2 * SETN);
+    for (int i = tid; i < CP * Kpad; i += WIDE_THREADS) {
+        const int cc = i / Kpad, k = i - cc * Kpad;
+        s_w[i] = k < K ? fc_w[(long long)cc * K + k] : 0.f;
+    }
+    __syncthreads();
+    int t = ((int)blockIdx.x * (WIDE_THREADS / 64) + wave) * per_wave;
+    const int t_end = t + per_wave < n_tiles ? t + per_wave : n_tiles;
+    if (t >= t_end) return;
+    const float b0 = fc_b[0], b1 = fc_b[CP - 1];
+    typedef StreamVec<float> SV;
+    SV va[SETN], vb[SETN];
+    auto load_set = [&](SV (&v)[SETN], const float* x, int s0) {
+#pragma unroll
+        for (int u = 0; u < SETN; ++u) {
+            int k = (s0 + u) * SEG + j * 4;
+            k = k < K ? k : K - 4;
+            v[u].load(x + k);
+        }
+    };
+    float a0 = 0.f, a1 = 0.f, xm = 0.f;
+    auto consume = [&](const SV (&v)[SETN], int s0) {
+        if (rowmax) {
+#pragma unroll
+            for (int u = 0; u < SETN; ++u)
+#pragma unroll
+                for (int e = 0; e < 4; ++e) xm = fmaxf(xm, fabsf(v[u].at(e)));
+        }
+#pragma unroll
+        for (int u = 0; u < SETN; ++u) {
+            const int ks = (s0 + u < nseg ? s0 + u : nseg) * SEG + j * 4;
+            const f32x4 w0 = *reinterpret_cast<const f32x4*>(s_w + ks);
+#pragma unroll
+            for (int e = 0; e < 4; ++e) a0 = fmaf(v[u].at(e), w0[e], a0);
+            if constexpr (CP == 2) {
+                const f32x4 w1 = *reinterpret_cast<const f32x4*>(s_w + Kpad + ks);
+#pragma unroll
+                for (int e = 0; e < 4; ++e) a1 = fmaf(v[u].at(e), w1[e], a1);
+            }
+        }
+    };
+    int bag = t / tiles_per_bag, tile = t - bag * tiles_per_bag;
+    long long off0 = offsets[bag];
+    const int Nb = (int)(offsets[bag + 1] - off0);
+    auto groups_of = [&](int tl) { const int left = (Nb - tl * R0 + 7) >> 3; return left < R0 / 8 ? left : R0 / 8; };
+    auto row_of = [&](int tl, int g) { const int r = tl * R0 + g * 8 + rr; return r < Nb ? r : Nb - 1; };
+    auto ptr_of = [&](long long o, int r) { return feats + phys_row(rowmap, o + r) * (long long)K; };
+    int g = 0, ng = groups_of(tile);
+    int r = row_of(tile, 0);
+    const float* x = ptr_of(off0, r);
+    float bv0 = -INFINITY, bv1 = -INFINITY;
+    long long bi0 = 0x7fffffffffffffffLL, bi1 = 0x7fffffffffffffffLL;
+    load_set(va, x, 0);
+    for (;;) {
+        const bool tile_done = g + 1 == ng, last = tile_done && t + 1 == t_end;
+        int bag_n = bag, tile_n = tile, g_n = g + 1;
+        long long off0_n = off0;
+        if (last) g_n = g;
+        else if (tile_done) {
+            g_n = 0;
+            if (++tile_n == tiles_per_bag) { tile_n = 0; ++bag_n; off0_n = offsets[bag_n]; }
+        }
+        const int r_n = row_of(tile_n, g_n);
+        const float* x_n = ptr_of(off0_n, r_n);
+#pragma unroll 1
+        for (int p = 0; p < npair; ++p) {
+            const bool more = p + 1 < npair;
+            load_set(vb, x, (2 * p + 1) * SETN);
+            __builtin_amdgcn_sched_barrier(0);
+            consume(va, 2 * p * SETN);
+            __builtin_amdgcn_sched_barrier(0);
+            load_set(va, more ? x : x_n, more ? (2 * p + 2) * SETN : 0);
+            __builtin_amdgcn_sched_barrier(0);
+            consume(vb, (2 * p + 1) * SETN);
+            __builtin_amdgcn_sched_barrier(0);
+        }
+#pragma unroll
+        for (int m = 1; m < 8; m <<= 1) {
+            a0 += __shfl_xor(a0, m, 64);
+            if constexpr (CP == 2) a1 += __shfl_xor(a1, m, 64);
+        }
+        a0 += b0;
+        a1 += b1;
+        const bool mine = j == 0 && tile * R0 + g * 8 + rr < Nb;
+        if (rowmax) {
+#pragma unroll
+            for (int m = 1; m < 8; m <<= 1) xm = fmaxf(xm, __shfl_xor(xm, m, 64));
+            if (mine) rowmax[off0 + r] = xm;
+        }
+        if (mine) {
+            float* o = classes_out + (off0 + r) * (long long)CP;
+            o[0] = a0;
+            if constexpr (CP == 2) o[1] = a1;
+        }
+        if (better(a0, r, bv0, bi0)) { bv0 = a0; bi0 = r; }
+        if (CP == 2 && better(a1, r, bv1, bi1)) { bv1 = a1; bi1 = r; }
+        a0 = 0.f; a1 = 0.f; xm = 0.f;
+        if (tile_done) {
+#pragma unroll
+            for (int m = 8; m < 64; m <<= 1) {
+                const float ov0 = __shfl_xor(bv0, m, 64);
+                const long long oi0 = __shfl_xor(bi0, m, 64);
+                if (better(ov0, oi0, bv0, bi0)) { bv0 = ov0; bi0 = oi0; }
+                if constexpr (CP == 2) {
+                    const float ov1 = __shfl_xor(bv1, m, 64);
+                    const long long oi1 = __shfl_xor(bi1, m, 64);
+                    if (better(ov1, oi1, bv1, bi1)) { bv1 = ov1; bi1 = oi1; }
+                }
+            }
+            if (lane == 0) {
+                const long long slot = off0 / R0 + bag + tile;
+                part_val[slot * CP] = bv0;
+                part_idx[slot * CP] = bi0;
+                if constexpr (CP == 2) { part_val[slot * CP + 1] = bv1; part_idx[slot * CP + 1] = bi1; }
+            }
+            bv0 = bv1 = -INFINITY;
+            bi0 = bi1 = 0x7fffffffffffffffLL;
+            if (last) break;
+            ++t;
+            ng = groups_of(tile_n);
+        }
+        bag = bag_n; tile = tile_n; g = g_n; off0 = off0_n;
+        r = r_n; x = x_n;
+    }
+}
+
 template <int VEC, typename T = float, bool PRE = false>
 __device__ __forceinline__ void qmax_block(
     const T* __restrict__ feats, const int64_t* __restrict__ offsets,
@@ -1053,13 +1195,20 @@
     const int64_t* __restrict__ offsets, const float* __restrict__ part_ml,
     const float* __restrict__ part_B, const float* __restrict__ fcc_w,
     float* __restrict__ A, float* __restrict__ B, float* __restrict__ pred_part, int Kv, int C, int BM,
-    float* __restrict__ ml_out = nullptr, int seg_per = 0, int seg_T = 0, const int* __restrict__ tile_pre = nullptr) {
+    float* __restrict__ ml_out = nullptr, int seg_per = 0, int seg_T = 0, const int* __restrict__ tile_pre = nullptr,
+    int seg_V = 0, int seg_n = 0) {
     const int bag = blockIdx.y, nblk = gridDim.x;
     const long long off0 = offsets[bag];
     const long long Nb = offsets[bag + 1] - off0;
     long long slot0 = off0 / BM + bag;
     long long ntile = (Nb + BM - 1) / BM;
-    if (seg_per > 0 && ntile > 0) {
+    if (seg_V > 0 && ntile > 0) {
+        const unsigned n = (unsigned)(tile_pre ? tile_pre[gridDim.y] : seg_n), runs = (unsigned)seg_V < n ? (unsigned)seg_V : n;
+        const unsigned it0 = (unsigned)(tile_pre ? tile_pre[bag] : bag * seg_T), q = n / runs, rem = n % runs;
+        const long long v_lo = f3_run_of(it0, n, q, rem, runs), v_hi = f3_run_of(it0 + (unsigned)ntile - 1, n, q, rem, runs);
+        slot0 = v_lo + bag;
+        ntile = v_hi - v_lo + 1;
+    } else if (seg_per > 0 && ntile > 0) {
         const long long it0 = tile_pre ? (long long)tile_pre[bag] : (long long)bag * seg_T, g_lo = it0 / seg_per, g_hi = (it0 + ntile - 1) / seg_per;
         slot0 = g_lo + bag;
         ntile = g_hi - g_lo + 1;
@@ -1207,6 +1356,8 @@
     int f2_abl, f2_grid, f3_dbg;
     int no_prologue_role;
     int mlp;
+    int pair_cus;
+    int f3_vruns;
 };
 #ifdef DSMIL_EXPERIMENTS
 const Expt& expt() {
@@ -1215,7 +1366,7 @@
         const char* m = getenv("DSMIL_MLP");
         return Expt{env("DSMIL_EXPT"), env("DSMIL_NW"), env("DSMIL_LDS_PAD"), env("DSMIL_LOGITS_OLD"), env("DSMIL_NO_HS"),
                     env("DSMIL_NO_QMI"), env("DSMIL_NO_F2"), env("DSMIL_F2_ABL"), env("DSMIL_F2_GRID"), env("DSMIL_F3_DBG"),
-                    env("DSMIL_NO_PROLOGUE_ROLE"), !m ? 0 : !strcmp(m, "f32") ? 1 : !strcmp(m, "s9") ? 9 : 0};
+                    env("DSMIL_NO_PROLOGUE_ROLE"), !m ? 0 : !strcmp(m, "f32") ? 1 : !strcmp(m, "s9") ? 9 : 0, env("DSMIL_PAIR_CUS"), env("DSMIL_F3_VRUNS")};
     }();
     return e;
 }
@@ -1289,6 +1440,35 @@
     ring[pos.fetch_add(1, std::memory_order_relaxed) & 3].store(me, std::memory_order_relaxed);
     return several;
 }
+std::atomic<int> g_pair_cus{0};
+struct PairChain {
+    static constexpr int RING = 16;
+    std::mutex mu;
+    hipEvent_t ev[RING] = {};
+    unsigned pos = 0;
+    hipEvent_t last[2] = {nullptr, nullptr};
+    hipEvent_t enter(int kind, hipStream_t st) {
+        hipEvent_t& e = ev[pos++ % RING];
+        if (!e && hipEventCreateWithFlags(&e, hipEventDisableTiming) != hipSuccess) { e = nullptr; return nullptr; }
+        if (last[kind] && hipStreamWaitEvent(st, last[kind], 0) != hipSuccess) return nullptr;
+        return e;
+    }
+    bool leave(int kind, hipEvent_t e, hipStream_t st) {
+        if (hipEventRecord(e, st) != hipSuccess) return false;
+        last[kind] = e;
+        return true;
+    }
+    void release() {
+        std::lock_guard<std::mutex> lock(mu);
+        for (auto& e : ev) if (e) { (void)hipEventDestroy(e); e = nullptr; }
+        last[0] = last[1] = nullptr;
+    }
+};
+PairChain g_pair_chain[64];
+PairChain* pair_chain() {
+    int dev = 0;
+    return (hipGetDevice(&dev) == hipSuccess && dev >= 0 && dev < 64) ? &g_pair_chain[dev] : nullptr;
+}
 constexpr int PIPE_R0 = 512;
 constexpr int PIPE_QT = 256;
 int persistent_grid(int cap) {
@@ -1312,6 +1492,12 @@
 bool pipe_shape(const Call& c) {
     return c.bf16 && stream_ok(c) && c.K == 512 && c.C <= 2 && pick_nw(c.n_bags, c.total_rows) == 4 && c.phase == 0 &&
            !c.row_map && c.max_rows < 0x7fffffffLL;
+}
+
+bool wide_shape(const Call& c) {
+    const long long T = (c.max_rows + R0 - 1) / R0;
+    return !c.bf16 && stream_ok(c) && c.C <= 2 && pick_nw(c.n_bags, c.total_rows) == 4 && c.phase == 0 && !c.prologue_job &&
+           (long long)c.max_rows * c.n_bags == (long long)c.total_rows && c.max_rows < 0x7fffffffLL && T * c.n_bags < 0x7fffffffLL;
 }
 
 Route pick_route(const Call& c) {
@@ -1335,6 +1521,12 @@
     r.ragged = NW == 4 && sok && c.phase == 0 && (long long)c.max_rows * c.n_bags != (long long)c.total_rows &&
                c.total_rows / 32 + c.n_bags < 0x7fffffffLL;
     r.tile_attend = bf16 ? RS_BM : F3_BM;
+    const int pair_mode = g_pair_cus.load(std::memory_order_relaxed);
+    if (use_f2 && c.nonlinear && C <= 2 && batch_form == 2 && wide_shape(c) && !c.no_pair &&
+        (pair_mode == 2 || (pair_mode == 1 && c.several_streams))) {
+        const int cus = c.cus > 0 ? c.cus : device_cus(), S = ex.pair_cus > 0 ? ex.pair_cus : WIDE_CUS;
+        if (cus > S) { r.pair = S; r.attend_grid = cus - S; r.logits = DSMIL_LOGITS_WIDE; }
+    }
     r.tile_logits = r.r0;
     const long long hs_wgs = ((c.max_rows + HS_BM - 1) / HS_BM + C) * (long long)c.n_bags;
     auto hs_inline_fits = [&] { return hs_wgs <= 2LL * (c.cus > 0 ? c.cus : device_cus()); };
@@ -1356,7 +1548,7 @@
         r.attend = kind; r.attend_nw = nw; r.attend_vec = vec; r.attend_np = np; r.attend_xe = xe; r.attend_tu = tu;
     };
     const int vec = v4 ? 4 : 1;
-    if (use_f3) r.attend = DSMIL_ATTEND_F3;
+    if (use_f3) { r.attend = DSMIL_ATTEND_F3; if (!r.pair) r.attend_grid = persistent_grid(F3_MAX_WG); }
     else if (use_f2) r.attend = DSMIL_ATTEND_F2;
     else if (bf16_res) r.attend = DSMIL_ATTEND_BF16_RES;
     else if (bf16_dma) r.attend = DSMIL_ATTEND_BF16_DMA;
@@ -1390,7 +1582,7 @@
     return hipGetLastError() == hipSuccess ? DSMIL_OK : DSMIL_E_LAUNCH;
 }
 
-struct Attended { int rc, per, T; };
+struct Attended { int rc, per, T, V, n; };
 
 template <typename Kern, typename... Lead>
 Attended launch_runs(Kern kern, int threads, int lds, int bm, int cap, int ragged_T, const AttendArgs& a, long long max_rows,
@@ -1398,13 +1590,13 @@
     const int cus = persistent_grid(cap);
     const long long T = a.tile_pre ? ragged_T : (max_rows + bm - 1) / bm;
     const long long n_items = a.tile_pre ? total_rows / bm + n_bags : T * n_bags;
-    if (n_items > 0x7fffffffLL) return {DSMIL_E_UNSUPPORTED, 0, 0};
+    if (n_items > 0x7fffffffLL) return {DSMIL_E_UNSUPPORTED, 0, 0, 0, 0};
     const long long per = (n_items + cus - 1) / cus;
     const unsigned grid = (unsigned)((n_items + per - 1) / per);
-    return {launch_attend_kernel(kern, dim3(grid), threads, (size_t)lds, st, a, lead..., (int)T, (int)n_items, (int)per), (int)per, (int)T};
-}
-
-Attended launch_f3(const AttendArgs& a, const float* rowmax, long long max_rows, long long total_rows, int n_bags, hipStream_t st) {
+    return {launch_attend_kernel(kern, dim3(grid), threads, (size_t)lds, st, a, lead..., (int)T, (int)n_items, (int)per), (int)per, (int)T, 0, 0};
+}
+
+Attended launch_f3(const AttendArgs& a, const float* rowmax, long long max_rows, long long total_rows, int n_bags, int wgs, hipStream_t st) {
     void (*fn)(AttendArgs, const float*, int, int, int) = nullptr;
     const bool two = a.C == 2;
     switch (a.K / 32) {
@@ -1419,7 +1611,14 @@
     if (a.K == 512 && a.C == 1) switch (expt().f3_dbg) { F3_DBG(1) F3_DBG(2) F3_DBG(3) F3_DBG(4) F3_DBG(5) default: break; }
 #undef F3_DBG
 #endif
-    return launch_runs(fn, F3_THREADS, f3_lds_bytes(a.K), F3_BM, F3_MAX_WG, 0, a, max_rows, total_rows, n_bags, st, rowmax);
+    const long long T = a.tile_pre ? 0 : (max_rows + F3_BM - 1) / F3_BM;
+    const long long n_items = a.tile_pre ? total_rows / F3_BM + n_bags : T * n_bags;
+    if (n_items > 0x7fffffffLL || wgs < 1) return {DSMIL_E_UNSUPPORTED, 0, 0, 0, 0};
+    if (!a.tile_pre && max_rows * n_bags != total_rows) return {DSMIL_E_UNSUPPORTED, 0, 0, 0, 0};
+    const unsigned grid = (unsigned)(wgs < F3_MAX_WG ? wgs : F3_MAX_WG);
+    const int V = expt().f3_vruns > 0 && expt().f3_vruns <= F3_MAX_WG ? expt().f3_vruns : F3_VRUNS;
+    return {launch_attend_kernel(fn, dim3(grid), F3_THREADS, (size_t)f3_lds_bytes(a.K), st, a, rowmax, (int)T, (int)n_items, V),
+            0, (int)T, V, (int)n_items};
 }
 
 int launch_f2(const AttendArgs& a, const float* rowmax, long long max_rows, int n_bags, hipStream_t st) {
@@ -1474,9 +1673,9 @@
     const dim3 grid((unsigned)((max_rows + BM - 1) / (BM ? BM : 1)), (unsigned)n_bags);
     const size_t lds_ring = (size_t)(2 * W_TILE + 2 * BM * LDK) * sizeof(float);
     const bool n4 = r.attend_nw == 4, vec4 = r.attend_vec == 4;
-    auto plain = [](int rc) { return Attended{rc, 0, 0}; };
+    auto plain = [](int rc) { return Attended{rc, 0, 0, 0, 0}; };
     switch (r.attend) {
-        case DSMIL_ATTEND_F3: return launch_f3(a, rowmax, max_rows, total_rows, n_bags, st);
+        case DSMIL_ATTEND_F3: return launch_f3(a, rowmax, max_rows, total_rows, n_bags, r.attend_grid, st);
         case DSMIL_ATTEND_F2: return plain(launch_f2(a, rowmax, max_rows, n_bags, st));
         case DSMIL_ATTEND_BF16_RES:
         case DSMIL_ATTEND_BF16_DMA:
@@ -1546,6 +1745,12 @@
 int dsmil_agg_logits_form(int mode) {
     if (mode >= 0 && mode <= 2) return g_logits_form.exchange(mode);
     return g_logits_form.load();
+}
+int dsmil_agg_pair_cus(int mode) {
+    if (mode < 0 || mode > 2) return g_pair_cus.load();
+    const int prev = g_pair_cus.exchange(mode);
+    if (mode == 0) for (auto& c : g_pair_chain) c.release();
+    return prev;
 }
 int dsmil_agg_persistent_grid(int n) {
     if (n >= 1 && n <= 1024) return g_persistent_grid.exchange(n);
@@ -1659,8 +1864,14 @@
     const bf16_t* b16 = (const bf16_t*)feats;
 
     Call call = describe_call(feats, vals, n_bags, total_rows, max_rows, p, bf16, classes_in != nullptr, sh, packed_split, rowmap);
-    if (pipe_shape(call)) call.several_streams = several_streams_recently(st);
+    if (pipe_shape(call) || wide_shape(call)) call.several_streams = several_streams_recently(st);
+    if (wide_shape(call) && g_pair_cus.load(std::memory_order_relaxed)) {
+        hipStreamCaptureStatus cap = hipStreamCaptureStatusNone;
+        if (hipStreamIsCapturing(st, &cap) != hipSuccess || cap != hipStreamCaptureStatusNone) call.no_pair = 1;
+    }
     const Route r = pick_route(call);
+    PairChain* chain = r.pair ? pair_chain() : nullptr;
+    if (r.pair && !chain) return DSMIL_E_LAUNCH;
     AttendArgs a{feats, vals, (const bf16_t*)packed_bf16, offsets, p->q0_w, p->q0_b, p->q2_w, p->q2_b, qmax, A,
                  part_ml, part_B, K, Kv, C, p->nonlinear, expt().bits, 0, rowmap};
     float* rowmax = r.rowmax ? (float*)(w8 + L.rowmax) : nullptr;
@@ -1687,8 +1898,21 @@
             const dim3 gridj(grid.x + (unsigned)job.blocks, grid.y);
             hipLaunchKernelGGL(kern, gridj, dim3(256), ldsw, st, x, offsets, p->fc_w, p->fc_b, classes_out, part_val, part_idx, K, C, 0, rowmap, r.r0, qflag, job, rowmax, tile_pre_l, n_bags);
         };
+        auto wide = [&](auto kern) {
+            if (!dsmil_lds::allow((const void*)kern, WIDE_LDS)) return false;
+            const int T = (int)((max_rows + R0 - 1) / R0), n_tiles = T * n_bags, waves = r.pair * (WIDE_THREADS / 64);
+            std::lock_guard<std::mutex> lock(chain->mu);
+            hipEvent_t e = chain->enter(0, st);
+            if (!e) return false;
+            const int slot = dsmil_prof::begin(dsmil_prof::CH_LOGITS, st);
+            hipLaunchKernelGGL(kern, dim3((unsigned)r.pair), dim3(WIDE_THREADS), WIDE_LDS, st, f32, offsets, p->fc_w, p->fc_b, classes_out, part_val, part_idx,
+                               K, rowmap, rowmax, T, n_tiles, (n_tiles + waves - 1) / waves);
+            dsmil_prof::end(dsmil_prof::CH_LOGITS, slot, st);
+            return chain->leave(0, e, st);
+        };
         const bool two = r.logits_cp == 2, vec4 = r.logits_vec == 4;
         switch (r.logits) {
+            case DSMIL_LOGITS_WIDE: if (!(two ? wide(k_logits_wide<2>) : wide(k_logits_wide<1>))) return DSMIL_E_LAUNCH; break;
             case DSMIL_LOGITS_GIVEN: argmax(k_logits_argmax<1, true, float>, f32); break;
             case DSMIL_LOGITS_PIPE: if (two) pipe(k_logits_pipe<2>); else pipe(k_logits_pipe<1>); break;
             case DSMIL_LOGITS_STREAM:
@@ -1732,12 +1956,19 @@
         default: break;
     }
     if (r.ragged_attend) { a.tile_pre = tile_pre_a; a.n_bags = n_bags; }
-    const Attended att = launch_attend(r, a, rowmax, max_rows, total_rows, n_bags, st);
+    Attended att;
+    if (r.pair) {
+        std::lock_guard<std::mutex> lock(chain->mu);
+        hipEvent_t e = chain->enter(1, st);
+        if (!e) return DSMIL_E_LAUNCH;
+        att = launch_attend(r, a, rowmax, max_rows, total_rows, n_bags, st);
+        if (att.rc == DSMIL_OK && !chain->leave(1, e, st)) return DSMIL_E_LAUNCH;
+    } else att = launch_attend(r, a, rowmax, max_rows, total_rows, n_bags, st);
     if (att.rc != DSMIL_OK) return att.rc;
     if (r.finish == DSMIL_FINISH_NONE) return DSMIL_OK;
     auto finish = [&](auto kern, int per, int T, const int* tile_pre) {
         hipLaunchKernelGGL(kern, dim3((unsigned)L.nchunk_max, (unsigned)n_bags), dim3(256), 0, st, offsets, part_ml, part_B, p->fcc_w, A, B, pred_part, Kv, C,
-                           r.finish_rows, sh.ml_out, per, T, tile_pre);
+                           r.finish_rows, sh.ml_out, per, T, tile_pre, att.V, att.n);
     };
     if (r.finish == DSMIL_FINISH_LEAN) finish(k_finish<4, 2>, att.per, att.T, a.tile_pre);
     else if (r.finish == DSMIL_FINISH_VEC4) finish(k_finish<4>, att.per, att.T, a.tile_pre);
diff --git a/dsmil-wsi_amd/csrc/prof.h b/dsmil-wsi_amd/csrc/prof.h
--- a/dsmil-wsi_amd/csrc/prof.h
+++ b/dsmil-wsi_amd/csrc/prof.h
@@ -2,7 +2,7 @@
 #include <hip/hip_runtime.h>
 
 namespace dsmil_prof {
-constexpr int CH_ATTEND = 0, CH_CONV = 1, NCH = 2;
+constexpr int CH_ATTEND = 0, CH_CONV = 1, CH_LOGITS = 2, NCH = 3;
 int begin(int channel, hipStream_t st);
 void end(int channel, int slot, hipStream_t st);
 }
diff --git a/include/dsmil_hip.h b/include/dsmil_hip.h
--- a/include/dsmil_hip.h
+++ b/include/dsmil_hip.h
@@ -71,6 +71,8 @@
 int dsmil_agg_persistent_grid(int n);
 
 int dsmil_agg_logits_form(int mode);
+
+int dsmil_agg_pair_cus(int mode);
 
 int dsmil_device_cus(void);
 
@@ -326,9 +328,10 @@
     int32_t prologue_job;
     int32_t several_streams;
     int32_t cus;
+    int32_t no_pair;
 } dsmil_agg_call;
 
-enum { DSMIL_LOGITS_NONE = 0, DSMIL_LOGITS_GIVEN, DSMIL_LOGITS_STREAM, DSMIL_LOGITS_PIPE, DSMIL_LOGITS_ARGMAX };
+enum { DSMIL_LOGITS_NONE = 0, DSMIL_LOGITS_GIVEN, DSMIL_LOGITS_STREAM, DSMIL_LOGITS_PIPE, DSMIL_LOGITS_ARGMAX, DSMIL_LOGITS_WIDE };
 enum { DSMIL_QMAX_LAUNCH = 0, DSMIL_QMAX_INLINE, DSMIL_QMAX_SHARD1, DSMIL_QMAX_SHARD2 };
 enum { DSMIL_IMAGE_NONE = 0, DSMIL_IMAGE_F2_CALLER, DSMIL_IMAGE_F2_CUT, DSMIL_IMAGE_SPLIT_CALLER, DSMIL_IMAGE_SPLIT_CUT,
        DSMIL_IMAGE_BF16 };
@@ -361,6 +364,8 @@
     int32_t finish;
     int32_t finish_rows;
     int32_t pred;
+    int32_t pair;
+    int32_t attend_grid;
 } dsmil_agg_route;
 
 int dsmil_agg_forward_route(const dsmil_agg_call* call, dsmil_agg_route* route);
```
